# EnnaDelfen/SUHMO

Measured on AMD Instinct MI355X. Metric: multigrid V-cycles/s (FAS head solve) + GSRB cell-updates/s; achieved HBM GB/s vs peak, higher is better.
Workload: dtype f64; 1 GPU; SHMIP-A head solve, 4096x4096 cells per GPU (square cells of 24.4 m), single AMR level, 64x64 boxes, 6 MG depths, 4+4 GSRB sweeps per depth, 16 bottom (BASELINE north_star: 4096^2 single-level); partition=none

## Files before the change

suhmo_amd/csrc/suhmo_bcoef.hip:

```cpp
#include "suhmo_hier.h"
#include "suhmo_level_int.h"
#include "suhmo_batch.h"
#include <algorithm>
#include <cmath>
#include <initializer_list>
#include <type_traits>
__device__ __forceinline__ void d_gradcc_val(const DV &v, const FP &fp, int hasMask, int i, int j, double &gx, double &gy)
{
    const double *__restrict__ phi = fp.f[SUHMO_F_PHI];
    int idx = cidx(v, i, j);
    double c = phi[idx];
    double e = phiE(v, phi, idx, i, c, false), w = phiW(v, phi, idx, i, c, false);
    double n = phiN(v, phi, idx, j, c, false), s = phiS(v, phi, idx, j, c, false);
    double gW = v.fdx * (c - w), gE = v.fdx * (e - c), gS = v.fdy * (c - s), gN = v.fdy * (n - c);
    if (hasMask) {
        const double *__restrict__ m = fp.f[SUHMO_F_MASK];
        bool mc = m[idx] < 1e-6;
        if (mc || m[idx - 1] < 1e-6) gW = 0.0;
        if (mc || m[idx + 1] < 1e-6) gE = 0.0;
        if (mc || m[idx - v.P] < 1e-6) gS = 0.0;
        if (mc || m[idx + v.P] < 1e-6) gN = 0.0;
    }
    gx = 0.5 * (gW + gE);
    gy = 0.5 * (gS + gN);
}
__device__ __forceinline__ void d_gradcc_at(const DV &v, const FP &fp, int hasMask, int i, int j)
{
    if (i >= v.nx || j >= v.ny) return;
    double gx, gy;
    d_gradcc_val(v, fp, hasMask, i, j, gx, gy);
    const int idx = cidx(v, i, j);
    fp.f[SUHMO_F_GRADX][idx] = gx;
    fp.f[SUHMO_F_GRADY][idx] = gy;
}
__device__ __forceinline__ void d_gradcc(const DV &v, const FP &fp, int hasMask)
{
    d_gradcc_at(v, fp, hasMask, blockIdx.x * blockDim.x + threadIdx.x, blockIdx.y * blockDim.y + threadIdx.y);
}
template <class T> __global__ __launch_bounds__(256) void k_gradcc(T t) { d_gradcc(t.view(), t.fields(), t.phys().use_mask_gradients); }
__global__ __launch_bounds__(256) void k_gradcc_list(DV v, FP fp, int hasMask, const int2 *__restrict__ cells, int n)
{
    const int t = blockIdx.x * blockDim.x + threadIdx.x;
    if (t >= n) return;
    d_gradcc_at(v, fp, hasMask, cells[t].x, cells[t].y);
}
__device__ __forceinline__ void d_grad_ghosts(const DV &v, double *__restrict__ gx, double *__restrict__ gy)
{
    int t = blockIdx.x * blockDim.x + threadIdx.x;
    double *g2[2] = {gx, gy};
    if (t < 2 * v.ny) {
        int side = t / v.ny, j = t % v.ny;
        if (v.cfx[side]) return;
        for (int c = 0; c < 2; c++) {
            double *g = g2[c];
            if (side == 0) { int idx = cidx(v, 0, j); g[idx - 1] = v.per[0] ? g[idx + v.nx - 1] : 2.0 * g[idx] - g[idx + 1]; }
            else { int idx = cidx(v, v.nx - 1, j); g[idx + 1] = v.per[0] ? g[idx - (v.nx - 1)] : 2.0 * g[idx] - g[idx - 1]; }
        }
        return;
    }
    t -= 2 * v.ny;
    if (t < 2 * v.nx) {
        int side = t / v.nx, i = t % v.nx;
        if (v.ext[side]) return;
        for (int c = 0; c < 2; c++) {
            double *g = g2[c];
            if (side == 0) { int idx = cidx(v, i, 0); g[idx - v.P] = v.per[1] ? g[idx + (v.ny - 1) * v.P] : 2.0 * g[idx] - g[idx + v.P]; }
            else { int idx = cidx(v, i, v.ny - 1); g[idx + v.P] = v.per[1] ? g[idx - (v.ny - 1) * v.P] : 2.0 * g[idx] - g[idx - v.P]; }
        }
    }
}
template <class T> __global__ void k_grad_ghosts(T t)
{
    const FP &fp = t.fields();
    d_grad_ghosts(t.view(), fp.f[SUHMO_F_GRADX], fp.f[SUHMO_F_GRADY]);
}
__device__ __forceinline__ void d_gradcc_ghosts(const DV &v, const FP &fp, int hasMask)
{
    const int i = blockIdx.x * blockDim.x + threadIdx.x, j = blockIdx.y * blockDim.y + threadIdx.y;
    if (i >= v.nx || j >= v.ny) return;
    double gx, gy, ox, oy;
    d_gradcc_val(v, fp, hasMask, i, j, gx, gy);
    const int idx = cidx(v, i, j);
    double *__restrict__ GX = fp.f[SUHMO_F_GRADX], *__restrict__ GY = fp.f[SUHMO_F_GRADY];
    GX[idx] = gx; GY[idx] = gy;
    if (i == 0 && !v.cfx[0]) {
        d_gradcc_val(v, fp, hasMask, v.per[0] ? v.nx - 1 : 1, j, ox, oy);
        GX[idx - 1] = v.per[0] ? ox : 2.0 * gx - ox; GY[idx - 1] = v.per[0] ? oy : 2.0 * gy - oy;
    }
    if (i == v.nx - 1 && !v.cfx[1]) {
        d_gradcc_val(v, fp, hasMask, v.per[0] ? 0 : v.nx - 2, j, ox, oy);
        GX[idx + 1] = v.per[0] ? ox : 2.0 * gx - ox; GY[idx + 1] = v.per[0] ? oy : 2.0 * gy - oy;
    }
    if (j == 0 && !v.ext[0]) {
        d_gradcc_val(v, fp, hasMask, i, v.per[1] ? v.ny - 1 : 1, ox, oy);
        GX[idx - v.P] = v.per[1] ? ox : 2.0 * gx - ox; GY[idx - v.P] = v.per[1] ? oy : 2.0 * gy - oy;
    }
    if (j == v.ny - 1 && !v.ext[1]) {
        d_gradcc_val(v, fp, hasMask, i, v.per[1] ? 0 : v.ny - 2, ox, oy);
        GX[idx + v.P] = v.per[1] ? ox : 2.0 * gx - ox; GY[idx + v.P] = v.per[1] ? oy : 2.0 * gy - oy;
    }
}
__global__ __launch_bounds__(256) void k_gradcc_ghosts(OnBoxes t) { d_gradcc_ghosts(t.view(), t.fields(), t.phys().use_mask_gradients); }
__global__ __launch_bounds__(256) void k_gradcc_ghosts_lv(suhmo_lvboxes lv, int hasMask)
{
    int z = blockIdx.z, q = -1;
#pragma unroll
    for (int t = 0; t < SUHMO_LVMAX; t++)
        if (t < lv.n && q < 0) { if (z < lv.nbox[t]) q = t; else z -= lv.nbox[t]; }
    if (q < 0) return;
    const DV *dv = nullptr; const FP *fp = nullptr;
#pragma unroll
    for (int t = 0; t < SUHMO_LVMAX; t++) if (t == q) { dv = lv.dv[t]; fp = lv.fp[t]; }
    d_gradcc_ghosts(dv[z], fp[z], hasMask);
}
__device__ __forceinline__ double d_re_val(const FP &fp, const suhmo_phys_t &ph, int idx)
{
    double gx = fp.f[SUHMO_F_GRADX][idx], gy = fp.f[SUHMO_F_GRADY][idx], B = fp.f[SUHMO_F_B][idx];
    double sg = sqrt(gx * gx + gy * gy);
    double discr = 1.0 + 4.0 * ph.omega * (B * B * B * ph.grav * sg) / (12.0 * ph.nu * ph.nu);
    return (-1.0 + sqrt(discr)) / (2.0 * ph.omega);
}
__device__ __forceinline__ void d_re(const DV &v, const FP &fp, suhmo_phys_t ph)
{
    int i = (int)(blockIdx.x * blockDim.x + threadIdx.x) - 1, j = (int)(blockIdx.y * blockDim.y + threadIdx.y) - 1;
    if (i > v.nx || j > v.ny) return;
    bool xo = (i < 0 || i >= v.nx), yo = (j < 0 || j >= v.ny);
    if (xo && yo) return;
    int idx = cidx(v, i, j);
    fp.f[SUHMO_F_RE][idx] = d_re_val(fp, ph, idx);
}
template <class T> __global__ __launch_bounds__(256) void k_re(T t) { d_re(t.view(), t.fields(), t.phys()); }
__device__ __forceinline__ double bcoef_face(const suhmo_phys_t &ph, double Rc, double Rm, double Bc, double Bm,
                                             double mc, double mm, bool dom_edge)
{
    double Ref = 0.5 * (Rc + Rm), Bf = 0.5 * (Bc + Bm);
    double mec;
    if (fabs(mc - mm) < 1e-10) mec = (mc > 0.0) ? 1.0 : -1.0; else mec = 0.0;
    if (dom_edge) mec = 0.0;
    double num_q = -(Bf * Bf * Bf * ph.grav);
    double denom_q = 12.0 * ph.nu * (1.0 + ph.omega * Ref);
    if (mec < 0.0 && ph.cutOffB > 0) return 0.0;
    return num_q / denom_q;
}
__device__ __forceinline__ void d_bcoef_faces(const DV &v, const FP &fp, suhmo_phys_t ph)
{
    int i = blockIdx.x * blockDim.x + threadIdx.x, j = blockIdx.y * blockDim.y + threadIdx.y;
    if (i > v.nx || j > v.ny) return;
    int idx = cidx(v, i, j);
    const double *__restrict__ Re = fp.f[SUHMO_F_RE], *__restrict__ B = fp.f[SUHMO_F_B], *__restrict__ m = fp.f[SUHMO_F_MASK];
    if (j < v.ny)
        fp.f[SUHMO_F_BX][idx] = bcoef_face(ph, Re[idx], Re[idx - 1], B[idx], B[idx - 1], m[idx], m[idx - 1], i + v.i0 == 0 || i + v.i0 == v.nxg);
    if (i < v.nx) {
        int jg = j + v.j0;
        fp.f[SUHMO_F_BY][idx] = bcoef_face(ph, Re[idx], Re[idx - v.P], B[idx], B[idx - v.P], m[idx], m[idx - v.P], jg == 0 || jg == v.nyg);
    }
}
template <class T> __global__ __launch_bounds__(256) void k_bcoef_faces(T t) { d_bcoef_faces(t.view(), t.fields(), t.phys()); }
__global__ __launch_bounds__(256) void k_re_bcoef(OnBoxes t)
{
    const DV &v = t.view();
    const FP &fp = t.fields();
    const suhmo_phys_t &ph = t.phys();
    const int i = (int)(blockIdx.x * blockDim.x + threadIdx.x) - 1, j = (int)(blockIdx.y * blockDim.y + threadIdx.y) - 1;
    if (i > v.nx || j > v.ny) return;
    const bool xo = (i < 0 || i >= v.nx), yo = (j < 0 || j >= v.ny);
    if (xo && yo) return;
    const int idx = cidx(v, i, j);
    const double Rc = d_re_val(fp, ph, idx);
    fp.f[SUHMO_F_RE][idx] = Rc;
    if (i < 0 || j < 0) return;
    const double *__restrict__ B = fp.f[SUHMO_F_B], *__restrict__ m = fp.f[SUHMO_F_MASK];
    if (j < v.ny)
        fp.f[SUHMO_F_BX][idx] = bcoef_face(ph, Rc, d_re_val(fp, ph, idx - 1), B[idx], B[idx - 1], m[idx], m[idx - 1], i + v.i0 == 0 || i + v.i0 == v.nxg);
    if (i < v.nx) {
        const int jg = j + v.j0;
        fp.f[SUHMO_F_BY][idx] = bcoef_face(ph, Rc, d_re_val(fp, ph, idx - v.P), B[idx], B[idx - v.P], m[idx], m[idx - v.P], jg == 0 || jg == v.nyg);
    }
}

template <bool INTERIOR, int BT_X, int BT_Y, bool MASKED>
__device__ __forceinline__ void bcoef_tile(const DV &v, const FP &fp, const suhmo_phys_t &ph, int hasMask_, double *sphi, double *sB, double *sM,
                                           unsigned *negflag, unsigned epoch, unsigned *smallflag)
{
    const int hasMask = MASKED ? hasMask_ : 0;
    constexpr int PW = BT_X + 4, PH = BT_Y + 4;
    constexpr int RW = BT_X + 2, RH = BT_Y + 2;
    constexpr int TX = BT_X + 2, TY = 256 / TX;
    constexpr int NK = RH / TY;
    static_assert(TX * TY == 256 && RH % TY == 0, "tile shape");
    double *sre = sphi;
    const int i0 = blockIdx.x * BT_X, j0 = blockIdx.y * BT_Y;
    const int tx = threadIdx.x, ty = threadIdx.y;
    const double *__restrict__ phi = fp.f[SUHMO_F_PHI], *__restrict__ Bf = fp.f[SUHMO_F_B], *__restrict__ mk = fp.f[SUHMO_F_MASK];
    double *__restrict__ bxo = fp.f[SUHMO_F_BX], *__restrict__ byo = fp.f[SUHMO_F_BY];
    const bool halo_lo = v.ext[0], halo_hi = v.ext[1], selfper_y = v.per[1] && !halo_lo && !halo_hi;
    auto xin = [&](int i) { return INTERIOR || (i >= 0 && i < v.nx) || v.per[0]; };
    auto yin = [&](int j) { return INTERIOR || (j >= 0 && j < v.ny) || selfper_y || (j < 0 && halo_lo && j >= -v.gy) || (j >= v.ny && halo_hi && j < v.ny + v.gy); };
    auto wrapx = [&](int i) { return (!INTERIOR && v.per[0]) ? (i < 0 ? i + v.nx : (i >= v.nx ? i - v.nx : i)) : i; };
    auto wrapy = [&](int j) { return (!INTERIOR && selfper_y) ? (j < 0 ? j + v.ny : (j >= v.ny ? j - v.ny : j)) : j; };

    for (int lj = ty; lj < PH; lj += TY) {
        const int j = j0 - 2 + lj;
        const bool yi = yin(j);
        for (int li = tx; li < PW; li += TX) {
            const int i = i0 - 2 + li;
            const bool xi = xin(i);
            double val = 0.0;
            if (xi && yi) val = phi[cidx(v, wrapx(i), wrapy(j))];
            else if (yi && (i == -1 || i == v.nx)) {
                int ic = i < 0 ? 0 : v.nx - 1, idx = cidx(v, ic, wrapy(j));
                double c = phi[idx];
                val = i < 0 ? phiW(v, phi, idx, ic, c, false) : phiE(v, phi, idx, ic, c, false);
            } else if (xi && (j == -1 || j == v.ny)) {
                int jc = j < 0 ? 0 : v.ny - 1, idx = cidx(v, wrapx(i), jc);
                double c = phi[idx];
                val = j < 0 ? phiS(v, phi, idx, jc, c, false) : phiN(v, phi, idx, jc, c, false);
            }
            sphi[lj * PW + li] = val;
        }
    }
    const int i = i0 - 1 + tx;
    const bool xi = xin(i);
    double Br[NK];
    bool hasB[NK];
    bool neg = false, small = false;
#pragma unroll
    for (int k = 0; k < NK; k++) {
        const int lj = ty + TY * k, j = j0 - 1 + lj;
        hasB[k] = INTERIOR || (i >= -1 && i <= v.nx && j >= -v.gy && j <= v.ny + v.gy - 1 && !((i < 0 || i >= v.nx) && (j < 0 || j >= v.ny)));
        double b = 0.0, m = 0.0;
        if (hasB[k]) { int idx = cidx(v, i, j); b = Bf[idx]; if (MASKED) m = mk[idx]; }
        if (MASKED) {
            neg = neg || (m < 0.0 && i >= 0 && i < v.nx && j >= 0 && j < v.ny);
            small = small || (hasB[k] && m < 1e-6 && j >= -1 && j <= v.ny);
        }
        Br[k] = b;
        sB[lj * RW + tx] = b;
        if (MASKED) sM[lj * RW + tx] = m;
    }
    if (MASKED && negflag && neg) *negflag = epoch;
    if (MASKED && smallflag && small) *smallflag = 1u;
    __syncthreads();
    auto gradcc = [&](int p, int gi, int gj, double &gx, double &gy) {
        double c = sphi[p], w = sphi[p - 1], e = sphi[p + 1], s = sphi[p - PW], n = sphi[p + PW];
        double gW = v.fdx * (c - w), gE = v.fdx * (e - c), gS = v.fdy * (c - s), gN = v.fdy * (n - c);
        if (hasMask) {
            int idx = cidx(v, wrapx(gi), wrapy(gj));
            bool mc = mk[idx] < 1e-6;
            if (mc || mk[idx - 1] < 1e-6) gW = 0.0;
            if (mc || mk[idx + 1] < 1e-6) gE = 0.0;
            if (mc || mk[idx - v.P] < 1e-6) gS = 0.0;
            if (mc || mk[idx + v.P] < 1e-6) gN = 0.0;
        }
        gx = 0.5 * (gW + gE); gy = 0.5 * (gS + gN);
    };
    double rer[NK];
#pragma unroll
    for (int k = 0; k < NK; k++) {
        const int lj = ty + TY * k, j = j0 - 1 + lj;
        const bool yi = yin(j);
        const int p = (lj + 1) * PW + (tx + 1);
        double gx = 0.0, gy = 0.0;
        if (xi && yi) {
            gradcc(p, i, j, gx, gy);
        } else if (xi != yi) {
            int d = 0, di = 0, dj = 0;
            if (!xi && (i == -1 || i == v.nx)) { di = i < 0 ? 1 : -1; d = di; }
            else if (!yi && (j == -1 || j == v.ny)) { dj = j < 0 ? 1 : -1; d = dj * PW; }
            if (d != 0) {
                double g1x, g1y, g2x, g2y;
                gradcc(p + d, i + di, j + dj, g1x, g1y);
                gradcc(p + 2 * d, i + 2 * di, j + 2 * dj, g2x, g2y);
                gx = 2.0 * g1x - g2x; gy = 2.0 * g1y - g2y;
            }
        }
        double re = 0.0;
        if (hasB[k]) {
            double B = Br[k];
            double sg = sqrt(gx * gx + gy * gy);
            double discr = 1.0 + 4.0 * ph.omega * (B * B * B * ph.grav * sg) / (12.0 * ph.nu * ph.nu);
            re = (-1.0 + sqrt(discr)) / (2.0 * ph.omega);
        }
        rer[k] = re;
    }
    __syncthreads();
#pragma unroll
    for (int k = 0; k < NK; k++) sre[(ty + TY * k) * RW + tx] = rer[k];
    __syncthreads();
    const int nxt = (!INTERIOR && i0 + BT_X >= v.nx) ? v.nx - i0 + 1 : BT_X, nyt = (!INTERIOR && j0 + BT_Y >= v.ny) ? v.ny - j0 + 1 : BT_Y;
    const int fx = tx - 1;
    if (fx >= 0 && fx < nxt) {
        for (int fy = ty; fy < nyt; fy += TY) {
            const int j = j0 + fy, idx = cidx(v, i, j), r = (fy + 1) * RW + tx;
            if (INTERIOR || j < v.ny)
                bxo[idx] = bcoef_face(ph, sre[r], sre[r - 1], sB[r], sB[r - 1], MASKED ? sM[r] : 1.0, MASKED ? sM[r - 1] : 1.0, !INTERIOR && (i == 0 || i == v.nx));
            if (INTERIOR || i < v.nx) {
                int jg = j + v.j0;
                byo[idx] = bcoef_face(ph, sre[r], sre[r - RW], sB[r], sB[r - RW], MASKED ? sM[r] : 1.0, MASKED ? sM[r - RW] : 1.0, !INTERIOR && (jg == 0 || jg == v.nyg));
            }
        }
    }
}
struct MaskHalo { const double *m[SUHMO_MAXDEPTH]; int nx[SUHMO_MAXDEPTH], ny[SUHMO_MAXDEPTH], P[SUHMO_MAXDEPTH], gy[SUHMO_MAXDEPTH]; int nd, lo, hi; };
__global__ __launch_bounds__(256) void k_mask_halo_report(MaskHalo h, unsigned *negflag, unsigned epoch, unsigned *smallflag)
{
    const int d = blockIdx.z, i = blockIdx.x * blockDim.x + threadIdx.x;
    if (d >= h.nd || i >= h.nx[d]) return;
    const int g = h.gy[d];
    bool neg = false, small = false;
    for (int r = blockIdx.y; r < 2 * g; r += gridDim.y) {
        const bool top = r >= g;
        if (top ? !h.hi : !h.lo) continue;
        const int j = top ? h.ny[d] + (r - g) : -1 - r;
        const double *__restrict__ row = h.m[d] + (long)(j + g) * h.P[d] + SUHMO_XOFF;
        const double m = row[i];
        neg = neg || m < 0.0;
        const int dist = top ? r - g : r;
        small = small || ((d == 0 && dist < 2) ? m < 1e-6 : m < 0.0);
        if (smallflag && d == 0 && i == 0 && (j == -1 || j == h.ny[d])) small = small || row[-1] < 1e-6 || row[h.nx[d]] < 1e-6;
    }
    if (negflag && neg) *negflag = epoch;
    if (smallflag && small) *smallflag = 1u;
}
template <int BT_X, int BT_Y, bool MASKED>
__device__ __forceinline__ void d_bcoef_fused(const DV &v, const FP &fp, const suhmo_phys_t &ph, int hasMask, unsigned *negflag, unsigned epoch, unsigned *smallflag)
{
    __shared__ double sphi[(BT_X + 4) * (BT_Y + 4)], sB[(BT_X + 2) * (BT_Y + 2)], sM[MASKED ? (BT_X + 2) * (BT_Y + 2) : 1];
    const int i0 = blockIdx.x * BT_X, j0 = blockIdx.y * BT_Y;
    const bool interior = i0 - 2 >= 0 && i0 + BT_X + 1 <= v.nx - 1 && j0 - 2 >= 0 && j0 + BT_Y + 1 <= v.ny - 1;
    if (interior) bcoef_tile<true, BT_X, BT_Y, MASKED>(v, fp, ph, hasMask, sphi, sB, sM, negflag, epoch, smallflag);
    else bcoef_tile<false, BT_X, BT_Y, MASKED>(v, fp, ph, hasMask, sphi, sB, sM, negflag, epoch, smallflag);
}
template <class T, int BT_X, int BT_Y, bool MASKED = true>
__global__ __launch_bounds__(256) void k_bcoef_fused(T t, unsigned *negflag, unsigned epoch, unsigned *smallflag)
{
    const suhmo_phys_t ph = t.phys();
    if (std::is_same<T, OnMembers>::value) { negflag = nullptr; epoch = 0u; smallflag = nullptr; }
    d_bcoef_fused<BT_X, BT_Y, MASKED>(t.view(), t.fields(), ph, ph.use_mask_gradients, negflag, epoch, smallflag);
}
template <class T> int launch_bcoef_fused(const T &t, bool wide, unsigned *flag, unsigned epoch, hipStream_t st, unsigned *small, bool unmasked)
{
    if constexpr (std::is_same<T, OnLevel>::value) {
        const dim3 gw((t.nx() + 125) / 126, (t.ny() + 13) / 14), gn((t.nx() + 61) / 62, (t.ny() + 13) / 14);
        unsigned *const none = nullptr;
        if (unmasked && wide) return launch_grid(k_bcoef_fused<T, 126, 14, false>, t, gw, dim3(128, 2), st, none, 0u, none);
        if (unmasked) return launch_grid(k_bcoef_fused<T, 62, 14, false>, t, gn, dim3(64, 4), st, none, 0u, none);
        if (wide) return launch_grid(k_bcoef_fused<T, 126, 14>, t, gw, dim3(128, 2), st, flag, epoch, small);
    }
    return launch_grid(k_bcoef_fused<T, 62, 14>, t, dim3((t.nx() + 61) / 62, (t.ny() + 13) / 14), dim3(64, 4), st, flag, epoch, small);
}
template int launch_bcoef_fused(const OnMembers &, bool, unsigned *, unsigned, hipStream_t, unsigned *, bool);
void suhmo_mask_poll(suhmo_level *L)
{
    if (!L->mask_scan_pending) return;
    const hipError_t e = hipEventQuery(L->mask_ev);
    if (e == hipErrorNotReady) { (void)hipGetLastError(); return; }
    L->mask_scan_pending = 0;
    if (e != hipSuccess) { (void)hipGetLastError(); L->mask_scan_errors++; return; }
    if (L->mask_scan_version == L->mask_version) L->mask_state = *(volatile unsigned *)L->mask_host ? SUHMO_MASK_DIRTY : SUHMO_MASK_CLEAN;
}
int suhmo_mask_scan_begin(suhmo_level *L, hipStream_t st)
{
    if (!L->mask_ev) HIPCHK(hipEventCreateWithFlags(&L->mask_ev, hipEventDisableTiming));
    HIPCHK(hipMemsetAsync(suhmo_mask_scan_word(L), 0, sizeof(unsigned), st));
    return 0;
}
int suhmo_mask_scan_end(suhmo_level *L, hipStream_t st)
{
    HIPCHK(hipMemcpyAsync(L->mask_host, suhmo_mask_scan_word(L), sizeof(unsigned), hipMemcpyDeviceToHost, st));
    HIPCHK(hipEventRecord(L->mask_ev, st));
    L->mask_scan_pending = 1; L->mask_scan_version = L->mask_version; L->mask_scans++;
    return 0;
}
template <class T> int launch_re(const T &t, hipStream_t st) { return launch_over(k_re<T>, t, GHOSTED, st); }
template <class T> int launch_bcoef_faces(const T &t, hipStream_t st) { return launch_over(k_bcoef_faces<T>, t, FACES, st); }
template <class T> int launch_grad_cc(const T &t, hipStream_t st)
{
    int rc = launch_over(k_gradcc<T>, t, CELLS, st);
    return rc ? rc : launch_over(k_grad_ghosts<T>, t, PERIMETER, st);
}
template int launch_re(const OnLevel &, hipStream_t);
template int launch_re(const OnBoxes &, hipStream_t);
template int launch_re(const OnMembers &, hipStream_t);
template int launch_bcoef_faces(const OnLevel &, hipStream_t);
template int launch_bcoef_faces(const OnBoxes &, hipStream_t);
template int launch_bcoef_faces(const OnMembers &, hipStream_t);
template int launch_grad_cc(const OnMembers &, hipStream_t);

static bool bcoef_is_fused(const suhmo_level *L, int depth)
{
    const Depth &D = L->d[depth];
    return L->bcoef_fused && D.v.nx >= 4 && D.v.ny >= 4 && (!(D.v.ext[0] || D.v.ext[1]) || (D.v.gy >= 2 && D.v.ny >= 2))
           && L->desc.nx_global == 0;
}
bool suhmo_mask_would_scan(const suhmo_level *L)
{
    return L->mask_known && !L->mask_view && L->mask_scan_errors < 3 && L->mask_state == SUHMO_MASK_UNKNOWN && !L->mask_scan_pending && L->mask_host
           && !L->mask_capturing && bcoef_is_fused(L, 0);
}
extern "C" int suhmo_level_update_operator(suhmo_level_t *L, int depth, suhmo_stream_t s)
{
    SUHMO_TIME("VCAMRNonLinearPoissonOp::UpdateOperator");
    ARG(L); ARG(depth >= 0 && depth < L->ndepth);
    HIPCHK(hipSetDevice(L->device));
    hipStream_t st = (hipStream_t)s;
    Depth &D = L->d[depth];
    const bool fused = bcoef_is_fused(L, depth);
    int rc = suhmo_ensure_phi_halo(L, depth, fused ? 2 : 1, st); if (rc) return rc;
    if (fused) {
        const bool wide = L->bcoef_tile_x == 126 && D.v.nx >= 256;
        unsigned *flag = nullptr;
        if (depth == 0) { L->maskflag_epoch = 0; L->mask_reported = 0; }
        if (depth == 0 && !L->mask_capturing) suhmo_mask_poll(L);
        const bool unmasked = depth == 0 && suhmo_mask_clean(L, 0);
        unsigned *small = nullptr;
        const bool scan = depth == 0 && suhmo_mask_would_scan(L);
        if (scan) { small = suhmo_mask_scan_word(L); if ((rc = suhmo_mask_scan_begin(L, st))) return rc; }
        if (depth == 0 && L->mask_capturing && L->mask_known && !L->mask_view && !unmasked && L->mask_host) { small = suhmo_mask_scan_word(L); L->mask_scan_captured = 1; }
        if (depth == 0 && L->skip_mask && !unmasked) {
            flag = suhmo_mask_report_word(L);
            if (++L->mask_epoch == 0) L->mask_epoch = 1;
            L->mask_reported = 1;
        }
        if ((rc = launch_bcoef_fused(on_level(L, depth), wide, flag, L->mask_epoch, st, small, unmasked))) return rc;
        if (unmasked) L->bcoef_unmasked++;
        if ((flag || small) && (D.v.ext[0] || D.v.ext[1])) {
            MaskHalo h;
            h.nd = 0; h.lo = D.v.ext[0]; h.hi = D.v.ext[1];
            const int last = L->coarse_mask_ok ? (L->agg ? L->agg_depth : L->ndepth) : 1;
            int gmax = 1;
            for (int k = 0; k < last && k < SUHMO_MAXDEPTH; k++) {
                const Depth &Dk = L->d[k];
                h.m[k] = Dk.fp.f[SUHMO_F_MASK]; h.nx[k] = Dk.v.nx; h.ny[k] = Dk.v.ny; h.P[k] = Dk.v.P; h.gy[k] = Dk.v.gy;
                if (Dk.v.gy > gmax) gmax = Dk.v.gy;
// ... 402 lines not shown
```

suhmo_amd/csrc/suhmo_common.h:

```cpp
#pragma once
#include <hip/hip_runtime.h>
#include <cstdio>
#include <cstdlib>
#include <cstring>
#include <utility>
#include <string>
#include <vector>
#include "../../include/suhmo_hip.h"

#define SUHMO_XOFF 16
#define SUHMO_MAXDEPTH 16

struct DV {
    int nx, ny;
    int P;
    int gy;
    int rows;
    int j0, nyg;
    double dx, dy;
    double rdx, rdy;
    double fdx, fdy;
    double alpha, beta;
    int bct[2][2];
    double two_v[2][2];
    double neu[2][2];
    int per[2];
    int ext[2];
    int i0, nxg;
    int cfx[2];
    int rk[2];
};

struct FP { double *f[SUHMO_F_COUNT]; };

__host__ __device__ __forceinline__ int cidx(const DV &v, int i, int j)
{
    return (j + v.gy) * v.P + SUHMO_XOFF + i;
}

__device__ __forceinline__ double phiW(const DV &v, const double *__restrict__ p, int idx, int i, double c, bool homog)
{
    if (i > 0 || v.cfx[0]) return p[idx - 1];
    if (v.per[0]) return p[idx + v.nx - 1];
    if (v.bct[0][0] == 0) return (homog ? 0.0 : v.two_v[0][0]) - c;
    return homog ? c : c + v.neu[0][0];
}
__device__ __forceinline__ double phiE(const DV &v, const double *__restrict__ p, int idx, int i, double c, bool homog)
{
    if (i < v.nx - 1 || v.cfx[1]) return p[idx + 1];
    if (v.per[0]) return p[idx - (v.nx - 1)];
    if (v.bct[0][1] == 0) return (homog ? 0.0 : v.two_v[0][1]) - c;
    return homog ? c : c + v.neu[0][1];
}
__device__ __forceinline__ double phiS(const DV &v, const double *__restrict__ p, int idx, int j, double c, bool homog)
{
    if (j > 0 || v.ext[0]) return p[idx - v.P];
    if (v.per[1]) return p[idx + (v.ny - 1) * v.P];
    if (v.bct[1][0] == 0) return (homog ? 0.0 : v.two_v[1][0]) - c;
    return homog ? c : c + v.neu[1][0];
}
__device__ __forceinline__ double phiN(const DV &v, const double *__restrict__ p, int idx, int j, double c, bool homog)
{
    if (j < v.ny - 1 || v.ext[1]) return p[idx + v.P];
    if (v.per[1]) return p[idx - (v.ny - 1) * v.P];
    if (v.bct[1][1] == 0) return (homog ? 0.0 : v.two_v[1][1]) - c;
    return homog ? c : c + v.neu[1][1];
}

__device__ __forceinline__ void nl_terms(const suhmo_phys_t &ph, double phi, double B, double Pi,
                                         double zb, double mask, double &nl, double &dnl)
{
    if (!ph.use_NL || mask < 0.0) { nl = 0.0; dnl = 0.0; return; }
    double N = Pi - ph.rho_w_g * (phi - zb);
    nl = -ph.A * B * N * N * N;
    dnl = 3.0 * ph.A * B * 1000.0 * ph.grav * N * N;
    if (ph.cutOffbr > B) {
        nl = nl * (1.0 - (ph.cutOffbr - B) / ph.cutOffbr);
        dnl = dnl * B / ph.cutOffbr;
    }
    if (ph.maxOffbr < B) {
        nl = nl * (1.0 - (ph.maxOffbr - B) / ph.maxOffbr);
        dnl = dnl * B / ph.maxOffbr;
    }
}

__device__ __forceinline__ double lofphi_cell(const DV &v, double aterm, double c, double e, double w,
                                              double n, double s, double bxE, double bxW, double byN,
                                              double byS, double nl)
{
    return aterm * c
           - v.beta * (bxE * (e - c) * v.rdx - bxW * (c - w) * v.rdx
                       + byN * (n - c) * v.rdy - byS * (c - s) * v.rdy)
           + nl;
}

__device__ __forceinline__ double lambda_cell(const DV &v, double aterm, double bxE, double bxW,
                                              double byN, double byS)
{
    double lam = aterm;
    lam = lam + v.rdx * v.beta * (bxE + bxW);
    lam = lam + v.rdy * v.beta * (byN + byS);
    return lam;
}

struct Depth {
    DV v;
    FP fp;
    size_t elems;
    int nbox;
    int prolong_pending;
    int rhs_pending;
    double *phi_alt;
    int phi_fresh;
};

struct VGraph {
    int key[4]; hipGraphExec_t exec;
    double *p0[SUHMO_MAXDEPTH], *a0[SUHMO_MAXDEPTH];
    double *p1[SUHMO_MAXDEPTH], *a1[SUHMO_MAXDEPTH];
    double *rhs;
    int rout_req, rout_done, rout_np; const double *rout_rhs;
    int mask_clean; long n_bcoef_unmasked, n_relax_unmasked;
    int has_scan;
};
struct ProfEv { hipEvent_t a, b; long cells; int restricts; };

struct suhmo_level {
    int ndepth;
    int batch_owned;
    int stub;
    Depth d[SUHMO_MAXDEPTH];
    suhmo_level_desc_t desc;
    std::vector<int> boxes;
    suhmo_phys_t ph;
    int device;
    double *scratch;
    double *hscratch;
    double *hscratch_dev;
    unsigned long long hseq;
    int poll_readback;
    size_t scratch_elems;
    suhmo_exchange_fn ex;
    suhmo_allreduce_max_fn ar;
    suhmo_allreduce_fn ar2;
    int (*ard)(void *user, double *dev_values, int n, int op, suhmo_stream_t s);
    void *user;
    int (*ex_begin)(void *user);
    int (*ex_end)(void *user, suhmo_level *L, suhmo_stream_t s);
    long graph_max_cells;
    std::vector<VGraph> vgraphs; int vgraph_seen[4]; hipStream_t gstream;
    long vgraph_replays;
    suhmo_level *gap; double gap_dt;
    void *rccl;
    int faces_deferred;
    void *ipc; int ipc_owner;
    long agg_min_cells;
    int agg_depth, agg_world, agg_rank;
    suhmo_level *agg;
    int agg_static_stale;
    suhmo_allgather_fn ag; void *ag_user;
    double *agg_send, *agg_recv; size_t agg_cap; long agg_gathers;
    int resout_req, resout_armed, resout_done; const double *resout_rhs; long resout_count;
    int resout_np;
    long frhs_stream, frhs_tile;
    int prof_on;
    std::vector<ProfEv> prof;
    int gsrb_variant;
    long fused_min_cells;
    int bcoef_fused;
    int bcoef_tile_x;
    int fused_nt;
    int fused_restrict;
    int fused_hc;
    int fas_rhs_fused;
    int strips_rhs_local;
    int skip_mask;
    int mask_reported;
    int coarse_mask_ok;
    unsigned mask_epoch, maskflag_epoch;
    int mask_known, mask_state;
    unsigned mask_version, mask_scan_version;
    int mask_scan_pending, mask_capturing;
    int mask_scan_captured;
    int mask_view;
    int mask_scan_errors;
    unsigned *mask_host; hipEvent_t mask_ev;
    long mask_scans, bcoef_unmasked, relax_unmasked;
    int overlap_halo;
    hipStream_t xstream; hipEvent_t xev[2]; long overlapped;
    int tile_strips;
    int tile_chunks;
    int resid_in_relax;
    int fas_rhs_in_relax;
    long tile_max_cells;
    int tile_restrict;
    int tile_order;
    int bottom_solver; long bottom_one_launch_max_cells;
    unsigned long long *bottom_ctr; long bottom_host_iters, bottom_host_solves;
    int gsrb_tile, tile_t, tile_s;
};

enum { SUHMO_MASK_UNKNOWN = 0, SUHMO_MASK_CLEAN = 1, SUHMO_MASK_DIRTY = 2 };
static inline void suhmo_mask_written(suhmo_level *L)
{
    L->coarse_mask_ok = 0; L->maskflag_epoch = 0;
    L->mask_version++; L->mask_state = SUHMO_MASK_UNKNOWN;
}
static inline void suhmo_mask_halo_written(suhmo_level *L) { L->mask_version++; L->mask_state = SUHMO_MASK_UNKNOWN; }
bool suhmo_mask_would_scan(const suhmo_level *L);
#define SUHMO_HSCRATCH_DOUBLES 64
#define SUHMO_HSCRATCH_MASK 60
static inline unsigned *suhmo_mask_report_word(const suhmo_level *L) { return (unsigned *)(L->scratch + L->scratch_elems - 1); }
static inline unsigned *suhmo_mask_scan_word(const suhmo_level *L) { return suhmo_mask_report_word(L) + 1; }
int suhmo_mask_scan_begin(suhmo_level *L, hipStream_t st);
int suhmo_mask_scan_end(suhmo_level *L, hipStream_t st);
void suhmo_mask_poll(suhmo_level *L);
static inline bool suhmo_mask_clean(const suhmo_level *L, int depth)
{
    return L->mask_known && !L->mask_view && L->mask_state == SUHMO_MASK_CLEAN && (depth == 0 || L->coarse_mask_ok) && L->desc.nx_global == 0;
}
void suhmo_set_error(const char *fmt, ...);
struct SuhmoTimer { const char *name; double t0; int mode; explicit SuhmoTimer(const char *n); ~SuhmoTimer(); };
#define SUHMO_TIME(label) SuhmoTimer suhmo_tm_(label)
#define HIPCHK(x) do { hipError_t e_ = (x); if (e_ != hipSuccess) { \
    suhmo_set_error("%s:%d %s -> %s", __FILE__, __LINE__, #x, hipGetErrorString(e_)); return -2; } } while (0)
#define ARG(cond) do { if (!(cond)) { suhmo_set_error("%s:%d bad argument: %s", __FILE__, __LINE__, #cond); return -1; } } while (0)

double *suhmo_field(suhmo_level *L, int depth, int field);
int suhmo_level_create_(suhmo_level_t **out, const suhmo_level_desc_t *desc, bool stub);
void suhmo_level_share_transport(suhmo_level *dst, const suhmo_level *src);
int suhmo_level_materialize_(suhmo_level *L);
void suhmo_fp_changed();
unsigned long suhmo_fp_epoch();
struct SwapGuard {
    double **a, **b; bool armed;
    SwapGuard() : a(nullptr), b(nullptr), armed(false) {}
    void arm(double **a_, double **b_) { a = a_; b = b_; std::swap(*a, *b); armed = true; suhmo_fp_changed(); }
    void back() { if (armed) { std::swap(*a, *b); armed = false; suhmo_fp_changed(); } }
    ~SwapGuard() { back(); }
};
int suhmo_average_operator_all(suhmo_level *L, int nd, hipStream_t st);
int suhmo_restrict_both(suhmo_level *L, int depth, hipStream_t st);
bool suhmo_gsrb_can_fuse_prolong(suhmo_level *L, int depth, int sweeps);
int suhmo_level_residual_and_norm(suhmo_level *L, double *out, hipStream_t st);
int suhmo_level_norm_from_partials(suhmo_level *L, int np, double *out, hipStream_t st);
bool suhmo_gsrb_can_fuse_rhs(suhmo_level *L, int depth, int sweeps, bool rhs_local = false);
int suhmo_launch_gsrb(suhmo_level *L, int depth, int sweeps, int tail, hipStream_t st, int *restricted = nullptr);
void suhmo_level_drop_graphs(suhmo_level *L);
int suhmo_ensure_phi_halo(suhmo_level *L, int depth, int need, hipStream_t st);
int suhmo_fas_coarse_rhs(suhmo_level *L, int depth, hipStream_t st, int hcomp = 0);
struct HostSlot { double *val; unsigned long long *flag; unsigned long long seq; };
HostSlot suhmo_host_slot(suhmo_level *L);
int suhmo_readback(suhmo_level *L, hipStream_t st, double *out, double *out2 = nullptr);
HostSlot suhmo_reduce_slot(suhmo_level *L);
int suhmo_reduce_finish(suhmo_level *L, hipStream_t st, int n, int op, double *out, double *out2 = nullptr);
__device__ __forceinline__ void suhmo_publish(const HostSlot &h, double v)
{
    if (!h.val) return;
    h.val[0] = v;
    __hip_atomic_store(h.flag, h.seq, __ATOMIC_RELEASE, __HIP_MEMORY_SCOPE_SYSTEM);
}
int suhmo_build_mg_coefficients(suhmo_level *L, bool with_faces, hipStream_t st);
void suhmo_ipc_release(suhmo_level *L);
int suhmo_ipc_batch(suhmo_level *L, int open, hipStream_t st);
int suhmo_agg_setup(suhmo_level *L);
void suhmo_agg_release(suhmo_level *L);
int suhmo_agg_gather_static(suhmo_level *L, bool with_faces, hipStream_t st);
int suhmo_agg_gather_faces(suhmo_level *L, int nd, hipStream_t st);
int suhmo_agg_gather_state(suhmo_level *L, hipStream_t st);
int suhmo_agg_scatter(suhmo_level *L, hipStream_t st);
int suhmo_exchange_list(suhmo_level *L, int depth, const int *fields, int n, hipStream_t st);
bool suhmo_bottom_one_launch(const suhmo_level *L, int dep);
int suhmo_bottom_configure(suhmo_level *L, int solver, long one_launch_max_cells);
long suhmo_bottom_counter(const suhmo_level *L, int which);
int suhmo_bottom_solve(suhmo_level *L, int dep, int tail, hipStream_t st);
static inline int suhmo_halo_rows(const DV &v) { return v.gy < v.ny ? v.gy : v.ny; }
struct SolveNoInit {
    double rnorm, initial_rnorm, norm_last;
    int iter;
    void start(double r) { rnorm = r; initial_rnorm = r; norm_last = 2.0 * r; iter = 0; }
    bool go(const suhmo_solver_params_t *sp) const
    {
        const bool goNorm = rnorm > sp->norm_thresh, goRedu = rnorm > sp->eps * initial_rnorm, goIter = iter < sp->max_iter;
        const bool goHang = iter < sp->imin || rnorm < (1.0 - sp->hang) * norm_last, goMin = iter < sp->iter_min;
        return goMin || (goIter && goRedu && goHang && goNorm);
    }
    void cycled(double r) { norm_last = rnorm; rnorm = r; iter++; }
};
template <class Residual, class Cycle>
int suhmo_solve_no_init(const suhmo_solver_params_t *sp, int *iters, double *hist, Residual residual, Cycle cycle)
{
    int rc;
    double rnorm = 0.0;
    if ((rc = residual(&rnorm))) return rc;
    SolveNoInit s;
    s.start(rnorm);
    if (hist) hist[0] = rnorm;
    while (s.go(sp)) {
        if ((rc = cycle()) || (rc = residual(&rnorm))) return rc;
        s.cycled(rnorm);
        if (hist) hist[s.iter] = rnorm;
    }
    if (iters) *iters = s.iter;
    return 0;
}
```

suhmo_amd/csrc/suhmo_fas.hip:

```cpp
#include "suhmo_common.h"
#include <cstdlib>

static int eff_depths(const suhmo_level *L, const suhmo_solver_params_t *sp)
{
    int nd = L->ndepth;
    if (sp->max_depth >= 0 && sp->max_depth + 1 < nd) nd = sp->max_depth + 1;
    return nd;
}

static int relax(suhmo_level *L, int dep, int sweeps, int tail, suhmo_stream_t s, bool observable = false, int *restricted = nullptr)
{
    L->resout_armed = observable && dep == 0 && L->resout_req && L->resid_in_relax;
    int rc = suhmo_launch_gsrb(L, dep, sweeps, tail, (hipStream_t)s, restricted);
    L->resout_armed = 0;
    if (rc) return rc;
    if (sweeps > 0 && observable) return suhmo_level_fill_ghosts(L, dep, SUHMO_F_PHI, 1, s);
    return 0;
}

static int rows_after_prolong(int dep, int num_smooth)
{
    int tail_post = 2;
    for (int d = 1; d <= dep; d++) tail_post = (2 * num_smooth + tail_post + 1) / 2;
    return 2 * num_smooth + tail_post;
}
int suhmo_prolong_with_halo(suhmo_level *L, int depth, hipStream_t st);

static int fas_cycle(suhmo_level *L, int dep, const suhmo_solver_params_t *sp, int nd, suhmo_stream_t s)
{
    int rc;
    const int S = sp->num_smooth;
    const int tail_post = dep == 0 ? 2 : (rows_after_prolong(dep - 1, S) + 1) / 2;
    if (dep == nd - 1) {
        if (!L->bottom_solver) return relax(L, dep, sp->num_bottom, tail_post, s, dep == 0);
        if ((rc = relax(L, dep, sp->num_bottom, tail_post, s))) return rc;
        if ((rc = suhmo_bottom_solve(L, dep, tail_post, (hipStream_t)s))) return rc;
        return dep == 0 ? suhmo_level_fill_ghosts(L, dep, SUHMO_F_PHI, 0, s) : 0;
    }
    Depth &C = L->d[dep + 1];
    int restricted = 0;
    if ((rc = relax(L, dep, S, rows_after_prolong(dep, S), s, false, &restricted))) return rc;
    if (!restricted && (rc = suhmo_restrict_both(L, dep, (hipStream_t)s))) return rc;
    if (L->agg && dep + 1 == L->agg_depth) {
        suhmo_level *A = L->agg;
        const int ndA = nd - L->agg_depth;
        if (L->agg_static_stale && (rc = suhmo_agg_gather_static(L, true, (hipStream_t)s))) return rc;
        if ((rc = suhmo_agg_gather_state(L, (hipStream_t)s))) return rc;
        const int next_sweeps = ndA == 1 ? sp->num_bottom : S;
        if (suhmo_gsrb_can_fuse_rhs(A, 0, next_sweeps)) A->d[0].rhs_pending = 1;
        else if ((rc = suhmo_fas_coarse_rhs(A, 0, (hipStream_t)s))) return rc;
        if ((rc = fas_cycle(A, 0, sp, ndA, s))) return rc;
        if ((rc = suhmo_agg_scatter(L, (hipStream_t)s))) return rc;
        if (suhmo_gsrb_can_fuse_prolong(L, dep, S)) L->d[dep].prolong_pending = 1;
        else if ((rc = suhmo_prolong_with_halo(L, dep, (hipStream_t)s))) return rc;
        return relax(L, dep, S, tail_post, s, dep == 0);
    }
    const bool one_pass_rhs = L->fas_rhs_fused != 0;
    const bool rhs_local = L->ex && (C.v.rk[0] || C.v.rk[1]) && one_pass_rhs && L->desc.nx_global == 0 && L->strips_rhs_local
                           && suhmo_halo_rows(C.v) >= 2;
    if (rhs_local) {
        static const int both[2] = {SUHMO_F_PHI, SUHMO_F_RES};
        if ((rc = suhmo_exchange_list(L, dep + 1, both, 2, (hipStream_t)s))) return rc;
    } else if ((rc = suhmo_ensure_phi_halo(L, dep + 1, suhmo_halo_rows(C.v), (hipStream_t)s))) return rc;
    if (one_pass_rhs && (L->desc.nx_global == 0)) {
        const int next_sweeps = (dep + 1 == nd - 1) ? sp->num_bottom : S;
        if (suhmo_gsrb_can_fuse_rhs(L, dep + 1, next_sweeps, rhs_local)) C.rhs_pending = 1;
        else if ((rc = suhmo_fas_coarse_rhs(L, dep + 1, (hipStream_t)s, rhs_local ? suhmo_halo_rows(C.v) - 1 : 0))) return rc;
    } else {
        HIPCHK(hipMemcpyAsync(C.fp.f[SUHMO_F_PHIOLD], C.fp.f[SUHMO_F_PHI], C.elems * sizeof(double), hipMemcpyDeviceToDevice, (hipStream_t)s));
        if ((rc = suhmo_level_apply_op(L, dep + 1, 0, s))) return rc;
        if ((rc = suhmo_level_axby(L, dep + 1, SUHMO_F_RHS, SUHMO_F_RES, SUHMO_F_LPHI, 1.0, 1.0, s))) return rc;
    }
    if (!rhs_local && (rc = suhmo_level_exchange(L, dep + 1, SUHMO_F_RHS, s))) return rc;
    if ((rc = fas_cycle(L, dep + 1, sp, nd, s))) return rc;
    if (suhmo_gsrb_can_fuse_prolong(L, dep, S)) {
        L->d[dep].prolong_pending = 1;
    } else {
        if ((rc = suhmo_prolong_with_halo(L, dep, (hipStream_t)s))) return rc;
    }
    return relax(L, dep, S, tail_post, s, dep == 0);
}

static int vcycle_body(suhmo_level *L, const suhmo_solver_params_t *sp, int nd, suhmo_stream_t s)
{
    int rc;
    if (sp->bcoeff_otf) {
        L->faces_deferred = 1;
        rc = suhmo_level_update_operator(L, 0, s);
        if (rc) { L->faces_deferred = 0; return rc; }
        if (L->mask_reported) L->maskflag_epoch = L->mask_epoch;
        if ((rc = suhmo_average_operator_all(L, nd, (hipStream_t)s))) return rc;
    } else L->maskflag_epoch = 0;
    rc = fas_cycle(L, 0, sp, nd, s);
    L->maskflag_epoch = 0;
    return rc;
}

void suhmo_level_drop_graphs(suhmo_level *L)
{
    if (getenv("SUHMO_GRAPH_DEBUG")) { int ok = 0; for (VGraph &g : L->vgraphs) ok += g.exec != nullptr; fprintf(stderr,
        "[suhmo] level %dx%d: %zu V-cycle graphs, %d executable\n", L->d[0].v.nx, L->d[0].v.ny, L->vgraphs.size(), ok); }
    for (VGraph &g : L->vgraphs) if (g.exec) (void)hipGraphExecDestroy(g.exec);
    L->vgraphs.clear();
    if (L->gstream) { (void)hipStreamDestroy(L->gstream); L->gstream = nullptr; }
}
static int vcycle_graph(suhmo_level *L, const suhmo_solver_params_t *sp, int nd, suhmo_stream_t s, bool &done)
{
    done = false;
    const int key[4] = {sp->num_smooth, sp->num_bottom, sp->bcoeff_otf, nd};
    const int mask_clean = (suhmo_mask_clean(L, 0) ? 1 : 0) | (L->ndepth > 1 && suhmo_mask_clean(L, 1) ? 2 : 0);
    const bool scanning = sp->bcoeff_otf && suhmo_mask_would_scan(L);
    auto launch = [&](const VGraph &g) {
        int rc = 0;
        if (scanning && (rc = suhmo_mask_scan_begin(L, (hipStream_t)s))) return rc;
        HIPCHK(hipGraphLaunch(g.exec, (hipStream_t)s)); L->vgraph_replays++;
        if (scanning && (rc = suhmo_mask_scan_end(L, (hipStream_t)s))) return rc;
        return 0;
    };
    auto replayed = [&](const VGraph &g) {
        L->bcoef_unmasked += g.n_bcoef_unmasked; L->relax_unmasked += g.n_relax_unmasked;
        if (g.rout_done) { L->resout_done = 1; L->resout_count++; L->resout_np = g.rout_np; }
    };
    auto at_start = [&](const VGraph &g) {
        if (memcmp(g.key, key, sizeof(key)) || g.mask_clean != mask_clean) return false;
        for (int d = 0; d < L->ndepth; d++) if (L->d[d].fp.f[SUHMO_F_PHI] != g.p0[d] || L->d[d].phi_alt != g.a0[d]) return false;
        if (g.rout_req != (L->resid_in_relax ? L->resout_req : 0) || g.rout_rhs != L->resout_rhs) return false;
        return L->d[0].fp.f[SUHMO_F_RHS] == g.rhs;
    };
    for (const VGraph &g : L->vgraphs)
        if (at_start(g)) {
            if (!g.exec || (scanning && !g.has_scan)) return 0;
            { int rc = launch(g); if (rc) return rc; }
            for (int d = 0; d < L->ndepth; d++) { L->d[d].fp.f[SUHMO_F_PHI] = g.p1[d]; L->d[d].phi_alt = g.a1[d]; } suhmo_fp_changed();
            replayed(g);
            done = true;
            return 0;
        }
    for (int k = 0; k < 4; k++) if (L->vgraph_seen[k] != key[k]) { memcpy(L->vgraph_seen, key, sizeof(key)); return 0; }
    if (L->vgraphs.size() >= 16) return 0;
    if (!L->gstream) HIPCHK(hipStreamCreateWithFlags(&L->gstream, hipStreamNonBlocking));
    VGraph g; memcpy(g.key, key, sizeof(key)); g.exec = nullptr; g.mask_clean = mask_clean; g.has_scan = 0;
    for (int d = 0; d < SUHMO_MAXDEPTH; d++) { g.p0[d] = g.a0[d] = g.p1[d] = g.a1[d] = nullptr; }
    for (int d = 0; d < L->ndepth; d++) { g.p0[d] = L->d[d].fp.f[SUHMO_F_PHI]; g.a0[d] = L->d[d].phi_alt; }
    g.rhs = L->d[0].fp.f[SUHMO_F_RHS];
    g.rout_req = L->resid_in_relax ? L->resout_req : 0; g.rout_rhs = L->resout_rhs; g.rout_done = 0;
    const int rout_before = L->resout_done; const long rout_count = L->resout_count;
    const long bcoef_unmasked = L->bcoef_unmasked, relax_unmasked = L->relax_unmasked;
    HIPCHK(hipStreamSynchronize((hipStream_t)s));
    hipGraph_t graph = nullptr;
    hipError_t e = hipStreamBeginCapture(L->gstream, hipStreamCaptureModeThreadLocal);
    int rc = 0;
    if (e == hipSuccess) {
        L->mask_capturing = 1; L->mask_scan_captured = 0;
        rc = vcycle_body(L, sp, nd, (suhmo_stream_t)L->gstream);
        L->mask_capturing = 0; g.has_scan = L->mask_scan_captured;
        e = hipStreamEndCapture(L->gstream, &graph);
    }
    g.n_bcoef_unmasked = L->bcoef_unmasked - bcoef_unmasked; g.n_relax_unmasked = L->relax_unmasked - relax_unmasked;
    L->bcoef_unmasked = bcoef_unmasked; L->relax_unmasked = relax_unmasked;
    g.rout_done = L->resout_count != rout_count;
    g.rout_np = L->resout_np;
    L->resout_done = rout_before; L->resout_count = rout_count;
    bool clean = true;
    for (int d = 0; d < L->ndepth; d++) {
        clean = clean && !L->d[d].prolong_pending && !L->d[d].rhs_pending;
        g.p1[d] = L->d[d].fp.f[SUHMO_F_PHI]; g.a1[d] = L->d[d].phi_alt;
        L->d[d].prolong_pending = 0; L->d[d].rhs_pending = 0;
        L->d[d].fp.f[SUHMO_F_PHI] = g.p0[d]; L->d[d].phi_alt = g.a0[d];
    }
    if (e == hipSuccess && rc == 0 && clean && graph && hipGraphInstantiate(&g.exec, graph, nullptr, nullptr, 0) != hipSuccess) g.exec = nullptr;
    if (!(e == hipSuccess && rc == 0 && clean)) g.exec = nullptr;
    if (graph) (void)hipGraphDestroy(graph);
    (void)hipGetLastError();
    L->vgraphs.push_back(g);
    if (!g.exec || (scanning && !g.has_scan)) return 0;
    if ((rc = launch(g))) return rc;
    for (int d = 0; d < L->ndepth; d++) { L->d[d].fp.f[SUHMO_F_PHI] = g.p1[d]; L->d[d].phi_alt = g.a1[d]; } suhmo_fp_changed();
    replayed(g);
    done = true;
    return 0;
}

extern "C" int suhmo_level_vcycle(suhmo_level_t *L, const suhmo_solver_params_t *sp, suhmo_stream_t s)
{
    SUHMO_TIME("AMRFASMultiGrid::VCycle");
    ARG(L && sp);
    HIPCHK(hipSetDevice(L->device));
    int nd = eff_depths(L, sp);
    const Depth &D = L->d[0];
    const bool ext = D.v.ext[0] || D.v.ext[1];
    const bool host_bottom = L->bottom_solver && !suhmo_bottom_one_launch(L, nd - 1);
    suhmo_mask_poll(L);
    if (L->graph_max_cells > 0 && !L->ex && !ext && !L->prof_on && !host_bottom && (long)D.v.nx * D.v.ny <= L->graph_max_cells) {
        bool done = false;
        int rc = vcycle_graph(L, sp, nd, s, done);
        if (rc || done) return rc;
    }
    return vcycle_body(L, sp, nd, s);
}

extern "C" int suhmo_level_solve(suhmo_level_t *L, const suhmo_solver_params_t *sp, int *iters, double *hist, suhmo_stream_t s)
{
    SUHMO_TIME("AMRFASMultiGrid::solve");
    ARG(L && sp);
    HIPCHK(hipSetDevice(L->device));
    bool have_res = false;
    int np = 0;
    auto residual = [&](double *rnorm) {
        if (!have_res) return suhmo_level_residual_and_norm(L, rnorm, (hipStream_t)s);
        if (np > 0) return suhmo_level_norm_from_partials(L, np, rnorm, (hipStream_t)s);
        return suhmo_level_norm(L, 0, SUHMO_F_RES, 0, rnorm, s);
    };
    auto cycle = [&] {
        L->resout_req = 1 | 4; L->resout_rhs = nullptr; L->resout_done = 0; L->resout_np = 0;
        int rc = suhmo_level_vcycle(L, sp, s);
        have_res = L->resout_done != 0;
        np = have_res ? L->resout_np : 0;
        L->resout_req = 0; L->resout_done = 0; L->resout_np = 0;
        return rc;
    };
    int rc = suhmo_solve_no_init(sp, iters, hist, residual, cycle);
    if (rc) return rc;
    return suhmo_level_fill_ghosts(L, 0, SUHMO_F_PHI, 0, s);
}
```

suhmo_amd/csrc/suhmo_gsrb.hip:

```cpp
#include "suhmo_hier.h"
#include "suhmo_batch.h"
#include <type_traits>

template <bool HAS_ALPHA>
__device__ __forceinline__ void d_gsrb_pass_simple(const DV &v, const FP &fp, suhmo_phys_t ph, int pass, int jlo, int jhi,
                                                   const FP *__restrict__ ft = nullptr, const int2 *__restrict__ push = nullptr)
{
    int j = jlo + (int)(blockIdx.y * blockDim.y + threadIdx.y);
    int t = blockIdx.x * blockDim.x + threadIdx.x;
    if (j > jhi) return;
    int i = 2 * t + ((j + v.j0 + pass) & 1);
    if (i >= v.nx) return;
    double *__restrict__ phi = fp.f[SUHMO_F_PHI];
    int idx = cidx(v, i, j);
    double c = phi[idx];
    double e = phiE(v, phi, idx, i, c, false), w = phiW(v, phi, idx, i, c, false);
    double n = phiN(v, phi, idx, j, c, false), s = phiS(v, phi, idx, j, c, false);
    double bxW = fp.f[SUHMO_F_BX][idx], bxE = fp.f[SUHMO_F_BX][idx + 1];
    double byS = fp.f[SUHMO_F_BY][idx], byN = fp.f[SUHMO_F_BY][idx + v.P];
    double nl, dnl;
    nl_terms(ph, c, fp.f[SUHMO_F_B][idx], fp.f[SUHMO_F_PI][idx], fp.f[SUHMO_F_ZB][idx],
             fp.f[SUHMO_F_MASK][idx], nl, dnl);
    double aterm = HAS_ALPHA ? v.alpha * fp.f[SUHMO_F_ACOEF][idx] : v.alpha;
    double lofphi = lofphi_cell(v, aterm, c, e, w, n, s, bxE, bxW, byN, byS, nl);
// ... 89 lines not shown
            const int dx = li < BOXG ? BOXG - li : (li >= BOXG + tw ? li - (BOXG + tw - 1) : 0), dy = lj < BOXG ? BOXG - lj : (lj >= BOXG + th ? lj - (BOXG + th - 1) : 0);
            const int d = max(dx, dy);
            const FP &fb = b == k ? fk : ft[b];
            if (d >= BOXG) { pl[q] = fb.f[fsrc][off]; continue; }
            const int Pb = b == k ? v.P : vt[b].P;
            cb[s][c] = b; co[s][c] = off; cd[s][c] = d;
            pl[q] = fb.f[fsrc][off];
            c_rhs[s][c] = fb.f[SUHMO_F_RHS][off];
            c_bxW[s][c] = fb.f[SUHMO_F_BX][off]; c_bxE[s][c] = fb.f[SUHMO_F_BX][off + 1];
            c_byS[s][c] = fb.f[SUHMO_F_BY][off]; c_byN[s][c] = fb.f[SUHMO_F_BY][off + Pb];
            c_B[s][c] = fb.f[SUHMO_F_B][off]; c_Pi[s][c] = fb.f[SUHMO_F_PI][off]; c_zb[s][c] = fb.f[SUHMO_F_ZB][off]; c_mk[s][c] = fb.f[SUHMO_F_MASK][off];
            c_at[s][c] = HAS_ALPHA ? v.alpha * fb.f[SUHMO_F_ACOEF][off] : v.alpha;
        }
    __syncthreads();
    int nk[S][2];
    double hW[S][2], hE[S][2], hS[S][2], hN[S][2];
#pragma unroll
    for (int s = 0; s < S; s++)
#pragma unroll
        for (int c = 0; c < 2; c++) {
            nk[s][c] = 0; hW[s][c] = hE[s][c] = hS[s][c] = hN[s][c] = 0.0;
            const int q = cq[s][c], b = cb[s][c];
            if (b < 0) continue;
            const bool oW = own[q - 1] < 0, oE = own[q + 1] < 0, oS = own[q - LW] < 0, oN = own[q + LW] < 0;
            if (!(oW || oE || oS || oN)) continue;
            const DV &vb = b == k ? v : vt[b];
            const double *__restrict__ psrc = (b == k ? fk : ft[b]).f[fsrc];
            const int off = co[s][c];
            if (oW) { if (vb.cfx[0]) { nk[s][c] |= 1; hW[s][c] = psrc[off - 1]; } else if (vb.bct[0][0] == 0) { nk[s][c] |= 2; hW[s][c] = vb.two_v[0][0];
                } else { nk[s][c] |= 3; hW[s][c] = vb.neu[0][0]; } }
            if (oE) { if (vb.cfx[1]) { nk[s][c] |= 1 << 2; hE[s][c] = psrc[off + 1]; } else if (vb.bct[0][1] == 0) { nk[s][c] |= 2 << 2; hE[s][c] = vb.two_v[0][1];
                } else { nk[s][c] |= 3 << 2; hE[s][c] = vb.neu[0][1]; } }
            if (oS) { if (vb.ext[0]) { nk[s][c] |= 1 << 4; hS[s][c] = psrc[off - vb.P]; } else if (vb.bct[1][0] == 0) { nk[s][c] |= 2 << 4;
                hS[s][c] = vb.two_v[1][0]; } else { nk[s][c] |= 3 << 4; hS[s][c] = vb.neu[1][0]; } }
            if (oN) { if (vb.ext[1]) { nk[s][c] |= 1 << 6; hN[s][c] = psrc[off + vb.P]; } else if (vb.bct[1][1] == 0) { nk[s][c] |= 2 << 6;
                hN[s][c] = vb.two_v[1][1]; } else { nk[s][c] |= 3 << 6; hN[s][c] = vb.neu[1][1]; } }
        }
    auto outside = [](int kind, double g, double c) { return kind == 1 ? g : (kind == 2 ? g - c : c + g); };
    auto update = [&](int q, int kinds, double g_w, double g_e, double g_s, double g_n, double rhs, double bxW, double bxE, double byS, double byN, double B,
        double Pi, double zb, double mk, double at) {
        const double c = pl[q];
        double w, e, sv, n;
        if (kinds == 0) { w = pl[q - 1]; e = pl[q + 1]; sv = pl[q - LW]; n = pl[q + LW]; }
        else {
            w = (kinds & 3) ? outside(kinds & 3, g_w, c) : pl[q - 1];
            e = ((kinds >> 2) & 3) ? outside((kinds >> 2) & 3, g_e, c) : pl[q + 1];
            sv = ((kinds >> 4) & 3) ? outside((kinds >> 4) & 3, g_s, c) : pl[q - LW];
            n = ((kinds >> 6) & 3) ? outside((kinds >> 6) & 3, g_n, c) : pl[q + LW];
        }
        double nl, dnl;
        nl_terms(ph, c, B, Pi, zb, mk, nl, dnl);
        const double lofphi = lofphi_cell(v, at, c, e, w, n, sv, bxE, bxW, byN, byS, nl);
        const double lam = lambda_cell(v, at, bxE, bxW, byN, byS);
        const double denom = 1.0e-16 + lam + dnl;
        pl[q] = c + (rhs - lofphi) / denom;
    };
    for (int m = 0; m < npass; m++) {
        const int reach = npass - 1 - m;
        if ((m & 1) == 0) {
#pragma unroll
            for (int s = 0; s < S; s++)
                if (cb[s][0] >= 0 && cd[s][0] <= reach)
                    update(cq[s][0], nk[s][0], hW[s][0], hE[s][0], hS[s][0], hN[s][0], c_rhs[s][0], c_bxW[s][0], c_bxE[s][0], c_byS[s][0], c_byN[s][0], c_B[s][0],
                        c_Pi[s][0], c_zb[s][0], c_mk[s][0], c_at[s][0]);
        } else {
#pragma unroll
            for (int s = 0; s < S; s++)
                if (cb[s][1] >= 0 && cd[s][1] <= reach)
                    update(cq[s][1], nk[s][1], hW[s][1], hE[s][1], hS[s][1], hN[s][1], c_rhs[s][1], c_bxW[s][1], c_bxE[s][1], c_byS[s][1], c_byN[s][1], c_B[s][1],
                        c_Pi[s][1], c_zb[s][1], c_mk[s][1], c_at[s][1]);
        }
        __syncthreads();
    }
    const double *__restrict__ psrc = fk.f[fsrc];
    double *__restrict__ pdst = fk.f[fdst];
    const bool gW = bcg && !v.cfx[0] && !v.per[0], gE = bcg && !v.cfx[1] && !v.per[0], gS = bcg && !v.ext[0] && !v.per[1], gN = bcg && !v.ext[1] && !v.per[1];
    for (int q = tid; q < tw * th; q += BOXNT) {
        const int jj = q / tw, ii = q - jj * tw, gi = x0 + ii, gj = y0 + jj, idx = cidx(v, gi, gj);
        const double c = pl[(BOXG + jj) * LW + BOXG + ii];
        pdst[idx] = c;
        if (gW && gi == 0) pdst[idx - 1] = phiW(v, pdst, idx, gi, c, true);
        if (gE && gi == v.nx - 1) pdst[idx + 1] = phiE(v, pdst, idx, gi, c, true);
        if (gS && gj == 0) pdst[idx - v.P] = phiS(v, pdst, idx, gj, c, true);
        if (gN && gj == v.ny - 1) pdst[idx + v.P] = phiN(v, pdst, idx, gj, c, true);
    }
    if (blockIdx.x == 0)
        for (int q = tid; q < 2 * (v.nx + 2) + 2 * v.ny; q += BOXNT) {
            int ii, jj;
            bool filled;
            if (q < v.nx + 2) { ii = q - 1; jj = -1; filled = gS && ii >= 0 && ii < v.nx; }
            else if (q < 2 * (v.nx + 2)) { ii = q - (v.nx + 2) - 1; jj = v.ny; filled = gN && ii >= 0 && ii < v.nx; }
            else if (q < 2 * (v.nx + 2) + v.ny) { ii = -1; jj = q - 2 * (v.nx + 2); filled = gW; }
            else { ii = v.nx; jj = q - 2 * (v.nx + 2) - v.ny; filled = gE; }
            if (filled) continue;
            const int idx = cidx(v, ii, jj);
            pdst[idx] = psrc[idx];
        }
}
template <int G, int T, int S>
static void launch_box(const suhmo_multi &m, const suhmo_phys_t &ph, bool has_alpha, const void *halo, const int *hbase, int fsrc, int fdst, int npass, int bc_ghosts, hipStream_t st)
{
    const dim3 grd(((m.maxnx + T - 1) / T) * ((m.maxny + T - 1) / T), m.nbox);
    if (has_alpha) hipLaunchKernelGGL((k_gsrb_box_m<true, G, T, S>), grd, dim3(BoxGeom<G, T, S>::NT), 0, st, m.dv, m.fp, (const int2 *)halo, hbase, ph, fsrc, fdst, npass, bc_ghosts);
    else hipLaunchKernelGGL((k_gsrb_box_m<false, G, T, S>), grd, dim3(BoxGeom<G, T, S>::NT), 0, st, m.dv, m.fp, (const int2 *)halo, hbase, ph, fsrc, fdst, npass, bc_ghosts);
}
int suhmo_multi_gsrb_box(const suhmo_multi &m, const suhmo_phys_t &ph, bool has_alpha, const void *halo, const int *hbase, int fsrc, int fdst, int npass, int bc_ghosts, hipStream_t st)
{
    if (m.nbox <= 0) return 0;
    if (npass < 1 || npass > 2 * SUHMO_BOX_HALO) { suhmo_set_error("internal: %d colour passes in one box launch", npass); return -4; }
    if (npass > 4) launch_box<8, 16, 1>(m, ph, has_alpha, halo, hbase, fsrc, fdst, npass, bc_ghosts, st);
    else launch_box<4, 16, 1>(m, ph, has_alpha, halo, hbase, fsrc, fdst, npass, bc_ghosts, st);
    HIPCHK(hipGetLastError());
    return 0;
}

struct FusedGeom {
    int W;
    int Hc;
    int nstrips, nchunks, ntiles;
    int ylo, yhi;
    int jbeg, jend;
    int wrap_y;
    const unsigned *negflag; unsigned mask_epoch;
    int nchl, chunk0, chunk1, edges;
    const double *pc, *pco; int Pc, gyc;
    double *rres, *rphi; int rP, rgy;
    const double *fres; double *frhs, *flphi, *fphiold;
    const double *ortrue; double *ores, *olphi;
    double *onorm;
};

template <bool MASKED> struct RowMask { double mask[2]; };
template <> struct RowMask<false> {};
template <bool MASKED>
struct RowCoef : RowMask<MASKED> {
    double rhs[2], B[2], Pi[2], zb[2], a[2], byS[2], byN[2];
    double bx0, bx1, bx2;
};
template <bool MASKED> __device__ __forceinline__ double row_mask(const RowCoef<MASKED> &q, int a)
{
    if constexpr (MASKED) return q.mask[a]; else return 1.0;
}
#define CP2(d, s, f) d.f[0] = s.f[0]; d.f[1] = s.f[1]
template <bool HAS_ALPHA, bool MASKED>
__device__ __forceinline__ void copy_coef(RowCoef<MASKED> &d, const RowCoef<MASKED> &s)
{
    CP2(d, s, rhs); CP2(d, s, B); CP2(d, s, Pi); CP2(d, s, zb);
    if constexpr (MASKED) { CP2(d, s, mask); }
    if (HAS_ALPHA) { CP2(d, s, a); }
    CP2(d, s, byS); CP2(d, s, byN);
    d.bx0 = s.bx0; d.bx1 = s.bx1; d.bx2 = s.bx2;
}

template <int K, bool HAS_ALPHA, int NT, int RM = 0, bool FRHS = false, bool MASKED = true>
__global__ __launch_bounds__(NT) void k_gsrb_fused(DV v, FP fp, const double *__restrict__ pin,
                                                   double *__restrict__ pout, suhmo_phys_t ph, FusedGeom g)
{
    constexpr bool ROUT = RM == 2, RR = RM != 0;
    static_assert(!(FRHS && (RR || HAS_ALPHA)), "the right-hand side is formed in the plain launch of an alpha = 0 operator");
    constexpr int LW = 2 * NT, R = 2 * K + 3 + (RR ? 1 : 0);
    constexpr int HX = 2 * K + (RR ? 2 : 0), EY = RR ? 1 : 0;
    __shared__ double lds[R * LW];

    int b = blockIdx.x, q = g.ntiles / 8, rem = g.ntiles % 8, xcd = b % 8;
    int tile = xcd * q + (xcd < rem ? xcd : rem) + b / 8;
    int strip = tile / g.nchl, chunk = tile % g.nchl;
    chunk = g.edges ? (chunk < g.chunk0 ? chunk : g.chunk1 + (chunk - g.chunk0)) : g.chunk0 + chunk;

    const int t = threadIdx.x;
    const int c0 = strip * g.W;
    const int xl = 2 * t;
    const int i0 = c0 - HX + xl;
    const bool in_row = xl < g.W + 2 * HX;
    int im = i0;
    if (v.per[0]) { if (im < 0) im += v.nx; else if (im >= v.nx) im -= v.nx; }
    const bool cval = in_row && im >= 0 && im < v.nx;
    const int cend = (c0 + g.W < v.nx) ? c0 + g.W : v.nx;
    const bool own = cval && i0 >= c0 && i0 < cend;

    const int jA = g.jbeg + chunk * g.Hc;
    const int jB = (jA + g.Hc < g.jend) ? jA + g.Hc : g.jend;
    const int jmin = (jA - EY - 2 * K > g.ylo) ? jA - EY - 2 * K : g.ylo;
    const int jmax = (jB - 1 + EY + 2 * K < g.yhi) ? jB - 1 + EY + 2 * K : g.yhi;

    const double *__restrict__ f_rhs = fp.f[SUHMO_F_RHS], *__restrict__ f_B = fp.f[SUHMO_F_B];
    const double *__restrict__ f_Pi = fp.f[SUHMO_F_PI], *__restrict__ f_zb = fp.f[SUHMO_F_ZB];
    const double *__restrict__ f_mask = fp.f[SUHMO_F_MASK], *__restrict__ f_a = fp.f[SUHMO_F_ACOEF];
    const double *__restrict__ f_bx = fp.f[SUHMO_F_BX], *__restrict__ f_by = fp.f[SUHMO_F_BY];

    auto wrapj = [&](int j) { if (g.wrap_y) { if (j < 0) j += v.ny; else if (j >= v.ny) j -= v.ny; } return j; };
    auto ld2 = [&](const double *__restrict__ p, int idx) { return *reinterpret_cast<const double2 *>(p + idx); };

    RowCoef<MASKED> cf0, cf1, cf2, cf3, cf4, cf5;
    double racc = 0.0, raccp = 0.0;
    double nmax = 0.0;
    const bool xbc = !v.per[0] && (c0 - HX <= 0 || c0 + g.W + HX >= v.nx);
    const bool ybc = !v.per[1] && (jmin <= 0 || jmax >= v.ny - 1);
    double2 pnext = make_double2(0.0, 0.0);
    double2 pprev = make_double2(0.0, 0.0);
    bool usemask = false;
    if constexpr (MASKED) usemask = !g.negflag || *g.negflag == g.mask_epoch;

    int sr = 0;
    auto ring = [](int x) { return x < 0 ? x + R : x; };
    for (int r = jmin - 1; r <= jB - 1 + 2 * K + EY; r++) {
        bool lphi = cval && (r + 1 >= jmin) && (r + 1 <= jmax);
        if (lphi) {
            const int jr = wrapj(r + 1);
            pnext = ld2(pin, cidx(v, im, jr));
            if (g.pc) {
                const int ic = ((jr >> 1) + g.gyc) * g.Pc + SUHMO_XOFF + (im >> 1);
                const double corr = 1.0 * g.pc[ic] + (-1.0) * g.pco[ic];
                pnext.x = pnext.x + corr; pnext.y = pnext.y + corr;
            }
        }
        bool lcf = cval && (r >= jmin) && (r <= jmax);
        if (lcf) {
            int idx = cidx(v, im, wrapj(r));
#define LD2(dst, p, ix) { double2 t_ = ld2(p, ix); dst[0] = t_.x; dst[1] = t_.y; }
            LD2(cf0.rhs, (FRHS ? g.fres : f_rhs), idx); LD2(cf0.B, f_B, idx); LD2(cf0.Pi, f_Pi, idx);
            LD2(cf0.zb, f_zb, idx);
            if constexpr (MASKED) { if (usemask) { LD2(cf0.mask, f_mask, idx); } else { cf0.mask[0] = 1.0; cf0.mask[1] = 1.0; } }
            if (HAS_ALPHA) LD2(cf0.a, f_a, idx);
            LD2(cf0.byS, f_by, idx); LD2(cf0.byN, f_by, idx + v.P);
            double2 bxp = ld2(f_bx, idx);
            cf0.bx0 = bxp.x; cf0.bx1 = bxp.y; cf0.bx2 = f_bx[idx + 2];
        }
        __syncthreads();

        if constexpr (FRHS) {
            const int jf = r - 1;
            if (cval && jf >= jmin && jf <= jmax) {
                const int s0 = ring(sr - 1), sN = sr;
                const double *row = lds + s0 * LW;
                double lo[2], cc[2];
#pragma unroll
                for (int a = 0; a < 2; a++) {
                    const int x = xl + a, i = im + a;
                    double c = row[x];
                    double w = row[(a == 0 && xl == 0) ? 0 : x - 1], e = row[(a == 1 && xl == LW - 2) ? LW - 1 : x + 1];
                    double n = lds[sN * LW + x], s = a ? pprev.y : pprev.x;
                    if (xbc) {
                        if (i == 0) w = (v.bct[0][0] == 0) ? v.two_v[0][0] - c : c + v.neu[0][0];
                        if (i == v.nx - 1) e = (v.bct[0][1] == 0) ? v.two_v[0][1] - c : c + v.neu[0][1];
                    }
                    if (ybc) {
                        if (jf == 0 && !v.ext[0]) s = (v.bct[1][0] == 0) ? v.two_v[1][0] - c : c + v.neu[1][0];
                        if (jf == v.ny - 1 && !v.ext[1]) n = (v.bct[1][1] == 0) ? v.two_v[1][1] - c : c + v.neu[1][1];
                    }
                    double nl, dnl;
                    nl_terms(ph, c, cf1.B[a], cf1.Pi[a], cf1.zb[a], row_mask(cf1, a), nl, dnl);
                    const double bxW = a ? cf1.bx1 : cf1.bx0, bxE = a ? cf1.bx2 : cf1.bx1;
                    lo[a] = lofphi_cell(v, v.alpha, c, e, w, n, s, bxE, bxW, cf1.byN[a], cf1.byS[a], nl);
                    cc[a] = c;
                }
                cf1.rhs[0] = 1.0 * cf1.rhs[0] + 1.0 * lo[0]; cf1.rhs[1] = 1.0 * cf1.rhs[1] + 1.0 * lo[1];
                const bool lo_end = v.ext[0] && chunk == 0, hi_end = v.ext[1] && chunk == g.nchunks - 1;
                const int jP0 = lo_end ? jmin : jA, jP1 = hi_end ? jmax + 1 : jB;
                const int jR0 = lo_end ? jmin + 1 : jA, jR1 = hi_end ? jmax : jB;
                if (own && jf >= jP0 && jf < jP1) {
                    const int idx = cidx(v, i0, jf);
                    if (jf >= jR0 && jf < jR1) {
                        *reinterpret_cast<double2 *>(g.flphi + idx) = make_double2(lo[0], lo[1]);
                        *reinterpret_cast<double2 *>(g.frhs + idx) = make_double2(cf1.rhs[0], cf1.rhs[1]);
                    }
                    *reinterpret_cast<double2 *>(g.fphiold + idx) = make_double2(cc[0], cc[1]);
                }
                pprev = make_double2(cc[0], cc[1]);
            }
            __syncthreads();
        }

        auto advance_a = [&](const int m, const RowCoef<MASKED> &q, auto a_tag) {
            constexpr int a = decltype(a_tag)::value;
            const int j = r - m;
            const int x = xl + a, i = im + a;
            const int s0 = ring(sr - m), sN = ring(sr - m + 1), sS = ring(sr - m - 1);
            const double *row = lds + s0 * LW;
            double c = row[x];
            double w = row[(a == 0 && xl == 0) ? 0 : x - 1], e = row[(a == 1 && xl == LW - 2) ? LW - 1 : x + 1];
            double n = lds[sN * LW + x], s = lds[sS * LW + x];
            if (xbc) {
                if (i == 0) w = (v.bct[0][0] == 0) ? v.two_v[0][0] - c : c + v.neu[0][0];
                if (i == v.nx - 1) e = (v.bct[0][1] == 0) ? v.two_v[0][1] - c : c + v.neu[0][1];
            }
            if (ybc) {
                if (j == 0 && !v.ext[0]) s = (v.bct[1][0] == 0) ? v.two_v[1][0] - c : c + v.neu[1][0];
                if (j == v.ny - 1 && !v.ext[1]) n = (v.bct[1][1] == 0) ? v.two_v[1][1] - c : c + v.neu[1][1];
            }
            double nl, dnl;
            nl_terms(ph, c, q.B[a], q.Pi[a], q.zb[a], row_mask(q, a), nl, dnl);
            const double bxW = a ? q.bx1 : q.bx0, bxE = a ? q.bx2 : q.bx1;
            double aterm = HAS_ALPHA ? v.alpha * q.a[a] : v.alpha;
            double lofphi = lofphi_cell(v, aterm, c, e, w, n, s, bxE, bxW, q.byN[a], q.byS[a], nl);
            double lam = lambda_cell(v, aterm, bxE, bxW, q.byN[a], q.byS[a]);
            double denom = 1.0e-16 + lam + dnl;
            lds[s0 * LW + x] = c + (q.rhs[a] - lofphi) / denom;
        };
        auto advance = [&](const int m, const RowCoef<MASKED> &q) {
            const int j = r - m;
            if (j >= jmin && j <= jmax) {
                const int a = (j + v.j0 + ((m - 1) & 1)) & 1;
                if (a) { if (cval) advance_a(m, q, std::integral_constant<int, 1>()); }
                else   { if (cval) advance_a(m, q, std::integral_constant<int, 0>()); }
            }
        };
        advance(1, cf1);
        __syncthreads();
        advance(2, cf2);
        if constexpr (K >= 2) {
            __syncthreads();
            advance(3, cf3);
            __syncthreads();
            advance(4, cf4);
        }

        if constexpr (RR) {
            const int jr = r - 2 * K - 1;
            if (own && jr >= jA && jr < jB && jr >= 0 && jr < v.ny) {
                const RowCoef<MASKED> &q = (K >= 2) ? cf5 : cf3;
                const int s0 = ring(sr - (2 * K + 1)), sN = ring(sr - 2 * K), sS = ring(sr - (2 * K + 2));
                const double *row = lds + s0 * LW;
                double acc = (jr & 1) ? racc : 0.0, accp = (jr & 1) ? raccp : 0.0;
                double lo2[2] = {0.0, 0.0};
#pragma unroll
                for (int a = 0; a < 2; a++) {
                    const int x = xl + a, i = im + a;
                    double c = row[x], w = row[x - 1], e = row[x + 1];
                    double n = lds[sN * LW + x], s = lds[sS * LW + x];
                    if (xbc) {
                        if (i == 0) w = (v.bct[0][0] == 0) ? v.two_v[0][0] - c : c + v.neu[0][0];
                        if (i == v.nx - 1) e = (v.bct[0][1] == 0) ? v.two_v[0][1] - c : c + v.neu[0][1];
                    }
                    if (ybc) {
                        if (jr == 0 && !v.ext[0]) s = (v.bct[1][0] == 0) ? v.two_v[1][0] - c : c + v.neu[1][0];
                        if (jr == v.ny - 1 && !v.ext[1]) n = (v.bct[1][1] == 0) ? v.two_v[1][1] - c : c + v.neu[1][1];
                    }
                    double nl, dnl;
                    nl_terms(ph, c, q.B[a], q.Pi[a], q.zb[a], row_mask(q, a), nl, dnl);
                    const double bxW = a ? q.bx1 : q.bx0, bxE = a ? q.bx2 : q.bx1;
                    double aterm = HAS_ALPHA ? v.alpha * q.a[a] : v.alpha;
                    double lofphi = lofphi_cell(v, aterm, c, e, w, n, s, bxE, bxW, q.byN[a], q.byS[a], nl);
                    if constexpr (ROUT) lo2[a] = lofphi;
                    else {
                        acc = acc + (q.rhs[a] - lofphi) / 4.0;
                        accp = accp + c / 4.0;
                    }
                }
                if constexpr (ROUT) {
                    const int idx = cidx(v, i0, jr);
                    const double2 rt = *reinterpret_cast<const double2 *>(g.ortrue + idx);
                    const double r0 = -1.0 * lo2[0] + 1.0 * rt.x, r1 = -1.0 * lo2[1] + 1.0 * rt.y;
                    *reinterpret_cast<double2 *>(g.ores + idx) = make_double2(r0, r1);
                    if (g.olphi) *reinterpret_cast<double2 *>(g.olphi + idx) = make_double2(lo2[0], lo2[1]);
                    nmax = fmax(nmax, fmax(fabs(r0), fabs(r1)));
                } else if (jr & 1) {
                    const int ic = ((jr >> 1) + g.rgy) * g.rP + SUHMO_XOFF + (i0 >> 1);
                    g.rres[ic] = acc; g.rphi[ic] = accp;
                } else { racc = acc; raccp = accp; }
            }
        }
        {
            const int jo = r - 2 * K;
            if (own && jo >= jA && jo < jB) {
                const int so = ring(sr - 2 * K);
                double2 o = make_double2(lds[so * LW + xl], lds[so * LW + xl + 1]);
                *reinterpret_cast<double2 *>(pout + cidx(v, i0, jo)) = o;
            }
        }
        sr = sr + 1 == R ? 0 : sr + 1;
        if (in_row) { lds[sr * LW + xl] = pnext.x; lds[sr * LW + xl + 1] = pnext.y; }
        if constexpr (RR && K >= 2) copy_coef<HAS_ALPHA, MASKED>(cf5, cf4);
        if constexpr (K >= 2) { copy_coef<HAS_ALPHA, MASKED>(cf4, cf3); copy_coef<HAS_ALPHA, MASKED>(cf3, cf2); }
        else if constexpr (RR) copy_coef<HAS_ALPHA, MASKED>(cf3, cf2);
        copy_coef<HAS_ALPHA, MASKED>(cf2, cf1);
        copy_coef<HAS_ALPHA, MASKED>(cf1, cf0);
    }
    if constexpr (ROUT) {
        if (g.onorm) {
            static_assert(!ROUT || NT == 64, "one wave per workgroup");
#pragma unroll
            for (int o = 32; o > 0; o >>= 1) nmax = fmax(nmax, __shfl_xor(nmax, o));
            if (t == 0) g.onorm[strip * g.nchunks + chunk] = nmax;
        }
    }
}

static bool fused_ok(const suhmo_level *L, const Depth &D, int K)
{
    const DV &v = D.v;
    if (v.nx % 2 || v.nx < 64 || v.ny < 4 * K + 4) return false;
    if (v.cfx[0] || v.cfx[1] || L->desc.nx_global > 0) return false;
    if ((v.ext[0] || v.ext[1]) && (v.gy < 2 * K || v.ny < 2 * K)) return false;
    if (v.per[1] && !(v.ext[0] || v.ext[1]) && v.ny < 4 * K) return false;
    return true;
}

template <int K, int NT, int RM = 0>
static int launch_fused(suhmo_level *L, int depth, int ext_rows, hipStream_t st, int part = 0)
{
    constexpr bool RST = RM == 1, RR = RM != 0;
    Depth &D = L->d[depth];
    const DV &v = D.v;
    if (!D.phi_alt) {
        HIPCHK(hipMalloc(&D.phi_alt, D.elems * sizeof(double)));
        HIPCHK(hipMemsetAsync(D.phi_alt, 0, D.elems * sizeof(double), st));
    }
    FusedGeom g;
    constexpr int HX = 2 * K + (RR ? 2 : 0), EY = RR ? 1 : 0;
    const int maxW = 2 * NT - 2 * HX;
    g.nstrips = (v.nx + maxW - 1) / maxW;
    g.W = 2 * ((v.nx + 2 * g.nstrips - 1) / (2 * g.nstrips));
    g.nstrips = (v.nx + g.W - 1) / g.W;
    const bool unmasked = suhmo_mask_clean(L, depth) && v.alpha == 0.0;
    {
        static int slots_k[3][2] = {{0, 0}, {0, 0}, {0, 0}};
        if (!slots_k[K][unmasked]) {
            int nb = 0, ncu = 0, dev = 0;
            HIPCHK(hipGetDevice(&dev));
            HIPCHK(hipDeviceGetAttribute(&ncu, hipDeviceAttributeMultiprocessorCount, dev));
            if (unmasked) HIPCHK(hipOccupancyMaxActiveBlocksPerMultiprocessor(&nb, (k_gsrb_fused<K, false, NT, RM, false, false>), NT, 0));
            else HIPCHK(hipOccupancyMaxActiveBlocksPerMultiprocessor(&nb, (k_gsrb_fused<K, false, NT, RM>), NT, 0));
            slots_k[K][unmasked] = (nb > 0 ? nb : 1) * (ncu > 0 ? ncu : 256);
        }
        g.jbeg = v.ext[0] ? -ext_rows : 0;
        g.jend = v.ny + (v.ext[1] ? ext_rows : 0);
        const int nrows = g.jend - g.jbeg;
        int nch = slots_k[K][unmasked] / g.nstrips;
        if (nch < 1) nch = 1;
        g.Hc = (nrows + nch - 1) / nch;
        if (g.Hc < 8 * K) g.Hc = 8 * K;
        if ((long)v.nx * v.ny < 2000000L) g.Hc = 6;
        if (L->fused_hc > 0) g.Hc = L->fused_hc;
        if (RST) g.Hc += g.Hc & 1;
        if (g.Hc > nrows) g.Hc = nrows;
        g.nchunks = (nrows + g.Hc - 1) / g.Hc;
    }
    g.nchl = g.nchunks; g.chunk0 = 0; g.chunk1 = g.nchunks; g.edges = 0;
    if (part) {
        int c0 = 0, c1 = g.nchunks;
        if (v.ext[0]) while (c0 < g.nchunks && g.jbeg + c0 * g.Hc - 2 * K - EY < 0) c0++;
        if (v.ext[1]) while (c1 > c0 && std::min(g.jbeg + c1 * g.Hc, g.jend) - 1 + 2 * K + EY > v.ny - 1) c1--;
        const bool ok = c1 > c0 && c1 - c0 < g.nchunks;
        if (!ok) { if (part == 1) return 1; }
        else if (part == 1) { g.chunk0 = c0; g.chunk1 = c1; g.nchl = c1 - c0; }
        else { g.edges = 1; g.chunk0 = c0; g.chunk1 = c1; g.nchl = g.nchunks - (c1 - c0); }
    }
    g.ntiles = g.nstrips * g.nchl;
    bool selfper = v.per[1] && !(v.ext[0] || v.ext[1]);
    g.wrap_y = selfper;
    g.ylo = v.ext[0] ? g.jbeg - 2 * K - EY : (selfper ? -2 * K - EY : 0);
    g.yhi = v.ext[1] ? g.jend - 1 + 2 * K + EY : (selfper ? v.ny - 1 + 2 * K + EY : v.ny - 1);
    const double *pin = D.fp.f[SUHMO_F_PHI];
    g.pc = g.pco = nullptr; g.Pc = g.gyc = 0;
    if (D.prolong_pending) {
        Depth &C = L->d[depth + 1];
        g.pc = C.fp.f[SUHMO_F_PHI]; g.pco = C.fp.f[SUHMO_F_PHIOLD]; g.Pc = C.v.P; g.gyc = C.v.gy;
        if (part != 1) D.prolong_pending = 0;
    }
    g.negflag = nullptr; g.mask_epoch = 0;
    if (!unmasked && L->skip_mask && L->maskflag_epoch && L->maskflag_epoch == L->mask_epoch && (depth == 0 || L->coarse_mask_ok)
        && (L->desc.nx_global == 0)) {
        g.negflag = suhmo_mask_report_word(L); g.mask_epoch = L->mask_epoch;
    }
    g.rres = g.rphi = nullptr; g.rP = g.rgy = 0;
    if (RST) {
        Depth &C = L->d[depth + 1];
        g.rres = C.fp.f[SUHMO_F_RES]; g.rphi = C.fp.f[SUHMO_F_PHI]; g.rP = C.v.P; g.rgy = C.v.gy;
        C.phi_fresh = 0;
    }
    g.fres = nullptr; g.frhs = g.flphi = g.fphiold = nullptr;
    g.ortrue = nullptr; g.ores = g.olphi = nullptr;
    if (RM == 2) {
        if (v.alpha != 0.0) { suhmo_set_error("internal: residual output on a launch that cannot form it"); return -4; }
        g.ortrue = L->resout_rhs ? L->resout_rhs : D.fp.f[SUHMO_F_RHS];
        g.ores = D.fp.f[SUHMO_F_RES];
        if (L->resout_req & 2) { g.olphi = suhmo_field(L, depth, SUHMO_F_LPHI); if (!g.olphi) return -2; }
        g.onorm = nullptr;
        if ((L->resout_req & 4) && (size_t)g.nstrips * g.nchunks + 4 < L->scratch_elems) { g.onorm = L->scratch + 2; L->resout_np = g.nstrips * g.nchunks; }
        else L->resout_np = 0;
    }
    if (D.rhs_pending) {
        if constexpr (K == 2 && NT == 64 && !RR) {
            if (part || v.alpha != 0.0) { suhmo_set_error("internal: rhs_pending on a launch that cannot form it"); return -4; }
            g.fres = D.fp.f[SUHMO_F_RES]; g.frhs = D.fp.f[SUHMO_F_RHS]; g.flphi = suhmo_field(L, depth, SUHMO_F_LPHI); g.fphiold = suhmo_field(L, depth, SUHMO_F_PHIOLD);
            if (!g.flphi || !g.fphiold) return -2;
            D.rhs_pending = 0; L->frhs_stream++;
            if (unmasked) { hipLaunchKernelGGL((k_gsrb_fused<2, false, 64, 0, true, false>), dim3(g.ntiles), dim3(NT), 0, st, v, D.fp, pin, D.phi_alt, L->ph, g); L->relax_unmasked++; }
            else hipLaunchKernelGGL((k_gsrb_fused<2, false, 64, 0, true>), dim3(g.ntiles), dim3(NT), 0, st, v, D.fp, pin, D.phi_alt, L->ph, g);
            { std::swap(D.fp.f[SUHMO_F_PHI], D.phi_alt); suhmo_fp_changed(); }
            return 0;
        } else { suhmo_set_error("internal: rhs_pending on a launch that cannot form it"); return -4; }
    }
    if (v.alpha != 0.0)
        hipLaunchKernelGGL((k_gsrb_fused<K, true, NT, 0>), dim3(g.ntiles), dim3(NT), 0, st, v, D.fp, pin, D.phi_alt, L->ph, g);
    else if (unmasked) {
        hipLaunchKernelGGL((k_gsrb_fused<K, false, NT, RM, false, false>), dim3(g.ntiles), dim3(NT), 0, st, v, D.fp, pin, D.phi_alt, L->ph, g);
        L->relax_unmasked++;
    } else
        hipLaunchKernelGGL((k_gsrb_fused<K, false, NT, RM>), dim3(g.ntiles), dim3(NT), 0, st, v, D.fp, pin, D.phi_alt, L->ph, g);
    if (part != 1) { std::swap(D.fp.f[SUHMO_F_PHI], D.phi_alt); suhmo_fp_changed(); }
    return 0;
}

struct TileGeom {
    int ntx, nty;
    const double *pc, *pco; int Pc, gyc;
    double *rres, *rphi; int rP, rgy;
    int frhs;
    int jbeg, jend;
    int chunks;
    int order;
};
struct PairCoef { double rhs0, rhs1, B0, B1, Pi0, Pi1, zb0, zb1, a0, a1, byS0, byS1, byN0, byN1, bx0, bx1, bx2; int mneg; };

template <int T, bool RST> struct TileShape { static constexpr int TX = T, TY = (RST && T == 32) ? 28 : T; };
template <int S, int T, bool RST> struct TileThreads { static constexpr int NT = 256; };
template <int S, int T, bool HAS_ALPHA, bool RST = false, bool CHUNKED = false>
__device__ __forceinline__ void d_gsrb_tile(const DV &v, const FP &fp, const double *__restrict__ pin, double *__restrict__ pout,
                                            const suhmo_phys_t &ph, const TileGeom &g)
{
    constexpr int TX = TileShape<T, RST>::TX, TY = TileShape<T, RST>::TY;
    constexpr int HX = 2 * S + (RST ? 2 : 0), HY = 2 * S + (RST ? 1 : 0);
    constexpr int LX = TX + 2 * HX, LY = TY + 2 * HY, NP = LX / 2, NPAIR = NP * LY;
    constexpr int NT = TileThreads<S, T, RST>::NT, NK = (NPAIR + NT - 1) / NT;
    constexpr int PAD = LX + 2;
    __shared__ double lds_raw[LY * LX + 2 * PAD];
    double *const lds = lds_raw + PAD;
    __shared__ double lq[RST ? TY * TX : 1];
    int tl = blockIdx.x;
    if (g.order) {
        const int nt = g.ntx * g.nty, q8 = nt / 8, rem = nt % 8, xcd = tl % 8;
        tl = xcd * q8 + (xcd < rem ? xcd : rem) + tl / 8;
    }
    int tx = tl % g.ntx, ty = tl / g.ntx;
    if (g.order == 2) {
        const int pan = tl / (8 * g.ntx), r = tl - pan * 8 * g.ntx, hp = (g.nty - 8 * pan < 8) ? g.nty - 8 * pan : 8;
        tx = r / hp; ty = 8 * pan + r % hp;
    }
    const int tj0 = g.jbeg + ty * TY;
    const int gx0 = tx * TX - HX, gy0 = tj0 - HY;
    const int t = threadIdx.x;
    const int par = __builtin_amdgcn_readfirstlane((int)(threadIdx.x >> 6)) & 1;
    const int u0 = ((t >> 7) << 6) | (t & 63);
    auto pair_pos = [&](const int k, int &ly, int &lx) -> bool {
        const int u = u0 + (NT / 2) * k, r = u / NP;
        ly = 2 * r + par; lx = 2 * (u - r * NP);
        return ly < LY;
    };
    static_assert(LY % 2 == 0, "rows of the region come in pairs of parities");
    const bool perx = v.per[0] && !v.cfx[0] && !v.cfx[1], pery = v.per[1] && !v.ext[0] && !v.ext[1];
    const bool openW = !perx && gx0 <= (v.cfx[0] ? -1 : 0), openE = !perx && gx0 + LX - 1 >= v.nx - 1 + (v.cfx[1] ? 1 : 0);
    const bool openS = !pery && !v.rk[0] && gy0 <= (v.ext[0] ? -1 : 0), openN = !pery && !v.rk[1] && gy0 + LY - 1 >= v.ny - 1 + (v.ext[1] ? 1 : 0);
    auto wrap = [](int i, int n) { i %= n; return i < 0 ? i + n : i; };
    auto ld2 = [&](const double *__restrict__ p, int idx) { return *reinterpret_cast<const double2 *>(p + idx); };

    PairCoef cf0, cf1, cf2, cf3, cf4;
    bool lv0, lv1, lv2, lv3, lv4;
    static_assert(NK <= 5 && TX * TY / 4 <= NT, "tile too large for the workgroup");
#define TILE_EACH(F) { F(0, cf0, lv0); if constexpr (NK > 1) F(1, cf1, lv1); if constexpr (NK > 2) F(2, cf2, lv2); \
                       if constexpr (NK > 3) F(3, cf3, lv3); if constexpr (NK > 4) F(4, cf4, lv4); }
    bool special = false;
    const bool inner = gx0 >= 0 && gx0 + LX <= v.nx && gy0 >= 0 && gy0 + LY <= v.ny;
    auto ldcoef = [&](PairCoef &c, double2 &p2, const int idx, const int i, const int j) {
        if (g.pc) {
            const int ic = ((j >> 1) + g.gyc) * g.Pc + SUHMO_XOFF + (i >> 1);
            const double corr = 1.0 * g.pc[ic] + (-1.0) * g.pco[ic];
            p2.x = p2.x + corr; p2.y = p2.y + corr;
        }
        double2 d;
        d = ld2(g.frhs ? fp.f[SUHMO_F_RES] : fp.f[SUHMO_F_RHS], idx); c.rhs0 = d.x; c.rhs1 = d.y;
        d = ld2(fp.f[SUHMO_F_B], idx); c.B0 = d.x; c.B1 = d.y;
        d = ld2(fp.f[SUHMO_F_PI], idx); c.Pi0 = d.x; c.Pi1 = d.y;
        d = ld2(fp.f[SUHMO_F_ZB], idx); c.zb0 = d.x; c.zb1 = d.y;
        d = ld2(fp.f[SUHMO_F_MASK], idx); c.mneg = (d.x < 0.0 ? 1 : 0) | (d.y < 0.0 ? 2 : 0);
        if (HAS_ALPHA) { d = ld2(fp.f[SUHMO_F_ACOEF], idx); c.a0 = d.x; c.a1 = d.y; }
        d = ld2(fp.f[SUHMO_F_BY], idx); c.byS0 = d.x; c.byS1 = d.y;
        d = ld2(fp.f[SUHMO_F_BY], idx + v.P); c.byN0 = d.x; c.byN1 = d.y;
        d = ld2(fp.f[SUHMO_F_BX], idx); c.bx0 = d.x; c.bx1 = d.y; c.bx2 = fp.f[SUHMO_F_BX][idx + 2];
        special = special || c.mneg != 0 || ph.cutOffbr > c.B0 || ph.cutOffbr > c.B1 || ph.maxOffbr < c.B0 || ph.maxOffbr < c.B1;
    };
    auto load = [&](const int k, PairCoef &c, bool &live) {
        live = false;
        int ly, lx;
        if (pair_pos(k, ly, lx)) {
            int i = gx0 + lx, j = gy0 + ly;
            if (inner) {
                live = true;
                const int idx = cidx(v, i, j);
                double2 p2 = ld2(pin, idx);
                ldcoef(c, p2, idx, i, j);
                lds[ly * LX + lx] = p2.x; lds[ly * LX + lx + 1] = p2.y;
                return;
            }
            const bool inx = perx || (i >= 0 && i < v.nx), iny = pery || (j >= 0 && j < v.ny) || (j < 0 && v.rk[0] && j >= g.jbeg - HY) || (j >= v.ny && v.rk[1]
                && j < g.jend + HY);
            const bool exi = inx || (i == -2 && v.cfx[0]) || (i == v.nx && v.cfx[1]);
            const bool exj = iny || (j == -1 && v.ext[0] && !v.rk[0]) || (j == v.ny && v.ext[1] && !v.rk[1]);
            double2 p2 = make_double2(0.0, 0.0);
            if (exi && exj) {
                live = inx && iny;
                if (perx) i = wrap(i, v.nx);
                if (pery) j = wrap(j, v.ny);
                const int idx = cidx(v, i, j);
                p2 = ld2(pin, idx);
            }
            if (live) ldcoef(c, p2, cidx(v, i, j), i, j);
            lds[ly * LX + lx] = p2.x; lds[ly * LX + lx + 1] = p2.y;
        }
    };
    TILE_EACH(load);
    constexpr bool PLAIN_OK = !HAS_ALPHA && !RST && !CHUNKED;
    const bool plain = PLAIN_OK && !__syncthreads_or(special ? 1 : 0) && ph.use_NL && !openW && !openE && !openS && !openN
                       && !v.cfx[0] && !v.cfx[1] && !(v.ext[0] && !v.rk[0]) && !(v.ext[1] && !v.rk[1]);
    if constexpr (!PLAIN_OK) __syncthreads();

    if (g.frhs) {
        const int ylo = openS ? 0 : 1, yhi = openN ? LY - 1 : LY - 2;
        auto mkrhs = [&](const int k, PairCoef &q_, const bool live) {
            int ly, lx;
            if (pair_pos(k, ly, lx) && live) {
                const int i = gx0 + lx, j = gy0 + ly;
                if (ly >= ylo && ly <= yhi) {
                    const double *row = lds + ly * LX;
                    double lo[2], cc[2];
#pragma unroll
                    for (int a = 0; a < 2; a++) {
                        const int x = lx + a, ii = i + a;
                        double c = row[x];
                        double w = row[x > 0 ? x - 1 : 0], e = row[x < LX - 1 ? x + 1 : LX - 1];
                        double s_ = lds[(ly > 0 ? ly - 1 : 0) * LX + x], n = lds[(ly < LY - 1 ? ly + 1 : LY - 1) * LX + x];
                        if (!perx) {
                            if (ii == 0 && !v.cfx[0]) w = (v.bct[0][0] == 0) ? v.two_v[0][0] - c : c + v.neu[0][0];
// ... 191 lines not shown
                acc = acc + q0[0]; accp = accp + p0[0] / 4.0;
                acc = acc + q0[1]; accp = accp + p0[1] / 4.0;
                acc = acc + q0[TX]; accp = accp + p0[LX] / 4.0;
                acc = acc + q0[TX + 1]; accp = accp + p0[LX + 1] / 4.0;
                const int ic = ((j >> 1) + g.rgy) * g.rP + SUHMO_XOFF + (i >> 1);
                g.rres[ic] = acc; g.rphi[ic] = accp;
            }
        }
    }
}
#define TILE_KERNEL_ATTRS(S, T, RST) __launch_bounds__((TileThreads<S, T, RST>::NT)) __attribute__((amdgpu_waves_per_eu((TileThreads<S, T, RST>::NT == 384 ? 3 : 2))))
template <int S, int T, bool HAS_ALPHA, bool RST = false, bool CHUNKED = false>
__global__ TILE_KERNEL_ATTRS(S, T, RST) void k_gsrb_tile(DV v, FP fp, const double *__restrict__ pin, double *__restrict__ pout, suhmo_phys_t ph, TileGeom g)
{
    d_gsrb_tile<S, T, HAS_ALPHA, RST, CHUNKED>(v, fp, pin, pout, ph, g);
}
template <int S, int T, bool HAS_ALPHA, bool CHUNKED>
__global__ TILE_KERNEL_ATTRS(S, T, false) void k_gsrb_tile_b(BatchTab t, BatchTab c, BatchSel sel, TileGeom g, int prolong)
{
    const int k = batch_member(sel);
    const DV v = t.dv[k];
    const FP fp = batch_fp(t, k);
    const suhmo_phys_t ph = t.ph[k];
    if (prolong) { const FP fc = batch_fp(c, k); g.pc = fc.f[SUHMO_F_PHI]; g.pco = fc.f[SUHMO_F_PHIOLD]; }
    d_gsrb_tile<S, T, HAS_ALPHA, false, CHUNKED>(v, fp, fp.f[SUHMO_F_PHI], fp.f[SUHMO_F_PHI2], ph, g);
}
static bool tile_ok(const suhmo_level *L, const Depth &D)
{
    const DV &v = D.v;
    if (!L->gsrb_tile || !suhmo_batch_tile_ok(v)) return false;
    if ((v.rk[0] || v.rk[1]) && (!L->ex || !L->tile_strips || L->desc.nx_global > 0 || v.gy < 10 || v.ny < 10)) return false;
    return true;
}
bool suhmo_batch_tile_ok(const DV &v)
{
    if (v.nx & 1) return false;
    if (v.per[1] && (v.ny & 1)) return false;
    if ((v.per[0] && v.cfx[0] != v.cfx[1]) || (v.per[1] && v.ext[0] != v.ext[1])) return false;
    return true;
}

template <int S, int T, bool RST = false>
static int launch_tile(suhmo_level *L, int depth, int chunks, int ext_rows, hipStream_t st)
{
    Depth &D = L->d[depth];
    const DV &v = D.v;
    if (!D.phi_alt) {
        HIPCHK(hipMalloc(&D.phi_alt, D.elems * sizeof(double)));
        HIPCHK(hipMemsetAsync(D.phi_alt, 0, D.elems * sizeof(double), st));
    }
    TileGeom g;
    constexpr int TX = TileShape<T, RST>::TX, TY = TileShape<T, RST>::TY;
    g.jbeg = v.rk[0] ? -ext_rows : 0; g.jend = v.ny + (v.rk[1] ? ext_rows : 0);
    g.ntx = (v.nx + TX - 1) / TX; g.nty = (g.jend - g.jbeg + TY - 1) / TY;
    g.pc = g.pco = nullptr; g.Pc = g.gyc = 0;
    g.rres = g.rphi = nullptr; g.rP = g.rgy = 0;
    if (RST) {
        Depth &C = L->d[depth + 1];
        g.rres = C.fp.f[SUHMO_F_RES]; g.rphi = C.fp.f[SUHMO_F_PHI]; g.rP = C.v.P; g.rgy = C.v.gy;
        C.phi_fresh = 0;
    }
    if (D.prolong_pending) {
        Depth &C = L->d[depth + 1];
        g.pc = C.fp.f[SUHMO_F_PHI]; g.pco = C.fp.f[SUHMO_F_PHIOLD]; g.Pc = C.v.P; g.gyc = C.v.gy;
        D.prolong_pending = 0;
    }
    g.chunks = chunks;
    g.order = L->tile_order;
    g.frhs = 0;
    if (D.rhs_pending) {
        if (!suhmo_field(L, depth, SUHMO_F_LPHI) || !suhmo_field(L, depth, SUHMO_F_PHIOLD)) return -2;
        g.frhs = 1; D.rhs_pending = 0; L->frhs_tile++;
    }
    const double *pin = D.fp.f[SUHMO_F_PHI];
    if constexpr (S == 4) {
        if (chunks > 1) {
            if (v.alpha != 0.0)
                hipLaunchKernelGGL((k_gsrb_tile<S, T, true, RST, true>), dim3(g.ntx * g.nty), dim3(TileThreads<S, T, RST>::NT), 0, st, v, D.fp, pin, D.phi_alt, L->ph, g);
            else
                hipLaunchKernelGGL((k_gsrb_tile<S, T, false, RST, true>), dim3(g.ntx * g.nty), dim3(TileThreads<S, T, RST>::NT), 0, st, v, D.fp, pin, D.phi_alt, L->ph, g);
            { std::swap(D.fp.f[SUHMO_F_PHI], D.phi_alt); suhmo_fp_changed(); }
            return 0;
        }
    }
    if (chunks > 1) { suhmo_set_error("internal: chunked tile launch with S != 4"); return -4; }
    if (v.alpha != 0.0)
        hipLaunchKernelGGL((k_gsrb_tile<S, T, true, RST>), dim3(g.ntx * g.nty), dim3(TileThreads<S, T, RST>::NT), 0, st, v, D.fp, pin, D.phi_alt, L->ph, g);
    else
        hipLaunchKernelGGL((k_gsrb_tile<S, T, false, RST>), dim3(g.ntx * g.nty), dim3(TileThreads<S, T, RST>::NT), 0, st, v, D.fp, pin, D.phi_alt, L->ph, g);
    { std::swap(D.fp.f[SUHMO_F_PHI], D.phi_alt); suhmo_fp_changed(); }
    return 0;
}
static int tile_edge(const suhmo_level *L, const DV &v)
{
    if (L->tile_t) return L->tile_t;
    return ((long)v.nx * v.ny >= 600000L) ? 32 : 16;
}
static int single_tile_of(int tile_t, const DV &v)
{
    if (tile_t != 32 && v.nx <= 16 && v.ny <= 16) return 16;
    if (tile_t != 16 && v.nx <= 32 && v.ny <= 28) return 32;
    return 0;
}
static int single_tile(const suhmo_level *L, const DV &v) { return single_tile_of(L->tile_t, v); }
int suhmo_batch_single_tile(const DV &v) { return single_tile_of(0, v); }
static int launch_tile_any(suhmo_level *L, int depth, int S, int chunks, bool rst, int ext_rows, hipStream_t st)
{
    const int T = chunks > 1 ? single_tile(L, L->d[depth].v) : tile_edge(L, L->d[depth].v);
    if (rst) {
        if (T == 32) return S == 4 ? launch_tile<4, 32, true>(L, depth, chunks, ext_rows, st) : S == 2 ? launch_tile<2, 32, true>(L, depth, chunks, ext_rows,
            st) : launch_tile<1, 32, true>(L, depth, chunks, ext_rows, st);
        return S == 4 ? launch_tile<4, 16, true>(L, depth, chunks, ext_rows, st) : S == 2 ? launch_tile<2, 16, true>(L, depth, chunks, ext_rows, st) : launch_tile<1,
            16, true>(L, depth, chunks, ext_rows, st);
    }
    if (T == 32) return S == 4 ? launch_tile<4, 32>(L, depth, chunks, ext_rows, st) : S == 2 ? launch_tile<2, 32>(L, depth, chunks, ext_rows, st) : launch_tile<1, 32>(L, depth, chunks, ext_rows, st);
    return S == 4 ? launch_tile<4, 16>(L, depth, chunks, ext_rows, st) : S == 2 ? launch_tile<2, 16>(L, depth, chunks, ext_rows, st) : launch_tile<1, 16>(L, depth, chunks, ext_rows, st);
}

static int pick_variant(const suhmo_level *L, const Depth &D)
{
    int variant = L->gsrb_variant;
    if (variant < 0) {
        const long cells = (long)D.v.nx * D.v.ny;
        variant = (cells >= (long)L->fused_min_cells) ? 2 : 0;
        if (tile_ok(L, D) && cells < L->tile_max_cells) variant = 0;
    }
    return variant;
}
static int pick_K(const suhmo_level *L, const Depth &D, int variant, int remaining)
{
    if (variant >= 2 && remaining >= 2 && fused_ok(L, D, 2)) return 2;
    if (variant >= 1 && fused_ok(L, D, 1)) return 1;
    return 0;
}
static int prolong_halo_rows(const suhmo_level *L, int depth)
{
    const Depth &D = L->d[depth], &C = L->d[depth + 1];
    int R = D.phi_fresh < 2 * C.phi_fresh ? D.phi_fresh : 2 * C.phi_fresh;
    return R & ~1;
}
bool suhmo_gsrb_can_fuse_rhs(suhmo_level *L, int depth, int sweeps, bool rhs_local)
{
    Depth &D = L->d[depth];
    if (sweeps < 1 || !L->fas_rhs_in_relax) return false;
    const bool strip = D.v.rk[0] || D.v.rk[1];
    const int K = pick_K(L, D, pick_variant(L, D), sweeps);
    if (K <= 0) return !strip && (L->fas_rhs_in_relax & 1) && tile_ok(L, D);
    if (!(L->fas_rhs_in_relax & 2)) return false;
    const int nt = L->fused_nt ? L->fused_nt : ((long)D.v.nx * D.v.ny >= 8000000L ? 256 : 64);
    if (!(K == 2 && nt == 64 && sweeps >= 4 && D.v.alpha == 0.0)) return false;
    if (!(D.v.ext[0] || D.v.ext[1])) return true;
    return strip && L->ex && rhs_local && L->desc.nx_global == 0 && D.phi_fresh >= D.v.gy && D.v.gy >= 2 * K + 1 && D.v.ny >= D.v.gy;
}
bool suhmo_gsrb_can_fuse_prolong(suhmo_level *L, int depth, int sweeps)
{
    Depth &D = L->d[depth];
    if (sweeps < 1 || depth + 1 >= L->ndepth) return false;
    int K = pick_K(L, D, pick_variant(L, D), sweeps);
    if (K <= 0) {
        if (!tile_ok(L, D)) return false;
        if (!(D.v.rk[0] || D.v.rk[1])) return true;
        const int TS = sweeps >= 4 && L->tile_s >= 4 ? 4 : sweeps >= 2 && L->tile_s >= 2 ? 2 : 1;
        return prolong_halo_rows(L, depth) >= 2 * TS;
    }
    const bool ext = L->ex && (D.v.ext[0] || D.v.ext[1]);
    if ((D.v.ext[0] || D.v.ext[1]) && !ext) return false;
    return !ext || prolong_halo_rows(L, depth) >= 2 * K;
}

int suhmo_launch_gsrb(suhmo_level *L, int depth, int sweeps, int tail, hipStream_t st, int *restricted)
{
    Depth &D = L->d[depth];
    int variant = pick_variant(L, D);
    const bool ext = L->ex && (D.v.ext[0] || D.v.ext[1]);
    if (restricted) *restricted = 0;
    const bool may_restrict = restricted && L->fused_restrict && depth + 1 < L->ndepth && !(D.v.ny & 1) && !(D.v.j0 & 1)
                              && (!(D.v.ext[0] || D.v.ext[1]) || (ext && L->desc.nx_global == 0 && D.v.gy >= 5))
                              && D.v.alpha == 0.0;
    int F = ext ? D.phi_fresh : 0;
    if (ext && D.prolong_pending) F = prolong_halo_rows(L, depth);
    int it = 0;
    while (it < sweeps) {
        int K = pick_K(L, D, variant, sweeps - it);
        int TS = (K == 0 && tile_ok(L, D)) ? (sweeps - it >= 4 && L->tile_s >= 4 ? 4 : sweeps - it >= 2 && L->tile_s >= 2 ? 2 : 1) : 0;
        int tE = 0;
        bool trst = TS && restricted && L->fused_restrict && (L->tile_restrict == 1 || (L->tile_restrict == 2 && ext)) && depth + 1 < L->ndepth && !(D.v.ny & 1) && !(D.v.j0 & 1);
        if (TS && ext) {
            trst = trst && it + TS == sweeps;
            const int need = 2 * TS + (trst ? 1 : 0);
            if (F < need && !D.prolong_pending) {
                int rc = suhmo_ensure_phi_halo(L, depth, need, st); if (rc) return rc;
                F = D.phi_fresh;
            }
            if (F < need) {
                if (D.prolong_pending) { suhmo_set_error("internal: fused prolongation with a shallow halo"); return -4; }
                TS = 0;
            } else {
                const int want = 2 * (sweeps - it - TS) + tail;
                tE = F - need < want ? F - need : want;
                if (tE > D.v.gy - need - 1) tE = D.v.gy - need - 1;
                tE = tE < 0 ? 0 : tE & ~1;
            }
        }
        if (K == 0 && !TS && D.prolong_pending) { suhmo_set_error("internal: prolong_pending without a fused relax"); return -4; }
        ProfEv pe{};
        bool prof = L->prof_on && depth == 0;
        if (prof) {
            HIPCHK(hipEventCreate(&pe.a)); HIPCHK(hipEventCreate(&pe.b));
            HIPCHK(hipEventRecord(pe.a, st));
        }
        int tchunks = 1;
        if (TS) {
            if (L->tile_chunks && !ext && TS == 4 && single_tile(L, D.v)) tchunks = (sweeps - it) / TS;
            const bool rst = trst && it + TS * tchunks == sweeps;
            int rc = launch_tile_any(L, depth, TS, tchunks, rst, tE, st); if (rc) return rc;
            if (rst) *restricted = 1;
            if (ext) { F = tE; D.phi_fresh = tE; }
        } else if (K == 0) {
            for (int pass = 0; pass < 2; pass++) {
                if (ext && F < 1) {
                    int rc = suhmo_ensure_phi_halo(L, depth, 1, st); if (rc) return rc;
                    F = D.phi_fresh;
                }
                int want = 2 * (sweeps - it) - (pass + 1) + tail;
                int E = ext ? (F - 1 < want ? F - 1 : want) : 0;
                if (L->desc.nx_global > 0) E = 0;
                { int rc2 = launch_simple(L, depth, pass, E, st); if (rc2) return rc2; }
                if (ext) { F = E; D.phi_fresh = F; }
            }
        } else {
            const int nt = L->fused_nt ? L->fused_nt : ((long)D.v.nx * D.v.ny >= 8000000L ? 256 : 64);
            bool rst = may_restrict && nt == 64 && K == 2 && it + K == sweeps;
            bool rout = L->resout_armed && depth == 0 && !restricted && nt == 64 && K == 2 && it + K == sweeps && D.v.alpha == 0.0
                        && (!(D.v.ext[0] || D.v.ext[1]) || ext) && L->desc.nx_global == 0 && !D.rhs_pending;
            const int need = 2 * K + ((rst || rout) && ext ? 1 : 0);
            bool flying = false;
            if (ext && F < need) {
                if ((L->overlap_halo == 2 || (L->overlap_halo && (L->rccl || L->ipc))) && !D.prolong_pending && D.v.ny >= 6 * need) {
                    if (!L->xstream) {
                        HIPCHK(hipStreamCreateWithFlags(&L->xstream, hipStreamNonBlocking));
                        HIPCHK(hipEventCreateWithFlags(&L->xev[0], hipEventDisableTiming)); HIPCHK(hipEventCreateWithFlags(&L->xev[1], hipEventDisableTiming));
                    }
                    HIPCHK(hipEventRecord(L->xev[0], st));
                    HIPCHK(hipStreamWaitEvent(L->xstream, L->xev[0], 0));
                    int rc2 = suhmo_ensure_phi_halo(L, depth, need, L->xstream); if (rc2) return rc2;
                    HIPCHK(hipEventRecord(L->xev[1], L->xstream));
                    flying = true;
                } else { int rc2 = suhmo_ensure_phi_halo(L, depth, need, st); if (rc2) return rc2; }
                F = D.phi_fresh;
                if (F < 2 * K) { suhmo_set_error("internal: halo shallower than 2K"); return -4; }
            }
            int want = 2 * (sweeps - it - K) + tail;
            if (D.rhs_pending && ext) want = F;
            int E = ext ? (F - 2 * K < want ? F - 2 * K : want) : 0;
            int rc = 0;
            if ((rst || rout) && ext) {
                if (F < 2 * K + 1) rst = rout = false;
                else { E = F - 2 * K - 1 < want ? F - 2 * K - 1 : want; if (rst) E &= ~1; }
            }
            auto launch = [&](int part) {
                if (rout) return launch_fused<2, 64, 2>(L, depth, E, st, part);
                if (rst) return launch_fused<2, 64, 1>(L, depth, E, st, part);
                if (nt == 64) return (K == 2) ? launch_fused<2, 64>(L, depth, E, st, part) : launch_fused<1, 64>(L, depth, E, st, part);
                return (K == 2) ? launch_fused<2, 256>(L, depth, E, st, part) : launch_fused<1, 256>(L, depth, E, st, part);
            };
            if (flying) {
                rc = launch(1);
                if (rc < 0) return rc;
                HIPCHK(hipStreamWaitEvent(st, L->xev[1], 0));
                if (rc == 1) rc = launch(0); else { rc = launch(2); L->overlapped++; }
            } else rc = launch(0);
            if (rc) return rc;
            if (rst) *restricted = 1;
            if (rout) { L->resout_done = 1; L->resout_count++; }
            if (ext) { F = E; D.phi_fresh = F; }
        }
        int done = TS ? TS * tchunks : K == 0 ? 1 : K;
        if (prof) {
            HIPCHK(hipEventRecord(pe.b, st));
            pe.cells = (long)D.v.nx * D.v.ny * done;
            pe.restricts = (restricted && *restricted && it + done == sweeps) ? 1 : 0;
            L->prof.push_back(pe);
        }
        it += done;
    }
    HIPCHK(hipGetLastError());
    return 0;
}

template <int S, int T, bool CHUNKED>
static void launch_tile_b(const BatchTab &t, const BatchTab &c, const BatchSel &sel, const TileGeom &g, bool has_alpha, int prolong, hipStream_t st)
{
    const dim3 grd(g.ntx * g.nty, 1, sel.n), blk(TileThreads<S, T, false>::NT);
    if (has_alpha) hipLaunchKernelGGL((k_gsrb_tile_b<S, T, true, CHUNKED>), grd, blk, 0, st, t, c, sel, g, prolong);
    else hipLaunchKernelGGL((k_gsrb_tile_b<S, T, false, CHUNKED>), grd, blk, 0, st, t, c, sel, g, prolong);
}
int suhmo_batch_gsrb_tile(const BatchTab &t, const BatchTab *coarse, const DV *vc, const BatchSel &sel, const DV &v, int S, int T, int chunks, bool frhs, bool prolong,
                          bool has_alpha, int order, hipStream_t st)
{
    if (sel.n <= 0) return 0;
    TileGeom g;
    g.jbeg = 0; g.jend = v.ny;
    g.ntx = (v.nx + T - 1) / T; g.nty = (v.ny + T - 1) / T;
    g.pc = g.pco = nullptr; g.Pc = g.gyc = 0;
    g.rres = g.rphi = nullptr; g.rP = g.rgy = 0;
    if (prolong) {
        if (!coarse || !vc) { suhmo_set_error("internal: fused prolongation without the coarse tables"); return -4; }
        g.Pc = vc->P; g.gyc = vc->gy;
    }
    g.chunks = chunks; g.order = order; g.frhs = frhs ? 1 : 0;
    BatchTab c = coarse ? *coarse : t;
    if (chunks > 1) {
        if (S != 4 || g.ntx * g.nty != 1) { suhmo_set_error("internal: chunked tile launch of a batch"); return -4; }
        if (T == 32) launch_tile_b<4, 32, true>(t, c, sel, g, has_alpha, prolong, st); else launch_tile_b<4, 16, true>(t, c, sel, g, has_alpha, prolong, st);
    } else if (T == 32) {
        if (S == 4) launch_tile_b<4, 32, false>(t, c, sel, g, has_alpha, prolong, st);
        else if (S == 2) launch_tile_b<2, 32, false>(t, c, sel, g, has_alpha, prolong, st);
        else launch_tile_b<1, 32, false>(t, c, sel, g, has_alpha, prolong, st);
    } else {
        if (S == 4) launch_tile_b<4, 16, false>(t, c, sel, g, has_alpha, prolong, st);
        else if (S == 2) launch_tile_b<2, 16, false>(t, c, sel, g, has_alpha, prolong, st);
        else launch_tile_b<1, 16, false>(t, c, sel, g, has_alpha, prolong, st);
    }
    HIPCHK(hipGetLastError());
    return 0;
}
```

suhmo_amd/csrc/suhmo_level.hip:

```cpp
#include "suhmo_hier.h"
#include "suhmo_level_int.h"
#include <algorithm>
#include <cstdarg>
#include <cmath>
#include <initializer_list>

static thread_local char g_err[512] = "";
void suhmo_set_error(const char *fmt, ...)
{
    va_list ap; va_start(ap, fmt); vsnprintf(g_err, sizeof(g_err), fmt, ap); va_end(ap);
}
extern "C" const char *suhmo_last_error(void) { return g_err; }
#include <atomic>
#include <chrono>
#include <map>
#include <mutex>
namespace {
std::atomic<int> g_timer_mode{-1};
std::mutex g_timer_mu;
struct TimerRec { long count = 0; double total = 0.0; };
std::map<std::string, TimerRec> g_timers;
inline double now_s() { return std::chrono::duration<double>(std::chrono::steady_clock::now().time_since_epoch()).count(); }
inline int timer_mode()
{
    int m = g_timer_mode.load(std::memory_order_relaxed);
    if (m < 0) { const char *e = getenv("SUHMO_TIMERS"); m = e ? atoi(e) : 0; g_timer_mode.store(m); }
    return m;
}
}
SuhmoTimer::SuhmoTimer(const char *n) : name(n), t0(0.0), mode(timer_mode())
{
    if (!mode) return;
    if (mode >= 2) (void)hipDeviceSynchronize();
    t0 = now_s();
}
SuhmoTimer::~SuhmoTimer()
{
    if (!mode) return;
    if (mode >= 2) (void)hipDeviceSynchronize();
    double dt = now_s() - t0;
    std::lock_guard<std::mutex> lk(g_timer_mu);
    TimerRec &r = g_timers[name];
    r.count++; r.total += dt;
}
extern "C" int suhmo_timers_enable(int mode) { g_timer_mode.store(mode < 0 ? 0 : mode); return 0; }
extern "C" int suhmo_timers_reset(void) { std::lock_guard<std::mutex> lk(g_timer_mu); g_timers.clear(); return 0; }
extern "C" long suhmo_timers_report(char *buf, long size)
{
    std::vector<std::pair<std::string, TimerRec>> v;
    { std::lock_guard<std::mutex> lk(g_timer_mu); v.assign(g_timers.begin(), g_timers.end()); }
    std::sort(v.begin(), v.end(), [](const auto &a, const auto &b) { return a.second.total > b.second.total; });
    std::string out;
    char line[256];
    for (auto &e : v) {
        snprintf(line, sizeof(line), "%-56s %10ld %14.6f %12.2f\n", e.first.c_str(), e.second.count, e.second.total, 1e6 * e.second.total / std::max(1L, e.second.count));
        out += line;
    }
    if (buf && size > 0) { long n = std::min<long>(size - 1, (long)out.size()); memcpy(buf, out.data(), n); buf[n] = 0; }
    return (long)out.size() + 1;
}

extern "C" int suhmo_device_count(void)
{
    int n = 0;
    if (hipGetDeviceCount(&n) != hipSuccess) return 0;
    return n;
}

static bool boxes_coarsenable(const std::vector<int> &b, int r)
{
    for (size_t k = 0; k < b.size(); k += 4)
        if (b[k] % r || b[k + 1] % r || (b[k + 2] + 1) % r || (b[k + 3] + 1) % r) return false;
    return true;
}

static void make_dv(DV &v, const suhmo_level_desc_t &d, int depth)
{
    int c = 1 << depth;
    memset(&v, 0, sizeof(v));
    v.nx = d.nx / c; v.ny = d.ny / c;
    v.gy = d.halo_rows < 1 ? 1 : d.halo_rows;
    v.rows = v.ny + 2 * v.gy;
    v.P = ((v.nx + 2 * SUHMO_XOFF + 15) / 16) * 16;
    v.j0 = d.j0 / c; v.nyg = d.ny_global / c;
    v.i0 = d.i0 / c; v.nxg = (d.nx_global > 0 ? d.nx_global : d.nx) / c;
    v.dx = d.dx * c; v.dy = d.dy * c;
    v.rdx = 1.0 / (v.dx * v.dx); v.rdy = 1.0 / (v.dy * v.dy);
    v.fdx = 1.0 / v.dx; v.fdy = 1.0 / v.dy;
    v.alpha = d.alpha; v.beta = d.beta;
    for (int dir = 0; dir < 2; dir++) {
        v.per[dir] = d.bc.periodic[dir];
        for (int s = 0; s < 2; s++) {
            v.bct[dir][s] = d.bc.type[dir][s];
            v.two_v[dir][s] = 2.0 * d.bc.value[dir][s];
            double isign = s == 0 ? -1.0 : 1.0;
            v.neu[dir][s] = isign * (dir == 0 ? v.dx : v.dy) * d.bc.value[dir][s];
        }
    }
    bool whole = (d.j0 == 0 && d.ny == d.ny_global);
    v.ext[0] = (!whole) && (d.j0 > 0 || d.bc.periodic[1]);
    v.ext[1] = (!whole) && (d.j0 + d.ny < d.ny_global || d.bc.periodic[1]);
    v.cfx[0] = v.i0 > 0 || (v.per[0] && v.nx < v.nxg);
    v.cfx[1] = v.i0 + v.nx < v.nxg || (v.per[0] && v.nx < v.nxg);
    if (d.nx_global > 0) {
        const int pj0 = d.patch_ny > 0 ? d.patch_j0 : d.j0, pj1 = d.patch_ny > 0 ? d.patch_j0 + d.patch_ny : d.j0 + d.ny;
        v.rk[0] = d.j0 > pj0; v.rk[1] = d.j0 + d.ny < pj1;
    } else { v.rk[0] = v.ext[0]; v.rk[1] = v.ext[1]; }
}

static std::atomic<unsigned long> g_fp_epoch{1};
void suhmo_fp_changed() { g_fp_epoch.fetch_add(1, std::memory_order_relaxed); }
unsigned long suhmo_fp_epoch() { return g_fp_epoch.load(std::memory_order_relaxed); }

double *suhmo_field(suhmo_level *L, int depth, int field)
{
    Depth &D = L->d[depth];
    if (!D.fp.f[field]) {
        double *p = nullptr;
        if (L->stub) return nullptr;
        if (hipMalloc(&p, D.elems * sizeof(double)) != hipSuccess) return nullptr;
        (void)hipMemset(p, 0, D.elems * sizeof(double));
        D.fp.f[field] = p;
        suhmo_fp_changed();
    }
    return D.fp.f[field];
}

static int level_storage(suhmo_level *L);
int suhmo_level_create_(suhmo_level_t **out, const suhmo_level_desc_t *desc, bool stub);
extern "C" int suhmo_level_create(suhmo_level_t **out, const suhmo_level_desc_t *desc) { return suhmo_level_create_(out, desc, false); }
int suhmo_level_materialize_(suhmo_level *L) { return L->stub ? level_storage(L) : 0; }
int suhmo_level_create_(suhmo_level_t **out, const suhmo_level_desc_t *desc, bool stub)
{
    ARG(out && desc);
    ARG(desc->nx >= 2 && desc->ny >= 2 && desc->dx > 0 && desc->dy > 0);
    ARG(desc->ny_global >= desc->ny && desc->j0 >= 0 && desc->j0 + desc->ny <= desc->ny_global);
    ARG(desc->i0 >= 0 && (desc->nx_global == 0 ? desc->i0 == 0 : desc->i0 + desc->nx <= desc->nx_global));
    ARG(desc->i0 % 2 == 0);
    ARG(desc->patch_ny == 0 || (desc->nx_global > 0 && desc->patch_j0 <= desc->j0 && desc->j0 + desc->ny <= desc->patch_j0 + desc->patch_ny));
    ARG((long)(desc->nx + 64) * (long)(desc->ny + 2 * (desc->halo_rows < 1 ? 1 : desc->halo_rows)) < (1L << 31));
    int ndev = 0;
    HIPCHK(hipGetDeviceCount(&ndev));
    if (ndev <= 0) { suhmo_set_error("no HIP device: the product path has no CPU fallback"); return -3; }
    ARG(desc->device >= 0 && desc->device < ndev);
    HIPCHK(hipSetDevice(desc->device));
    suhmo_level *L = new suhmo_level();
    L->desc = *desc; L->ph = desc->phys; L->device = desc->device; L->batch_owned = 0;
    L->ex = nullptr; L->ar = nullptr; L->ar2 = nullptr; L->ard = nullptr; L->user = nullptr; L->ex_begin = nullptr; L->ex_end = nullptr; L->rccl = nullptr;
        L->ipc = nullptr; L->ipc_owner = 0; L->faces_deferred = 0; L->gap = nullptr; L->gap_dt = 0.0; L->prof_on = 0; L->gsrb_variant = -1; L->fused_hc = 0;
    L->bcoef_fused = 1;
    L->bcoef_tile_x = 62;
    L->fused_nt = 64;
    L->fused_restrict = 1;
    L->gsrb_tile = 1; L->tile_t = 0; L->tile_s = 4;
    L->tile_max_cells = 3000000;
    L->fas_rhs_in_relax = 3;
    L->tile_chunks = 1;
    L->tile_order = 2; L->tile_restrict = 0;
    L->tile_strips = 1;
    L->overlap_halo = 1; L->xstream = nullptr; L->xev[0] = L->xev[1] = nullptr; L->overlapped = 0;
    L->strips_rhs_local = 1;
    L->fas_rhs_fused = 1;
    L->agg_min_cells = 100000; L->agg_depth = 0; L->agg_world = 1; L->agg_rank = 0; L->agg = nullptr; L->ag = nullptr; L->ag_user = nullptr;
    L->agg_send = L->agg_recv = nullptr; L->agg_cap = 0; L->agg_gathers = 0; L->agg_static_stale = 0;
    L->frhs_stream = L->frhs_tile = 0;
    L->resout_np = 0;
    L->resout_req = L->resout_armed = L->resout_done = 0; L->resout_rhs = nullptr; L->resout_count = 0; L->resid_in_relax = 1;
    L->graph_max_cells = 1500000; L->gstream = nullptr; L->vgraph_replays = 0; memset(L->vgraph_seen, 0, sizeof(L->vgraph_seen));
    L->fused_min_cells = 1000000;
    L->skip_mask = 1; L->mask_known = 1; L->poll_readback = 1;
    L->bottom_solver = 0; L->bottom_one_launch_max_cells = 16384;
    L->bottom_ctr = nullptr; L->bottom_host_iters = L->bottom_host_solves = 0;
    {
        struct IntKnob { const char *env; int suhmo_level::*field; };
        struct LongKnob { const char *env; long suhmo_level::*field; };
        static const IntKnob ints[] = {
            {"SUHMO_GSRB_VARIANT", &suhmo_level::gsrb_variant}, {"SUHMO_FUSED_HC", &suhmo_level::fused_hc}, {"SUHMO_BCOEF_FUSED", &suhmo_level::bcoef_fused},
            {"SUHMO_BCOEF_TILE_X", &suhmo_level::bcoef_tile_x}, {"SUHMO_FUSED_NT", &suhmo_level::fused_nt}, {"SUHMO_OVERLAP_HALO", &suhmo_level::overlap_halo},
            {"SUHMO_STRIPS_RHS_LOCAL", &suhmo_level::strips_rhs_local}, {"SUHMO_FAS_RHS_FUSED", &suhmo_level::fas_rhs_fused},
            {"SUHMO_RESID_IN_RELAX", &suhmo_level::resid_in_relax}, {"SUHMO_TILE_STRIPS", &suhmo_level::tile_strips}, {"SUHMO_TILE_CHUNKS", &suhmo_level::tile_chunks},
            {"SUHMO_TILE_RESTRICT", &suhmo_level::tile_restrict}, {"SUHMO_TILE_ORDER", &suhmo_level::tile_order}, {"SUHMO_FAS_RHS_IN_RELAX", &suhmo_level::fas_rhs_in_relax},
            {"SUHMO_TILE_S", &suhmo_level::tile_s}, {"SUHMO_GSRB_TILE", &suhmo_level::gsrb_tile}, {"SUHMO_TILE_T", &suhmo_level::tile_t},
            {"SUHMO_FUSED_RESTRICT", &suhmo_level::fused_restrict}, {"SUHMO_SKIP_MASK", &suhmo_level::skip_mask}, {"SUHMO_MASK_KNOWN", &suhmo_level::mask_known},
            {"SUHMO_POLL_READBACK", &suhmo_level::poll_readback}};
        static const LongKnob longs[] = {
            {"SUHMO_AGG_MIN_CELLS", &suhmo_level::agg_min_cells}, {"SUHMO_TILE_MAX_CELLS", &suhmo_level::tile_max_cells},
            {"SUHMO_GRAPH_MAX_CELLS", &suhmo_level::graph_max_cells}, {"SUHMO_FUSED_MIN_CELLS", &suhmo_level::fused_min_cells},
            {"SUHMO_BOTTOM_ONE_LAUNCH_MAX_CELLS", &suhmo_level::bottom_one_launch_max_cells}};
        for (const IntKnob &k : ints) if (const char *e = getenv(k.env)) L->*(k.field) = atoi(e);
        for (const LongKnob &k : longs) if (const char *e = getenv(k.env)) L->*(k.field) = atol(e);
        L->fas_rhs_fused = L->fas_rhs_fused != 0;
        if (L->tile_order < 0 || L->tile_order > 2) L->tile_order = 0;
        if (L->tile_t != 16 && L->tile_t != 32) L->tile_t = 0;
    }
    if (desc->boxes && desc->nbox > 0) {
        L->boxes.assign(desc->boxes, desc->boxes + 4 * (size_t)desc->nbox);
    } else {
        int mb = desc->max_box > 0 ? desc->max_box : 64;
        for (int bj = 0; bj * mb < desc->ny; bj++)
            for (int bi = 0; bi * mb < desc->nx; bi++) {
                int lo0 = desc->i0 + bi * mb, lo1 = desc->j0 + bj * mb;
                int hi0 = std::min(lo0 + mb, desc->i0 + desc->nx) - 1, hi1 = std::min(lo1 + mb, desc->j0 + desc->ny) - 1;
                int b[4] = {lo0, lo1, hi0, hi1};
                L->boxes.insert(L->boxes.end(), b, b + 4);
            }
    }
    L->desc.boxes = nullptr;
    L->desc.nbox = (int)(L->boxes.size() / 4);
    {
        long cells = 0;
        for (size_t k = 0; k < L->boxes.size(); k += 4) {
            const int *b = &L->boxes[k];
            if (b[0] < desc->i0 || b[2] >= desc->i0 + desc->nx || b[1] < desc->j0 || b[3] >= desc->j0 + desc->ny || b[0] > b[2] || b[1] > b[3]) {
                suhmo_set_error("box %zu outside the strip", k / 4); delete L; return -1;
            }
            cells += (long)(b[2] - b[0] + 1) * (b[3] - b[1] + 1);
        }
        if (cells != (long)desc->nx * desc->ny) { suhmo_set_error("boxes do not tile the level"); delete L; return -1; }
    }
    L->ndepth = 1;
    for (int dep = 1; dep < SUHMO_MAXDEPTH; dep++) {
        if (!boxes_coarsenable(L->boxes, (1 << dep) * 2)) break;
        if ((desc->j0 % (1 << dep)) || (desc->ny_global % (1 << dep))) break;
        if ((desc->i0 % (2 << dep)) || (desc->nx_global % (1 << dep))) break;
        L->ndepth = dep + 1;
    }
    for (int dep = 0; dep < L->ndepth; dep++) {
        Depth &D = L->d[dep];
        make_dv(D.v, L->desc, dep);
        D.elems = (size_t)D.v.P * (size_t)(D.v.rows + 1);
        D.nbox = L->desc.nbox;
        memset(&D.fp, 0, sizeof(D.fp));
        D.phi_alt = nullptr; D.prolong_pending = 0; D.rhs_pending = 0; D.phi_fresh = 0;
    }
    L->scratch = nullptr; L->scratch_elems = 0; L->hscratch = nullptr; L->hscratch_dev = nullptr; L->hseq = 0;
    L->mask_epoch = 0; L->maskflag_epoch = 0; L->mask_reported = 0; L->coarse_mask_ok = 0;
    L->mask_state = SUHMO_MASK_UNKNOWN; L->mask_version = 1; L->mask_scan_version = 0; L->mask_scan_pending = 0; L->mask_capturing = 0;
    L->mask_scan_captured = 0; L->mask_view = 0; L->mask_scan_errors = 0;
    L->mask_host = nullptr; L->mask_ev = nullptr; L->mask_scans = L->bcoef_unmasked = L->relax_unmasked = 0;
    L->stub = 1;
    if (!stub) { int rc = level_storage(L); if (rc) { suhmo_level_destroy(L); return rc; } }
    *out = L;
    return 0;
}
static int level_storage(suhmo_level *L)
{
    static const int eager[] = {SUHMO_F_PHI, SUHMO_F_RHS, SUHMO_F_ACOEF, SUHMO_F_B, SUHMO_F_PI, SUHMO_F_ZB,
                                SUHMO_F_MASK, SUHMO_F_BX, SUHMO_F_BY, SUHMO_F_RES, SUHMO_F_LPHI};
    HIPCHK(hipSetDevice(L->device));
    L->stub = 0;
    for (int dep = 0; dep < L->ndepth; dep++) {
        for (int f : eager) {
            if (dep == 0 && f == SUHMO_F_LPHI) continue;
            if (!suhmo_field(L, dep, f)) { suhmo_set_error("hipMalloc failed (depth %d field %d)", dep, f); return -2; }
        }
        if (dep > 0) { suhmo_field(L, dep, SUHMO_F_PHIOLD); suhmo_field(L, dep, SUHMO_F_CORR); }
    }
    L->scratch_elems = 16384;
    HIPCHK(hipMalloc(&L->scratch, L->scratch_elems * sizeof(double)));
    HIPCHK(hipMemset(L->scratch, 0, L->scratch_elems * sizeof(double)));
    HIPCHK(hipHostMalloc(&L->hscratch, SUHMO_HSCRATCH_DOUBLES * sizeof(double), hipHostMallocMapped | hipHostMallocCoherent));
    memset(L->hscratch, 0, SUHMO_HSCRATCH_DOUBLES * sizeof(double));
    L->mask_host = (unsigned *)(L->hscratch + SUHMO_HSCRATCH_MASK);
    if (L->poll_readback && hipHostGetDevicePointer((void **)&L->hscratch_dev, L->hscratch, 0) != hipSuccess) { L->hscratch_dev = nullptr; L->poll_readback = 0; (void)hipGetLastError(); }
    return 0;
}

extern "C" int suhmo_level_destroy(suhmo_level_t *L)
{
    if (!L) return 0;
    if (L->batch_owned) { suhmo_set_error("this level is a member of a batch: suhmo_batch_destroy frees it"); return -1; }
    (void)hipSetDevice(L->device);
    (void)hipDeviceSynchronize();
    if (L->rccl) (void)suhmo_level_detach_rccl(L);
    if (L->gap) { (void)suhmo_level_destroy(L->gap); L->gap = nullptr; }
    suhmo_ipc_release(L);
    suhmo_agg_release(L);
    suhmo_level_drop_graphs(L);
    for (int dep = 0; dep < L->ndepth; dep++)
        for (int f = 0; f < SUHMO_F_COUNT; f++)
            if (L->d[dep].fp.f[f]) (void)hipFree(L->d[dep].fp.f[f]);
    for (int dep = 0; dep < L->ndepth; dep++)
        if (L->d[dep].phi_alt) (void)hipFree(L->d[dep].phi_alt);
    for (auto &pe : L->prof) { (void)hipEventDestroy(pe.a); (void)hipEventDestroy(pe.b); }
    if (L->xstream) { (void)hipStreamDestroy(L->xstream); (void)hipEventDestroy(L->xev[0]); (void)hipEventDestroy(L->xev[1]); }
    if (L->scratch) (void)hipFree(L->scratch);
    if (L->bottom_ctr) (void)hipFree(L->bottom_ctr);
    if (L->mask_ev) (void)hipEventDestroy(L->mask_ev);
    if (L->hscratch) (void)hipHostFree(L->hscratch);
    delete L;
    return 0;
}

static int remake_views(suhmo_level *L)
{
    for (int dep = 0; dep < L->ndepth; dep++) make_dv(L->d[dep].v, L->desc, dep);
    suhmo_level_drop_graphs(L);
    return 0;
}
extern "C" int suhmo_level_set_alpha_beta(suhmo_level_t *L, double alpha, double beta)
{
    ARG(L);
    L->desc.alpha = alpha; L->desc.beta = beta;
    if (L->agg) { int rc = suhmo_level_set_alpha_beta(L->agg, alpha, beta); if (rc) return rc; }
    return remake_views(L);
}
extern "C" int suhmo_level_set_bc(suhmo_level_t *L, const suhmo_bc_t *bc)
{
    ARG(L && bc);
    for (int d = 0; d < 2; d++)
        if ((bc->periodic[d] != 0) != (L->desc.bc.periodic[d] != 0)) { suhmo_set_error("setBC cannot change the periodicity of the domain"); return -1; }
    for (int d = 0; d < 2; d++) for (int s = 0; s < 2; s++) ARG(bc->type[d][s] == 0 || bc->type[d][s] == 1);
    L->desc.bc = *bc;
    if (L->agg) { int rc = suhmo_level_set_bc(L->agg, bc); if (rc) return rc; }
    return remake_views(L);
}

static long *option_slot_long(suhmo_level *L, const char *key)
{
    if (!strcmp(key, "fused_min_cells")) return &L->fused_min_cells;
    if (!strcmp(key, "tile_max_cells")) return &L->tile_max_cells;
    if (!strcmp(key, "graph_max_cells")) return &L->graph_max_cells;
    if (!strcmp(key, "agg_min_cells")) return &L->agg_min_cells;
    return nullptr;
}
static int *option_slot_int(suhmo_level *L, const char *key)
{
    static const struct { const char *k; int suhmo_level::*m; } tab[] = {
        {"gsrb_variant", &suhmo_level::gsrb_variant}, {"fused_hc", &suhmo_level::fused_hc}, {"bcoef_fused", &suhmo_level::bcoef_fused}, {"bcoef_tile_x", &suhmo_level::bcoef_tile_x},
        {"fused_nt", &suhmo_level::fused_nt}, {"fused_restrict", &suhmo_level::fused_restrict}, {"strips_rhs_local", &suhmo_level::strips_rhs_local},
        {"tile_strips", &suhmo_level::tile_strips}, {"overlap_halo", &suhmo_level::overlap_halo}, {"skip_mask", &suhmo_level::skip_mask}, {"mask_known", &suhmo_level::mask_known}, {"tile_chunks",
            &suhmo_level::tile_chunks}, {"tile_order", &suhmo_level::tile_order}, {"tile_restrict", &suhmo_level::tile_restrict}, {"fas_rhs_in_relax",
            &suhmo_level::fas_rhs_in_relax}, {"resid_in_relax", &suhmo_level::resid_in_relax}, {"fas_rhs_fused", &suhmo_level::fas_rhs_fused},
        {"tile_s", &suhmo_level::tile_s}, {"gsrb_tile", &suhmo_level::gsrb_tile}, {"tile_t", &suhmo_level::tile_t}, {"poll_readback", &suhmo_level::poll_readback}};
    for (const auto &e : tab) if (!strcmp(key, e.k)) return &(L->*(e.m));
    return nullptr;
}
extern "C" int suhmo_level_set_option(suhmo_level_t *L, const char *key, long value)
{
    ARG(L && key);
    if (!strcmp(key, "bottom_solver")) {
        if (value != 0 && value != 1) { suhmo_set_error("bottom_solver: 0 (bottom relaxes only) or 1 (RelaxSolver)"); return -1; }
        return suhmo_bottom_configure(L, (int)value, L->bottom_one_launch_max_cells);
    }
    if (!strcmp(key, "bottom_one_launch_max_cells")) {
        if (value < 0) { suhmo_set_error("bottom_one_launch_max_cells: >= 0"); return -1; }
        return suhmo_bottom_configure(L, L->bottom_solver, value);
    }
    if (long *p = option_slot_long(L, key)) {
        *p = value; suhmo_level_drop_graphs(L);
        if (!strcmp(key, "agg_min_cells")) return suhmo_agg_setup(L);
        return 0;
    }
    if (int *p = option_slot_int(L, key)) {
        if (!strcmp(key, "tile_t") && value != 0 && value != 16 && value != 32) { suhmo_set_error("tile_t: 0 (by size), 16 or 32"); return -1; }
        if (!strcmp(key, "fused_nt") && value != 64 && value != 256) { suhmo_set_error("fused_nt: 64 or 256"); return -1; }
        if (!strcmp(key, "poll_readback") && value && !L->hscratch_dev) { suhmo_set_error("poll_readback: no device address of the host slot"); return -1; }
        *p = (int)value; suhmo_level_drop_graphs(L); return 0;
    }
    suhmo_set_error("unknown option '%s'", key);
    return -1;
}
extern "C" int suhmo_level_get_option(const suhmo_level_t *L, const char *key, long *value)
{
    ARG(L && key && value);
    if (long *p = option_slot_long(const_cast<suhmo_level *>(L), key)) { *value = *p; return 0; }
    if (int *p = option_slot_int(const_cast<suhmo_level *>(L), key)) { *value = *p; return 0; }
    if (!strcmp(key, "overlapped_launches")) { *value = L->overlapped; return 0; }
    if (!strcmp(key, "agg_gathers")) { *value = L->agg_gathers; return 0; }
    if (!strcmp(key, "rhs_in_streaming_launches")) { *value = L->frhs_stream; return 0; }
    if (!strcmp(key, "rhs_in_tile_launches")) { *value = L->frhs_tile; return 0; }
    if (!strcmp(key, "residual_in_relax_launches")) { *value = L->resout_count; return 0; }
    if (!strcmp(key, "mask_scans")) { *value = L->mask_scans; return 0; }
    if (!strcmp(key, "mask_state")) { *value = L->mask_state; return 0; }
    if (!strcmp(key, "bcoef_unmasked_launches")) { *value = L->bcoef_unmasked; return 0; }
    if (!strcmp(key, "relax_unmasked_launches")) { *value = L->relax_unmasked; return 0; }
    if (!strcmp(key, "vcycle_graph_replays")) { *value = L->vgraph_replays; return 0; }
    if (!strcmp(key, "bottom_solver")) { *value = L->bottom_solver; return 0; }
    if (!strcmp(key, "bottom_one_launch_max_cells")) { *value = L->bottom_one_launch_max_cells; return 0; }
    if (!strcmp(key, "bottom_solver_iterations")) { *value = suhmo_bottom_counter(L, 0); return 0; }
    if (!strcmp(key, "bottom_solves_one_launch")) { *value = suhmo_bottom_counter(L, 1); return 0; }
    if (!strcmp(key, "bottom_solves_host_loop")) { *value = suhmo_bottom_counter(L, 2); return 0; }
    suhmo_set_error("unknown option '%s'", key);
    return -1;
}

extern "C" int suhmo_level_num_depths(const suhmo_level_t *L) { return L ? L->ndepth : -1; }
extern "C" int suhmo_level_synchronize(suhmo_level_t *L, suhmo_stream_t s)
{
    ARG(L);
    HIPCHK(hipStreamSynchronize((hipStream_t)s));
    return 0;
}
extern "C" int suhmo_level_set_hooks(suhmo_level_t *L, suhmo_exchange_fn ex, suhmo_allreduce_max_fn ar, void *user)
{
    ARG(L);
    L->ex = ex; L->ar = ar; L->ar2 = nullptr; L->ard = nullptr; L->user = user; L->ex_begin = nullptr; L->ex_end = nullptr;
    return 0;
}
void suhmo_level_share_transport(suhmo_level *dst, const suhmo_level *src)
{
    dst->ex = src->ex; dst->ar = src->ar; dst->ar2 = src->ar2; dst->ard = src->ard; dst->user = src->user;
    dst->ex_begin = src->ex_begin; dst->ex_end = src->ex_end; dst->ipc = src->ipc;
}
extern "C" int suhmo_level_set_allgather(suhmo_level_t *L, suhmo_allgather_fn fn, void *user)
{
    ARG(L);
    HIPCHK(hipSetDevice(L->device));
    L->ag = fn; L->ag_user = user;
    return suhmo_agg_setup(L);
}
extern "C" int suhmo_level_agglomerated_depth(const suhmo_level_t *L) { return L ? L->agg_depth : -1; }
extern "C" int suhmo_level_set_reduce_hook(suhmo_level_t *L, suhmo_allreduce_fn fn)
{
    ARG(L);
    L->ar2 = fn;
    return 0;
}

extern "C" int suhmo_level_exchange(suhmo_level_t *L, int depth, int field, suhmo_stream_t s)
{
    ARG(L); ARG(depth >= 0 && depth < L->ndepth); ARG(field >= 0 && field < SUHMO_F_COUNT);
    const DV &v = L->d[depth].v;
    if (L->ex && (v.ext[0] || v.ext[1])) {
        if (!suhmo_field(L, depth, field)) return -2;
        int rc = L->ex(L->user, L, depth, &field, 1, s);
        if (!rc && field == SUHMO_F_PHI) L->d[depth].phi_fresh = suhmo_halo_rows(v);
        if (field == SUHMO_F_MASK) suhmo_mask_halo_written(L);
        return rc;
    }
    return 0;
}
extern "C" int suhmo_level_halo_info(const suhmo_level_t *L, int depth, int *halo_rows, int *ext_lo, int *ext_hi, int *nx, int *ny)
{
    ARG(L); ARG(depth >= 0 && depth < L->ndepth);
    const DV &v = L->d[depth].v;
    if (halo_rows) *halo_rows = v.gy;
    if (ext_lo) *ext_lo = v.ext[0];
    if (ext_hi) *ext_hi = v.ext[1];
    if (nx) *nx = v.nx;
    if (ny) *ny = v.ny;
    return 0;
}


extern "C" int suhmo_level_field_view(suhmo_level_t *L, int depth, int field, double **base, long *pitch, long *origin)
{
    CHECK_DF(L, depth, field);
    double *p = suhmo_field(L, depth, field);
    if (!p) { suhmo_set_error("field allocation failed"); return -2; }
    if (field == SUHMO_F_MASK) { L->mask_view = 1; suhmo_mask_written(L); suhmo_level_drop_graphs(L); }
    if (base) *base = p;
    if (pitch) *pitch = L->d[depth].v.P;
    if (origin) *origin = cidx(L->d[depth].v, 0, 0);
    return 0;
}

static int copy2d(suhmo_level *L, int depth, int field, double *host, long hpitch, int i0, int j0, int ni, int nj,
                  bool to_canvas, bool on_device, hipStream_t st)
{
    if (ni <= 0 || nj <= 0) return 0;
    double *p = suhmo_field(L, depth, field);
    if (!p) { suhmo_set_error("field allocation failed"); return -2; }
    const DV &v = L->d[depth].v;
    double *c = p + cidx(v, i0, j0);
    hipMemcpyKind kind = to_canvas ? (on_device ? hipMemcpyDeviceToDevice : hipMemcpyHostToDevice)
                                   : (on_device ? hipMemcpyDeviceToDevice : hipMemcpyDeviceToHost);
    if (to_canvas)
        HIPCHK(hipMemcpy2DAsync(c, (size_t)v.P * 8, host, (size_t)hpitch * 8, (size_t)ni * 8, nj, kind, st));
    else
        HIPCHK(hipMemcpy2DAsync(host, (size_t)hpitch * 8, c, (size_t)v.P * 8, (size_t)ni * 8, nj, kind, st));
    return 0;
}

static int field_io(suhmo_level *L, int depth, int field, double *buf, int ghosted, int on_device, bool set, hipStream_t st)
{
    const DV &v = L->d[depth].v;
    int rc;
    if (is_xface(field)) rc = copy2d(L, depth, field, buf, v.nx + 1, 0, 0, v.nx + 1, v.ny, set, on_device, st);
    else if (is_yface(field)) rc = copy2d(L, depth, field, buf, v.nx, 0, 0, v.nx, v.ny + 1, set, on_device, st);
    else if (ghosted) rc = copy2d(L, depth, field, buf, v.nx + 2, -1, -1, v.nx + 2, v.ny + 2, set, on_device, st);
    else rc = copy2d(L, depth, field, buf, v.nx, 0, 0, v.nx, v.ny, set, on_device, st);
    if (rc) return rc;
    if (!on_device) HIPCHK(hipStreamSynchronize(st));
    return 0;
}

extern "C" int suhmo_level_set_field(suhmo_level_t *L, int depth, int field, const double *src, int ghosted,
                                     int on_device, suhmo_stream_t s)
{
    CHECK_DF(L, depth, field); ARG(src);
    HIPCHK(hipSetDevice(L->device));
    if (field == SUHMO_F_PHI) phi_changed(L, depth);
    if (field == SUHMO_F_MASK) suhmo_mask_written(L);
    return field_io(L, depth, field, (double *)src, ghosted, on_device, true, (hipStream_t)s);
}
extern "C" int suhmo_level_get_field(suhmo_level_t *L, int depth, int field, double *dst, int ghosted,
                                     int on_device, suhmo_stream_t s)
{
    CHECK_DF(L, depth, field); ARG(dst);
    HIPCHK(hipSetDevice(L->device));
    return field_io(L, depth, field, dst, ghosted, on_device, false, (hipStream_t)s);
}

static void box_region(const suhmo_level *L, int depth, int field, int ibox, int r[4])
{
    const int *b = &L->boxes[4 * (size_t)ibox];
    int c = 1 << depth;
    r[0] = b[0] / c - L->d[depth].v.i0; r[1] = b[1] / c - L->d[depth].v.j0;
    r[2] = (b[2] + 1) / c - 1 - L->d[depth].v.i0; r[3] = (b[3] + 1) / c - 1 - L->d[depth].v.j0;
    if (is_xface(field)) r[2] += 1;
    if (is_yface(field)) r[3] += 1;
}

extern "C" int suhmo_level_put_box(suhmo_level_t *L, int depth, int field, int ibox, const double *fab,
                                   int flo0, int flo1, int fhi0, int fhi1, int with_domain_ghosts, suhmo_stream_t s)
{
    CHECK_DF(L, depth, field); ARG(fab); ARG(ibox >= 0 && ibox < L->desc.nbox);
    HIPCHK(hipSetDevice(L->device));
    hipStream_t st = (hipStream_t)s;
    const DV &v = L->d[depth].v;
    if (field == SUHMO_F_PHI) phi_changed(L, depth);
    if (field == SUHMO_F_MASK) suhmo_mask_written(L);
    int r[4]; box_region(L, depth, field, ibox, r);
    int j0 = v.j0;
// ... 115 lines not shown
```

Measured before the change: 497.2 V-cycles/s.

## Form face coefficients inside the first fused GSRB relaxation launch

When coefficients are computed on the fly, the separate gradient, Re and face-coefficient kernels at the finest depth are replaced by a BCF variant of the fused two-sweep GSRB kernel. That variant builds the face coefficients from phi and B in shared memory while it relaxes, using a wider halo and one extra lagged row. The averaging to coarser depths then runs right after that launch. Shared helper functions are moved into the common header, and graph caching and capture are keyed on the new mode. The aim is to drop a separate full-grid pass that writes BX/BY and reads them back. The cost is extra recomputation and halo work inside the relax kernel. The path is narrowly gated: clean mask, alpha = 0, 64-thread blocks, K = 2.

```diff
diff --git a/suhmo_amd/csrc/suhmo_bcoef.hip b/suhmo_amd/csrc/suhmo_bcoef.hip
--- a/suhmo_amd/csrc/suhmo_bcoef.hip
+++ b/suhmo_amd/csrc/suhmo_bcoef.hip
@@ -12,17 +12,16 @@
     double c = phi[idx];
     double e = phiE(v, phi, idx, i, c, false), w = phiW(v, phi, idx, i, c, false);
     double n = phiN(v, phi, idx, j, c, false), s = phiS(v, phi, idx, j, c, false);
-    double gW = v.fdx * (c - w), gE = v.fdx * (e - c), gS = v.fdy * (c - s), gN = v.fdy * (n - c);
+    bool zW = false, zE = false, zS = false, zN = false;
     if (hasMask) {
         const double *__restrict__ m = fp.f[SUHMO_F_MASK];
         bool mc = m[idx] < 1e-6;
-        if (mc || m[idx - 1] < 1e-6) gW = 0.0;
-        if (mc || m[idx + 1] < 1e-6) gE = 0.0;
-        if (mc || m[idx - v.P] < 1e-6) gS = 0.0;
-        if (mc || m[idx + v.P] < 1e-6) gN = 0.0;
-    }
-    gx = 0.5 * (gW + gE);
-    gy = 0.5 * (gS + gN);
+        zW = mc || m[idx - 1] < 1e-6;
+        zE = mc || m[idx + 1] < 1e-6;
+        zS = mc || m[idx - v.P] < 1e-6;
+        zN = mc || m[idx + v.P] < 1e-6;
+    }
+    gradcc_from(v, c, w, e, s, n, zW, zE, zS, zN, gx, gy);
 }
 __device__ __forceinline__ void d_gradcc_at(const DV &v, const FP &fp, int hasMask, int i, int j)
 {
@@ -116,9 +115,7 @@
 __device__ __forceinline__ double d_re_val(const FP &fp, const suhmo_phys_t &ph, int idx)
 {
     double gx = fp.f[SUHMO_F_GRADX][idx], gy = fp.f[SUHMO_F_GRADY][idx], B = fp.f[SUHMO_F_B][idx];
-    double sg = sqrt(gx * gx + gy * gy);
-    double discr = 1.0 + 4.0 * ph.omega * (B * B * B * ph.grav * sg) / (12.0 * ph.nu * ph.nu);
-    return (-1.0 + sqrt(discr)) / (2.0 * ph.omega);
+    return re_from(ph, grad_norm(gx, gy), B);
 }
 __device__ __forceinline__ void d_re(const DV &v, const FP &fp, suhmo_phys_t ph)
 {
@@ -130,18 +127,6 @@
     fp.f[SUHMO_F_RE][idx] = d_re_val(fp, ph, idx);
 }
 template <class T> __global__ __launch_bounds__(256) void k_re(T t) { d_re(t.view(), t.fields(), t.phys()); }
-__device__ __forceinline__ double bcoef_face(const suhmo_phys_t &ph, double Rc, double Rm, double Bc, double Bm,
-                                             double mc, double mm, bool dom_edge)
-{
-    double Ref = 0.5 * (Rc + Rm), Bf = 0.5 * (Bc + Bm);
-    double mec;
-    if (fabs(mc - mm) < 1e-10) mec = (mc > 0.0) ? 1.0 : -1.0; else mec = 0.0;
-    if (dom_edge) mec = 0.0;
-    double num_q = -(Bf * Bf * Bf * ph.grav);
-    double denom_q = 12.0 * ph.nu * (1.0 + ph.omega * Ref);
-    if (mec < 0.0 && ph.cutOffB > 0) return 0.0;
-    return num_q / denom_q;
-}
 __device__ __forceinline__ void d_bcoef_faces(const DV &v, const FP &fp, suhmo_phys_t ph)
 {
     int i = blockIdx.x * blockDim.x + threadIdx.x, j = blockIdx.y * blockDim.y + threadIdx.y;
@@ -243,16 +228,16 @@
     __syncthreads();
     auto gradcc = [&](int p, int gi, int gj, double &gx, double &gy) {
         double c = sphi[p], w = sphi[p - 1], e = sphi[p + 1], s = sphi[p - PW], n = sphi[p + PW];
-        double gW = v.fdx * (c - w), gE = v.fdx * (e - c), gS = v.fdy * (c - s), gN = v.fdy * (n - c);
+        bool zW = false, zE = false, zS = false, zN = false;
         if (hasMask) {
             int idx = cidx(v, wrapx(gi), wrapy(gj));
             bool mc = mk[idx] < 1e-6;
-            if (mc || mk[idx - 1] < 1e-6) gW = 0.0;
-            if (mc || mk[idx + 1] < 1e-6) gE = 0.0;
-            if (mc || mk[idx - v.P] < 1e-6) gS = 0.0;
-            if (mc || mk[idx + v.P] < 1e-6) gN = 0.0;
-        }
-        gx = 0.5 * (gW + gE); gy = 0.5 * (gS + gN);
+            zW = mc || mk[idx - 1] < 1e-6;
+            zE = mc || mk[idx + 1] < 1e-6;
+            zS = mc || mk[idx - v.P] < 1e-6;
+            zN = mc || mk[idx + v.P] < 1e-6;
+        }
+        gradcc_from(v, c, w, e, s, n, zW, zE, zS, zN, gx, gy);
     };
     double rer[NK];
 #pragma unroll
@@ -276,10 +261,7 @@
         }
         double re = 0.0;
         if (hasB[k]) {
-            double B = Br[k];
-            double sg = sqrt(gx * gx + gy * gy);
-            double discr = 1.0 + 4.0 * ph.omega * (B * B * B * ph.grav * sg) / (12.0 * ph.nu * ph.nu);
-            re = (-1.0 + sqrt(discr)) / (2.0 * ph.omega);
+            re = re_from(ph, grad_norm(gx, gy), Br[k]);
         }
         rer[k] = re;
     }
diff --git a/suhmo_amd/csrc/suhmo_common.h b/suhmo_amd/csrc/suhmo_common.h
--- a/suhmo_amd/csrc/suhmo_common.h
+++ b/suhmo_amd/csrc/suhmo_common.h
@@ -103,6 +103,36 @@
     return lam;
 }
 
+__device__ __forceinline__ void gradcc_from(const DV &v, double c, double w, double e, double s, double n, bool zW, bool zE, bool zS,
+                                            bool zN, double &gx, double &gy)
+{
+    double gW = v.fdx * (c - w), gE = v.fdx * (e - c), gS = v.fdy * (c - s), gN = v.fdy * (n - c);
+    if (zW) gW = 0.0;
+    if (zE) gE = 0.0;
+    if (zS) gS = 0.0;
+    if (zN) gN = 0.0;
+    gx = 0.5 * (gW + gE);
+    gy = 0.5 * (gS + gN);
+}
+__device__ __forceinline__ double grad_norm(double gx, double gy) { return sqrt(gx * gx + gy * gy); }
+__device__ __forceinline__ double re_from(const suhmo_phys_t &ph, double sg, double B)
+{
+    double discr = 1.0 + 4.0 * ph.omega * (B * B * B * ph.grav * sg) / (12.0 * ph.nu * ph.nu);
+    return (-1.0 + sqrt(discr)) / (2.0 * ph.omega);
+}
+__device__ __forceinline__ double bcoef_face(const suhmo_phys_t &ph, double Rc, double Rm, double Bc, double Bm,
+                                             double mc, double mm, bool dom_edge)
+{
+    double Ref = 0.5 * (Rc + Rm), Bf = 0.5 * (Bc + Bm);
+    double mec;
+    if (fabs(mc - mm) < 1e-10) mec = (mc > 0.0) ? 1.0 : -1.0; else mec = 0.0;
+    if (dom_edge) mec = 0.0;
+    double num_q = -(Bf * Bf * Bf * ph.grav);
+    double denom_q = 12.0 * ph.nu * (1.0 + ph.omega * Ref);
+    if (mec < 0.0 && ph.cutOffB > 0) return 0.0;
+    return num_q / denom_q;
+}
+
 struct Depth {
     DV v;
     FP fp;
@@ -110,6 +140,7 @@
     int nbox;
     int prolong_pending;
     int rhs_pending;
+    int bcoef_pending;
     double *phi_alt;
     int phi_fresh;
 };
@@ -120,6 +151,7 @@
     double *p1[SUHMO_MAXDEPTH], *a1[SUHMO_MAXDEPTH];
     double *rhs;
     int rout_req, rout_done, rout_np; const double *rout_rhs;
+    int bcoef_in_relax; long n_bcoef_in_relax;
     int mask_clean; long n_bcoef_unmasked, n_relax_unmasked;
     int has_scan;
 };
@@ -162,6 +194,7 @@
     double *agg_send, *agg_recv; size_t agg_cap; long agg_gathers;
     int resout_req, resout_armed, resout_done; const double *resout_rhs; long resout_count;
     int resout_np;
+    int bcoef_in_relax, bcoef_nd; long bcoef_in_relax_count;
     long frhs_stream, frhs_tile;
     int prof_on;
     std::vector<ProfEv> prof;
@@ -245,6 +278,7 @@
 int suhmo_level_residual_and_norm(suhmo_level *L, double *out, hipStream_t st);
 int suhmo_level_norm_from_partials(suhmo_level *L, int np, double *out, hipStream_t st);
 bool suhmo_gsrb_can_fuse_rhs(suhmo_level *L, int depth, int sweeps, bool rhs_local = false);
+bool suhmo_gsrb_can_fuse_bcoef(suhmo_level *L, int sweeps);
 int suhmo_launch_gsrb(suhmo_level *L, int depth, int sweeps, int tail, hipStream_t st, int *restricted = nullptr);
 void suhmo_level_drop_graphs(suhmo_level *L);
 int suhmo_ensure_phi_halo(suhmo_level *L, int depth, int need, hipStream_t st);
diff --git a/suhmo_amd/csrc/suhmo_fas.hip b/suhmo_amd/csrc/suhmo_fas.hip
--- a/suhmo_amd/csrc/suhmo_fas.hip
+++ b/suhmo_amd/csrc/suhmo_fas.hip
@@ -84,7 +84,10 @@
 static int vcycle_body(suhmo_level *L, const suhmo_solver_params_t *sp, int nd, suhmo_stream_t s)
 {
     int rc;
-    if (sp->bcoeff_otf) {
+    if (sp->bcoeff_otf && nd > 1 && suhmo_gsrb_can_fuse_bcoef(L, sp->num_smooth)) {
+        L->d[0].bcoef_pending = 1; L->bcoef_nd = nd;
+        L->maskflag_epoch = 0; L->mask_reported = 0;
+    } else if (sp->bcoeff_otf) {
         L->faces_deferred = 1;
         rc = suhmo_level_update_operator(L, 0, s);
         if (rc) { L->faces_deferred = 0; return rc; }
@@ -92,6 +95,10 @@
         if ((rc = suhmo_average_operator_all(L, nd, (hipStream_t)s))) return rc;
     } else L->maskflag_epoch = 0;
     rc = fas_cycle(L, 0, sp, nd, s);
+    if (L->d[0].bcoef_pending) {
+        L->d[0].bcoef_pending = 0;
+        if (!rc) { suhmo_set_error("internal: no relaxation launch formed the face coefficients"); rc = -4; }
+    }
     L->maskflag_epoch = 0;
     return rc;
 }
@@ -110,6 +117,7 @@
     const int key[4] = {sp->num_smooth, sp->num_bottom, sp->bcoeff_otf, nd};
     const int mask_clean = (suhmo_mask_clean(L, 0) ? 1 : 0) | (L->ndepth > 1 && suhmo_mask_clean(L, 1) ? 2 : 0);
     const bool scanning = sp->bcoeff_otf && suhmo_mask_would_scan(L);
+    const int bcoef_in_relax = L->bcoef_in_relax != 0;
     auto launch = [&](const VGraph &g) {
         int rc = 0;
         if (scanning && (rc = suhmo_mask_scan_begin(L, (hipStream_t)s))) return rc;
@@ -118,11 +126,11 @@
         return 0;
     };
     auto replayed = [&](const VGraph &g) {
-        L->bcoef_unmasked += g.n_bcoef_unmasked; L->relax_unmasked += g.n_relax_unmasked;
+        L->bcoef_unmasked += g.n_bcoef_unmasked; L->relax_unmasked += g.n_relax_unmasked; L->bcoef_in_relax_count += g.n_bcoef_in_relax;
         if (g.rout_done) { L->resout_done = 1; L->resout_count++; L->resout_np = g.rout_np; }
     };
     auto at_start = [&](const VGraph &g) {
-        if (memcmp(g.key, key, sizeof(key)) || g.mask_clean != mask_clean) return false;
+        if (memcmp(g.key, key, sizeof(key)) || g.mask_clean != mask_clean || g.bcoef_in_relax != bcoef_in_relax) return false;
         for (int d = 0; d < L->ndepth; d++) if (L->d[d].fp.f[SUHMO_F_PHI] != g.p0[d] || L->d[d].phi_alt != g.a0[d]) return false;
         if (g.rout_req != (L->resid_in_relax ? L->resout_req : 0) || g.rout_rhs != L->resout_rhs) return false;
         return L->d[0].fp.f[SUHMO_F_RHS] == g.rhs;
@@ -139,13 +147,13 @@
     for (int k = 0; k < 4; k++) if (L->vgraph_seen[k] != key[k]) { memcpy(L->vgraph_seen, key, sizeof(key)); return 0; }
     if (L->vgraphs.size() >= 16) return 0;
     if (!L->gstream) HIPCHK(hipStreamCreateWithFlags(&L->gstream, hipStreamNonBlocking));
-    VGraph g; memcpy(g.key, key, sizeof(key)); g.exec = nullptr; g.mask_clean = mask_clean; g.has_scan = 0;
+    VGraph g; memcpy(g.key, key, sizeof(key)); g.exec = nullptr; g.mask_clean = mask_clean; g.has_scan = 0; g.bcoef_in_relax = bcoef_in_relax;
     for (int d = 0; d < SUHMO_MAXDEPTH; d++) { g.p0[d] = g.a0[d] = g.p1[d] = g.a1[d] = nullptr; }
     for (int d = 0; d < L->ndepth; d++) { g.p0[d] = L->d[d].fp.f[SUHMO_F_PHI]; g.a0[d] = L->d[d].phi_alt; }
     g.rhs = L->d[0].fp.f[SUHMO_F_RHS];
     g.rout_req = L->resid_in_relax ? L->resout_req : 0; g.rout_rhs = L->resout_rhs; g.rout_done = 0;
     const int rout_before = L->resout_done; const long rout_count = L->resout_count;
-    const long bcoef_unmasked = L->bcoef_unmasked, relax_unmasked = L->relax_unmasked;
+    const long bcoef_unmasked = L->bcoef_unmasked, relax_unmasked = L->relax_unmasked, bcoef_in_relax_count = L->bcoef_in_relax_count;
     HIPCHK(hipStreamSynchronize((hipStream_t)s));
     hipGraph_t graph = nullptr;
     hipError_t e = hipStreamBeginCapture(L->gstream, hipStreamCaptureModeThreadLocal);
@@ -157,15 +165,16 @@
         e = hipStreamEndCapture(L->gstream, &graph);
     }
     g.n_bcoef_unmasked = L->bcoef_unmasked - bcoef_unmasked; g.n_relax_unmasked = L->relax_unmasked - relax_unmasked;
+    g.n_bcoef_in_relax = L->bcoef_in_relax_count - bcoef_in_relax_count; L->bcoef_in_relax_count = bcoef_in_relax_count;
     L->bcoef_unmasked = bcoef_unmasked; L->relax_unmasked = relax_unmasked;
     g.rout_done = L->resout_count != rout_count;
     g.rout_np = L->resout_np;
     L->resout_done = rout_before; L->resout_count = rout_count;
     bool clean = true;
     for (int d = 0; d < L->ndepth; d++) {
-        clean = clean && !L->d[d].prolong_pending && !L->d[d].rhs_pending;
+        clean = clean && !L->d[d].prolong_pending && !L->d[d].rhs_pending && !L->d[d].bcoef_pending;
         g.p1[d] = L->d[d].fp.f[SUHMO_F_PHI]; g.a1[d] = L->d[d].phi_alt;
-        L->d[d].prolong_pending = 0; L->d[d].rhs_pending = 0;
+        L->d[d].prolong_pending = 0; L->d[d].rhs_pending = 0; L->d[d].bcoef_pending = 0;
         L->d[d].fp.f[SUHMO_F_PHI] = g.p0[d]; L->d[d].phi_alt = g.a0[d];
     }
     if (e == hipSuccess && rc == 0 && clean && graph && hipGraphInstantiate(&g.exec, graph, nullptr, nullptr, 0) != hipSuccess) g.exec = nullptr;
diff --git a/suhmo_amd/csrc/suhmo_gsrb.hip b/suhmo_amd/csrc/suhmo_gsrb.hip
--- a/suhmo_amd/csrc/suhmo_gsrb.hip
+++ b/suhmo_amd/csrc/suhmo_gsrb.hip
@@ -265,15 +265,20 @@
     d.bx0 = s.bx0; d.bx1 = s.bx1; d.bx2 = s.bx2;
 }
 
-template <int K, bool HAS_ALPHA, int NT, int RM = 0, bool FRHS = false, bool MASKED = true>
+template <int K, bool HAS_ALPHA, int NT, int RM = 0, bool FRHS = false, bool MASKED = true, bool BCF = false>
 __global__ __launch_bounds__(NT) void k_gsrb_fused(DV v, FP fp, const double *__restrict__ pin,
                                                    double *__restrict__ pout, suhmo_phys_t ph, FusedGeom g)
 {
     constexpr bool ROUT = RM == 2, RR = RM != 0;
     static_assert(!(FRHS && (RR || HAS_ALPHA)), "the right-hand side is formed in the plain launch of an alpha = 0 operator");
-    constexpr int LW = 2 * NT, R = 2 * K + 3 + (RR ? 1 : 0);
-    constexpr int HX = 2 * K + (RR ? 2 : 0), EY = RR ? 1 : 0;
+    static_assert(!BCF || (K == 2 && NT == 64 && RM == 0 && !FRHS && !HAS_ALPHA && !MASKED), "the faces are formed in the plain two-sweep launch of a clean-mask alpha = 0 operator");
+    constexpr bool WIDE = RR || BCF;
+    constexpr int DL = BCF ? 1 : 0;
+    constexpr int LW = 2 * NT, R = 2 * K + 3 + (WIDE ? 1 : 0);
+    constexpr int HX = 2 * K + (WIDE ? 2 : 0), EY = RR ? 1 : 0;
     __shared__ double lds[R * LW];
+    __shared__ double rre[BCF ? LW : 1], rsg[BCF ? LW : 1];
+    __shared__ double2 gpv[BCF ? 2 * NT : 1];
 
     int b = blockIdx.x, q = g.ntiles / 8, rem = g.ntiles % 8, xcd = b % 8;
     int tile = xcd * q + (xcd < rem ? xcd : rem) + b / 8;
@@ -300,6 +305,8 @@
     const double *__restrict__ f_Pi = fp.f[SUHMO_F_PI], *__restrict__ f_zb = fp.f[SUHMO_F_ZB];
     const double *__restrict__ f_mask = fp.f[SUHMO_F_MASK], *__restrict__ f_a = fp.f[SUHMO_F_ACOEF];
     const double *__restrict__ f_bx = fp.f[SUHMO_F_BX], *__restrict__ f_by = fp.f[SUHMO_F_BY];
+    const int jminP = BCF ? ((g.wrap_y || jmin > 0) ? jmin - 1 : jmin) : jmin;
+    const int jmaxP = BCF ? ((g.wrap_y || jmax < v.ny - 1) ? jmax + 1 : jmax) : jmax;
 
     auto wrapj = [&](int j) { if (g.wrap_y) { if (j < 0) j += v.ny; else if (j >= v.ny) j -= v.ny; } return j; };
     auto ld2 = [&](const double *__restrict__ p, int idx) { return *reinterpret_cast<const double2 *>(p + idx); };
@@ -311,13 +318,15 @@
     const bool ybc = !v.per[1] && (jmin <= 0 || jmax >= v.ny - 1);
     double2 pnext = make_double2(0.0, 0.0);
     double2 pprev = make_double2(0.0, 0.0);
+    double bw0 = 0.0, be0 = 0.0, bw1 = 0.0, be1 = 0.0, rn0 = 0.0, rn1 = 0.0, rep0 = 0.0, rep1 = 0.0, sgG = 0.0;
+    const bool xedge = c0 - HX <= 0 || c0 + g.W + HX >= v.nx;
     bool usemask = false;
     if constexpr (MASKED) usemask = !g.negflag || *g.negflag == g.mask_epoch;
 
     int sr = 0;
     auto ring = [](int x) { return x < 0 ? x + R : x; };
-    for (int r = jmin - 1; r <= jB - 1 + 2 * K + EY; r++) {
-        bool lphi = cval && (r + 1 >= jmin) && (r + 1 <= jmax);
+    for (int r = jminP - 1; r <= jB - 1 + 2 * K + EY + DL; r++) {
+        bool lphi = cval && (r + 1 >= jminP) && (r + 1 <= jmaxP);
         if (lphi) {
             const int jr = wrapj(r + 1);
             pnext = ld2(pin, cidx(v, im, jr));
@@ -331,13 +340,22 @@
         if (lcf) {
             int idx = cidx(v, im, wrapj(r));
 #define LD2(dst, p, ix) { double2 t_ = ld2(p, ix); dst[0] = t_.x; dst[1] = t_.y; }
-            LD2(cf0.rhs, (FRHS ? g.fres : f_rhs), idx); LD2(cf0.B, f_B, idx); LD2(cf0.Pi, f_Pi, idx);
-            LD2(cf0.zb, f_zb, idx);
+            if constexpr (!BCF) { LD2(cf0.rhs, (FRHS ? g.fres : f_rhs), idx); LD2(cf0.Pi, f_Pi, idx); LD2(cf0.zb, f_zb, idx); }
+            LD2(cf0.B, f_B, idx);
             if constexpr (MASKED) { if (usemask) { LD2(cf0.mask, f_mask, idx); } else { cf0.mask[0] = 1.0; cf0.mask[1] = 1.0; } }
             if (HAS_ALPHA) LD2(cf0.a, f_a, idx);
-            LD2(cf0.byS, f_by, idx); LD2(cf0.byN, f_by, idx + v.P);
-            double2 bxp = ld2(f_bx, idx);
-            cf0.bx0 = bxp.x; cf0.bx1 = bxp.y; cf0.bx2 = f_bx[idx + 2];
+            if constexpr (BCF) { bw0 = f_B[idx - 1]; be0 = f_B[idx + 2]; }
+            else {
+                LD2(cf0.byS, f_by, idx); LD2(cf0.byN, f_by, idx + v.P);
+                double2 bxp = ld2(f_bx, idx);
+                cf0.bx0 = bxp.x; cf0.bx1 = bxp.y; cf0.bx2 = f_bx[idx + 2];
+            }
+        }
+        if constexpr (BCF) {
+            if (cval && (r - 1 >= jmin) && (r - 1 <= jmax)) {
+                const int idx = cidx(v, im, wrapj(r - 1));
+                LD2(cf1.rhs, f_rhs, idx); LD2(cf1.Pi, f_Pi, idx); LD2(cf1.zb, f_zb, idx);
+            }
         }
         __syncthreads();
 
@@ -386,9 +404,9 @@
 
         auto advance_a = [&](const int m, const RowCoef<MASKED> &q, auto a_tag) {
             constexpr int a = decltype(a_tag)::value;
-            const int j = r - m;
+            const int j = r - m - DL;
             const int x = xl + a, i = im + a;
-            const int s0 = ring(sr - m), sN = ring(sr - m + 1), sS = ring(sr - m - 1);
+            const int s0 = ring(sr - m - DL), sN = ring(sr - m - DL + 1), sS = ring(sr - m - DL - 1);
             const double *row = lds + s0 * LW;
             double c = row[x];
             double w = row[(a == 0 && xl == 0) ? 0 : x - 1], e = row[(a == 1 && xl == LW - 2) ? LW - 1 : x + 1];
@@ -411,13 +429,104 @@
             lds[s0 * LW + x] = c + (q.rhs[a] - lofphi) / denom;
         };
         auto advance = [&](const int m, const RowCoef<MASKED> &q) {
-            const int j = r - m;
+            const int j = r - m - DL;
             if (j >= jmin && j <= jmax) {
                 const int a = (j + v.j0 + ((m - 1) & 1)) & 1;
                 if (a) { if (cval) advance_a(m, q, std::integral_constant<int, 1>()); }
                 else   { if (cval) advance_a(m, q, std::integral_constant<int, 0>()); }
             }
         };
+        if constexpr (BCF) {
+            const int j1 = r - 1;
+            const bool faces = j1 >= jmin && j1 <= jmax;
+            double *__restrict__ o_bx = fp.f[SUHMO_F_BX], *__restrict__ o_by = fp.f[SUHMO_F_BY];
+            if (faces && cval) {
+                const double *row = lds + ring(sr - 1) * LW, *rowN = lds + sr * LW, *rowS = lds + ring(sr - 2) * LW;
+                const double ca = row[xl], cb = row[xl + 1];
+                double w = row[xl == 0 ? 0 : xl - 1], e = row[xl == LW - 2 ? LW - 1 : xl + 2];
+                double na = rowN[xl], nb = rowN[xl + 1], sa = rowS[xl], sb = rowS[xl + 1];
+                if (xbc) {
+                    if (im == 0) w = (v.bct[0][0] == 0) ? v.two_v[0][0] - ca : ca + v.neu[0][0];
+                    if (im + 1 == v.nx - 1) e = (v.bct[0][1] == 0) ? v.two_v[0][1] - cb : cb + v.neu[0][1];
+                }
+                if (ybc) {
+                    if (j1 == 0) { sa = (v.bct[1][0] == 0) ? v.two_v[1][0] - ca : ca + v.neu[1][0]; sb = (v.bct[1][0] == 0) ? v.two_v[1][0] - cb : cb + v.neu[1][0]; }
+                    if (j1 == v.ny - 1) { na = (v.bct[1][1] == 0) ? v.two_v[1][1] - ca : ca + v.neu[1][1]; nb = (v.bct[1][1] == 0) ? v.two_v[1][1] - cb : cb + v.neu[1][1]; }
+                }
+                double gx0, gy0, gx1, gy1;
+                gradcc_from(v, ca, w, cb, sa, na, false, false, false, false, gx0, gy0);
+                gradcc_from(v, cb, ca, e, sb, nb, false, false, false, false, gx1, gy1);
+                const double sg0 = grad_norm(gx0, gy0), sg1 = grad_norm(gx1, gy1);
+                rn0 = re_from(ph, sg0, cf1.B[0]); rn1 = re_from(ph, sg1, cf1.B[1]);
+                *reinterpret_cast<double2 *>(rre + xl) = make_double2(rn0, rn1);
+                if (xedge) {
+                    if (v.per[0]) *reinterpret_cast<double2 *>(rsg + xl) = make_double2(sg0, sg1);
+                    else if (im == 0) sgG = grad_norm(2.0 * gx0 - gx1, 2.0 * gy0 - gy1);
+                    else if (im == v.nx - 2) sgG = grad_norm(2.0 * gx1 - gx0, 2.0 * gy1 - gy0);
+                }
+                cf1.byN[0] = 0.0; cf1.byN[1] = 0.0;
+                if (j1 > jmin) {
+                    cf1.byS[0] = bcoef_face(ph, rn0, rep0, cf1.B[0], cf2.B[0], 1.0, 1.0, false);
+                    cf1.byS[1] = bcoef_face(ph, rn1, rep1, cf1.B[1], cf2.B[1], 1.0, 1.0, false);
+                    cf2.byN[0] = cf1.byS[0]; cf2.byN[1] = cf1.byS[1];
+                    double gxp0 = 0.0, gxp1 = 0.0, gyp0 = 0.0, gyp1 = 0.0;
+                    if ((g.wrap_y && (j1 == 0 || j1 == v.ny)) || (ybc && (j1 == 1 || j1 == v.ny - 1))) {
+                        const double2 px = gpv[t], py = gpv[NT + t];
+                        gxp0 = px.x; gxp1 = px.y; gyp0 = py.x; gyp1 = py.y;
+                    }
+                    if (g.wrap_y && (j1 == 0 || j1 == v.ny)) {
+                        const double2 bS = ld2(f_B, cidx(v, im, -1)), bN = ld2(f_B, cidx(v, im, v.ny));
+                        const double sp0 = grad_norm(gxp0, gyp0), sp1 = grad_norm(gxp1, gyp1);
+                        cf1.byS[0] = bcoef_face(ph, rn0, re_from(ph, sp0, bS.x), cf1.B[0], bS.x, 1.0, 1.0, false);
+                        cf1.byS[1] = bcoef_face(ph, rn1, re_from(ph, sp1, bS.y), cf1.B[1], bS.y, 1.0, 1.0, false);
+                        cf2.byN[0] = bcoef_face(ph, re_from(ph, sg0, bN.x), rep0, bN.x, cf2.B[0], 1.0, 1.0, false);
+                        cf2.byN[1] = bcoef_face(ph, re_from(ph, sg1, bN.y), rep1, bN.y, cf2.B[1], 1.0, 1.0, false);
+                        if (own && j1 == v.ny && jB == g.jend) *reinterpret_cast<double2 *>(o_by + cidx(v, i0, v.ny)) = make_double2(cf2.byN[0], cf2.byN[1]);
+                    }
+                    if (ybc && j1 == 1) {
+                        const double2 bS = ld2(f_B, cidx(v, im, -1));
+                        const double rg0 = re_from(ph, grad_norm(2.0 * gxp0 - gx0, 2.0 * gyp0 - gy0), bS.x);
+                        const double rg1 = re_from(ph, grad_norm(2.0 * gxp1 - gx1, 2.0 * gyp1 - gy1), bS.y);
+                        cf2.byS[0] = bcoef_face(ph, rep0, rg0, cf2.B[0], bS.x, 1.0, 1.0, false);
+                        cf2.byS[1] = bcoef_face(ph, rep1, rg1, cf2.B[1], bS.y, 1.0, 1.0, false);
+                        if (own && jA <= 0) *reinterpret_cast<double2 *>(o_by + cidx(v, i0, 0)) = make_double2(cf2.byS[0], cf2.byS[1]);
+                    }
+                    if (ybc && j1 == v.ny - 1) {
+                        const double2 bN = ld2(f_B, cidx(v, im, v.ny));
+                        const double rg0 = re_from(ph, grad_norm(2.0 * gx0 - gxp0, 2.0 * gy0 - gyp0), bN.x);
+                        const double rg1 = re_from(ph, grad_norm(2.0 * gx1 - gxp1, 2.0 * gy1 - gyp1), bN.y);
+                        cf1.byN[0] = bcoef_face(ph, rg0, rn0, bN.x, cf1.B[0], 1.0, 1.0, false);
+                        cf1.byN[1] = bcoef_face(ph, rg1, rn1, bN.y, cf1.B[1], 1.0, 1.0, false);
+                        if (own && jB == g.jend) *reinterpret_cast<double2 *>(o_by + cidx(v, i0, v.ny)) = make_double2(cf1.byN[0], cf1.byN[1]);
+                    }
+                    if (own && j1 >= jA && j1 < jB) *reinterpret_cast<double2 *>(o_by + cidx(v, i0, j1)) = make_double2(cf1.byS[0], cf1.byS[1]);
+                } else { cf1.byS[0] = 0.0; cf1.byS[1] = 0.0; }
+                gpv[t] = make_double2(gx0, gx1); gpv[NT + t] = make_double2(gy0, gy1);
+            }
+            advance(1, cf2);
+            __syncthreads();
+            if (faces && cval) {
+                double reW = rre[xl == 0 ? 0 : xl - 1], reE = rre[xl == LW - 2 ? LW - 1 : xl + 2];
+                if (xedge) {
+                    if (im == 0) reW = re_from(ph, v.per[0] ? rsg[xl == 0 ? 0 : xl - 1] : sgG, bw1);
+                    if (im == v.nx - 2) reE = re_from(ph, v.per[0] ? rsg[xl == LW - 2 ? LW - 1 : xl + 2] : sgG, be1);
+                }
+                cf1.bx0 = bcoef_face(ph, rn0, reW, cf1.B[0], bw1, 1.0, 1.0, false);
+                cf1.bx1 = bcoef_face(ph, rn1, rn0, cf1.B[1], cf1.B[0], 1.0, 1.0, false);
+                cf1.bx2 = bcoef_face(ph, reE, rn1, be1, cf1.B[1], 1.0, 1.0, false);
+                if (own && j1 >= jA && j1 < jB) {
+                    const int idx = cidx(v, i0, j1);
+                    *reinterpret_cast<double2 *>(o_bx + idx) = make_double2(cf1.bx0, cf1.bx1);
+                    if (i0 == v.nx - 2) o_bx[idx + 2] = cf1.bx2;
+                }
+                rep0 = rn0; rep1 = rn1;
+            }
+            advance(2, cf3);
+            __syncthreads();
+            advance(3, cf4);
+            __syncthreads();
+            advance(4, cf5);
+        } else {
         advance(1, cf1);
         __syncthreads();
         advance(2, cf2);
@@ -426,6 +535,7 @@
             advance(3, cf3);
             __syncthreads();
             advance(4, cf4);
+        }
         }
 
         if constexpr (RR) {
@@ -474,20 +584,21 @@
             }
         }
         {
-            const int jo = r - 2 * K;
+            const int jo = r - 2 * K - DL;
             if (own && jo >= jA && jo < jB) {
-                const int so = ring(sr - 2 * K);
+                const int so = ring(sr - 2 * K - DL);
                 double2 o = make_double2(lds[so * LW + xl], lds[so * LW + xl + 1]);
                 *reinterpret_cast<double2 *>(pout + cidx(v, i0, jo)) = o;
             }
         }
         sr = sr + 1 == R ? 0 : sr + 1;
         if (in_row) { lds[sr * LW + xl] = pnext.x; lds[sr * LW + xl + 1] = pnext.y; }
-        if constexpr (RR && K >= 2) copy_coef<HAS_ALPHA, MASKED>(cf5, cf4);
+        if constexpr (WIDE && K >= 2) copy_coef<HAS_ALPHA, MASKED>(cf5, cf4);
         if constexpr (K >= 2) { copy_coef<HAS_ALPHA, MASKED>(cf4, cf3); copy_coef<HAS_ALPHA, MASKED>(cf3, cf2); }
         else if constexpr (RR) copy_coef<HAS_ALPHA, MASKED>(cf3, cf2);
         copy_coef<HAS_ALPHA, MASKED>(cf2, cf1);
-        copy_coef<HAS_ALPHA, MASKED>(cf1, cf0);
+        if constexpr (BCF) { CP2(cf1, cf0, B); bw1 = bw0; be1 = be0; }
+        else copy_coef<HAS_ALPHA, MASKED>(cf1, cf0);
     }
     if constexpr (ROUT) {
         if (g.onorm) {
@@ -520,7 +631,9 @@
         HIPCHK(hipMemsetAsync(D.phi_alt, 0, D.elems * sizeof(double), st));
     }
     FusedGeom g;
-    constexpr int HX = 2 * K + (RR ? 2 : 0), EY = RR ? 1 : 0;
+    const bool bcf = D.bcoef_pending != 0;
+    const int HX = 2 * K + ((RR || bcf) ? 2 : 0);
+    constexpr int EY = RR ? 1 : 0;
     const int maxW = 2 * NT - 2 * HX;
     g.nstrips = (v.nx + maxW - 1) / maxW;
     g.W = 2 * ((v.nx + 2 * g.nstrips - 1) / (2 * g.nstrips));
@@ -592,6 +705,16 @@
         g.onorm = nullptr;
         if ((L->resout_req & 4) && (size_t)g.nstrips * g.nchunks + 4 < L->scratch_elems) { g.onorm = L->scratch + 2; L->resout_np = g.nstrips * g.nchunks; }
         else L->resout_np = 0;
+    }
+    if (bcf) {
+        if constexpr (K == 2 && NT == 64 && !RR) {
+            if (part || depth != 0 || !unmasked || D.rhs_pending || g.pc || v.ext[0] || v.ext[1]) { suhmo_set_error("internal: bcoef_pending on a launch that cannot form the faces"); return -4; }
+            D.bcoef_pending = 0; L->bcoef_in_relax_count++;
+            hipLaunchKernelGGL((k_gsrb_fused<2, false, 64, 0, false, false, true>), dim3(g.ntiles), dim3(NT), 0, st, v, D.fp, pin, D.phi_alt, L->ph, g);
+            L->relax_unmasked++; L->bcoef_unmasked++;
+            { std::swap(D.fp.f[SUHMO_F_PHI], D.phi_alt); suhmo_fp_changed(); }
+            return 0;
+        } else { suhmo_set_error("internal: bcoef_pending on a launch that cannot form the faces"); return -4; }
     }
     if (D.rhs_pending) {
         if constexpr (K == 2 && NT == 64 && !RR) {
@@ -1089,6 +1212,14 @@
     if (!(D.v.ext[0] || D.v.ext[1])) return true;
     return strip && L->ex && rhs_local && L->desc.nx_global == 0 && D.phi_fresh >= D.v.gy && D.v.gy >= 2 * K + 1 && D.v.ny >= D.v.gy;
 }
+bool suhmo_gsrb_can_fuse_bcoef(suhmo_level *L, int sweeps)
+{
+    Depth &D = L->d[0];
+    if (!L->bcoef_in_relax || !suhmo_mask_clean(L, 0) || D.v.alpha != 0.0 || L->ex) return false;
+    if (D.v.ext[0] || D.v.ext[1] || D.v.cfx[0] || D.v.cfx[1] || D.prolong_pending || D.rhs_pending) return false;
+    const int nt = L->fused_nt ? L->fused_nt : ((long)D.v.nx * D.v.ny >= 8000000L ? 256 : 64);
+    return sweeps >= 3 && nt == 64 && pick_K(L, D, pick_variant(L, D), sweeps) == 2;
+}
 bool suhmo_gsrb_can_fuse_prolong(suhmo_level *L, int depth, int sweeps)
 {
     Depth &D = L->d[depth];
@@ -1147,6 +1278,7 @@
             HIPCHK(hipEventRecord(pe.a, st));
         }
         int tchunks = 1;
+        bool bcf = false;
         if (TS) {
             if (L->tile_chunks && !ext && TS == 4 && single_tile(L, D.v)) tchunks = (sweeps - it) / TS;
             const bool rst = trst && it + TS * tchunks == sweeps;
@@ -1206,7 +1338,11 @@
                 if (rc < 0) return rc;
                 HIPCHK(hipStreamWaitEvent(st, L->xev[1], 0));
                 if (rc == 1) rc = launch(0); else { rc = launch(2); L->overlapped++; }
-            } else rc = launch(0);
+            } else {
+                bcf = D.bcoef_pending != 0;
+                rc = launch(0);
+                if (!rc && bcf && D.bcoef_pending) rc = -4;
+            }
             if (rc) return rc;
             if (rst) *restricted = 1;
             if (rout) { L->resout_done = 1; L->resout_count++; }
@@ -1216,9 +1352,10 @@
         if (prof) {
             HIPCHK(hipEventRecord(pe.b, st));
             pe.cells = (long)D.v.nx * D.v.ny * done;
-            pe.restricts = (restricted && *restricted && it + done == sweeps) ? 1 : 0;
+            pe.restricts = bcf ? 2 : (restricted && *restricted && it + done == sweeps) ? 1 : 0;
             L->prof.push_back(pe);
         }
+        if (bcf) { int rc = suhmo_average_operator_all(L, L->bcoef_nd, st); if (rc) return rc; }
         it += done;
     }
     HIPCHK(hipGetLastError());
diff --git a/suhmo_amd/csrc/suhmo_level.hip b/suhmo_amd/csrc/suhmo_level.hip
--- a/suhmo_amd/csrc/suhmo_level.hip
+++ b/suhmo_amd/csrc/suhmo_level.hip
@@ -164,6 +164,7 @@
     L->agg_min_cells = 100000; L->agg_depth = 0; L->agg_world = 1; L->agg_rank = 0; L->agg = nullptr; L->ag = nullptr; L->ag_user = nullptr;
     L->agg_send = L->agg_recv = nullptr; L->agg_cap = 0; L->agg_gathers = 0; L->agg_static_stale = 0;
     L->frhs_stream = L->frhs_tile = 0;
+    L->bcoef_in_relax = 1; L->bcoef_nd = 0; L->bcoef_in_relax_count = 0;
     L->resout_np = 0;
     L->resout_req = L->resout_armed = L->resout_done = 0; L->resout_rhs = nullptr; L->resout_count = 0; L->resid_in_relax = 1;
     L->graph_max_cells = 1500000; L->gstream = nullptr; L->vgraph_replays = 0; memset(L->vgraph_seen, 0, sizeof(L->vgraph_seen));
@@ -178,7 +179,7 @@
             {"SUHMO_GSRB_VARIANT", &suhmo_level::gsrb_variant}, {"SUHMO_FUSED_HC", &suhmo_level::fused_hc}, {"SUHMO_BCOEF_FUSED", &suhmo_level::bcoef_fused},
             {"SUHMO_BCOEF_TILE_X", &suhmo_level::bcoef_tile_x}, {"SUHMO_FUSED_NT", &suhmo_level::fused_nt}, {"SUHMO_OVERLAP_HALO", &suhmo_level::overlap_halo},
             {"SUHMO_STRIPS_RHS_LOCAL", &suhmo_level::strips_rhs_local}, {"SUHMO_FAS_RHS_FUSED", &suhmo_level::fas_rhs_fused},
-            {"SUHMO_RESID_IN_RELAX", &suhmo_level::resid_in_relax}, {"SUHMO_TILE_STRIPS", &suhmo_level::tile_strips}, {"SUHMO_TILE_CHUNKS", &suhmo_level::tile_chunks},
+            {"SUHMO_RESID_IN_RELAX", &suhmo_level::resid_in_relax}, {"SUHMO_BCOEF_IN_RELAX", &suhmo_level::bcoef_in_relax}, {"SUHMO_TILE_STRIPS", &suhmo_level::tile_strips}, {"SUHMO_TILE_CHUNKS", &suhmo_level::tile_chunks},
             {"SUHMO_TILE_RESTRICT", &suhmo_level::tile_restrict}, {"SUHMO_TILE_ORDER", &suhmo_level::tile_order}, {"SUHMO_FAS_RHS_IN_RELAX", &suhmo_level::fas_rhs_in_relax},
             {"SUHMO_TILE_S", &suhmo_level::tile_s}, {"SUHMO_GSRB_TILE", &suhmo_level::gsrb_tile}, {"SUHMO_TILE_T", &suhmo_level::tile_t},
             {"SUHMO_FUSED_RESTRICT", &suhmo_level::fused_restrict}, {"SUHMO_SKIP_MASK", &suhmo_level::skip_mask}, {"SUHMO_MASK_KNOWN", &suhmo_level::mask_known},
@@ -231,7 +232,7 @@
         D.elems = (size_t)D.v.P * (size_t)(D.v.rows + 1);
         D.nbox = L->desc.nbox;
         memset(&D.fp, 0, sizeof(D.fp));
-        D.phi_alt = nullptr; D.prolong_pending = 0; D.rhs_pending = 0; D.phi_fresh = 0;
+        D.phi_alt = nullptr; D.prolong_pending = 0; D.rhs_pending = 0; D.bcoef_pending = 0; D.phi_fresh = 0;
     }
     L->scratch = nullptr; L->scratch_elems = 0; L->hscratch = nullptr; L->hscratch_dev = nullptr; L->hseq = 0;
     L->mask_epoch = 0; L->maskflag_epoch = 0; L->mask_reported = 0; L->coarse_mask_ok = 0;
@@ -331,7 +332,7 @@
         {"fused_nt", &suhmo_level::fused_nt}, {"fused_restrict", &suhmo_level::fused_restrict}, {"strips_rhs_local", &suhmo_level::strips_rhs_local},
         {"tile_strips", &suhmo_level::tile_strips}, {"overlap_halo", &suhmo_level::overlap_halo}, {"skip_mask", &suhmo_level::skip_mask}, {"mask_known", &suhmo_level::mask_known}, {"tile_chunks",
             &suhmo_level::tile_chunks}, {"tile_order", &suhmo_level::tile_order}, {"tile_restrict", &suhmo_level::tile_restrict}, {"fas_rhs_in_relax",
-            &suhmo_level::fas_rhs_in_relax}, {"resid_in_relax", &suhmo_level::resid_in_relax}, {"fas_rhs_fused", &suhmo_level::fas_rhs_fused},
+            &suhmo_level::fas_rhs_in_relax}, {"resid_in_relax", &suhmo_level::resid_in_relax}, {"bcoef_in_relax", &suhmo_level::bcoef_in_relax}, {"fas_rhs_fused", &suhmo_level::fas_rhs_fused},
         {"tile_s", &suhmo_level::tile_s}, {"gsrb_tile", &suhmo_level::gsrb_tile}, {"tile_t", &suhmo_level::tile_t}, {"poll_readback", &suhmo_level::poll_readback}};
     for (const auto &e : tab) if (!strcmp(key, e.k)) return &(L->*(e.m));
     return nullptr;
@@ -371,6 +372,7 @@
     if (!strcmp(key, "rhs_in_streaming_launches")) { *value = L->frhs_stream; return 0; }
     if (!strcmp(key, "rhs_in_tile_launches")) { *value = L->frhs_tile; return 0; }
     if (!strcmp(key, "residual_in_relax_launches")) { *value = L->resout_count; return 0; }
+    if (!strcmp(key, "bcoef_in_relax_launches")) { *value = L->bcoef_in_relax_count; return 0; }
     if (!strcmp(key, "mask_scans")) { *value = L->mask_scans; return 0; }
     if (!strcmp(key, "mask_state")) { *value = L->mask_state; return 0; }
     if (!strcmp(key, "bcoef_unmasked_launches")) { *value = L->bcoef_unmasked; return 0; }
```

New measurement: 504.8 V-cycles/s, median of 6. +1.5%, better.
